# Gadersd/whisper-burn

Measured on NVIDIA H100. Metric: audio-seconds/sec, higher is better.
Workload: dtype f32 (fp16-exact weights, fp32 activations/accumulate)

## Files before the change

### include/whisper_b200.h

```cpp
#ifndef WHISPER_B200_H
#define WHISPER_B200_H

#include <stddef.h>
#include <stdint.h>

#ifdef __cplusplus
extern "C" {
#endif

#define WB_OK 0
#define WB_ERR_INVALID_ARG 1
#define WB_ERR_CUDA 2
#define WB_ERR_OOM 3
#define WB_ERR_STATE 4
#define WB_ERR_UNSUPPORTED 5

#define WB_KV_F32 0
#define WB_KV_F16 1

#define WB_WINDOWS_REFERENCE 0
#define WB_WINDOWS_NATIVE 1

#define WB_SEARCH_BEAM 0
#define WB_SEARCH_GREEDY_LOOP 1

typedef struct wb_model wb_model;
typedef struct wb_session wb_session;

typedef struct wb_dims {
    int32_t n_mels, n_audio_ctx, n_audio_state, n_audio_head, n_audio_layer;
    int32_t n_vocab, n_text_ctx, n_text_state, n_text_head, n_text_layer;
} wb_dims;

typedef struct wb_special_ids {
    int64_t sot, lang, transcribe, notimestamps, eot;
} wb_special_ids;

const char* wb_version(void);
const char* wb_last_error(void);
int wb_device_count(int* n_out);

int64_t wb_max_waveform_samples(int64_t n_frame_max);
int64_t wb_window_samples(int64_t n_audio_ctx, int window_mode);
int wb_prep_audio(int device, const float* wave, int64_t n_batch, int64_t n_samples,
                  float* mel_out, int64_t* n_frames_out);
int wb_prep_audio_dev(int device, const float* wave_dev, int64_t n_batch, int64_t n_samples,
                      float* mel_out_dev, int64_t* n_frames_out);

int wb_model_create(const wb_dims* dims, int device, wb_model** out);
int wb_model_set_tensor(wb_model* m, const char* path, const float* data, const int64_t* shape, int ndim);
int wb_npy_tree_probe(const char* dir, wb_dims* dims_out);
int wb_model_load_npy_tree(const char* dir, int device, int ln_eps_outside, wb_model** out);
int wb_model_set_layernorm_eps_mode(wb_model* m, int outside);
int wb_model_finalize(wb_model* m);
void wb_model_destroy(wb_model* m);
int wb_model_get_dims(const wb_model* m, wb_dims* out);
int wb_model_weights_fp16_exact(const wb_model* m);

int wb_forward_encoder(wb_model* m, const float* mel, int64_t n_batch, int64_t n_mels, int64_t n_ctx,
                       float* out);
int wb_forward_decoder(wb_model* m, const int64_t* tokens, int64_t n_batch, int64_t seq_len,
                       const float* encoder_output, int64_t n_enc_ctx, float* logits_out);

int wb_session_create(wb_model* m, int64_t max_windows, int64_t max_beams, int64_t max_text_len,
                      int kv_dtype, wb_session** out);
int wb_session_create_windows(wb_model* m, int64_t max_windows, int64_t max_beams, int64_t max_text_len,
                              int kv_dtype, int window_mode, wb_session** out);
void wb_session_destroy(wb_session* s);
int wb_session_set_search(wb_session* s, int rule);
int wb_session_set_prev_prompt(wb_session* s, int64_t startofprev);
int wb_session_encode_waveforms(wb_session* s, const float* const* waves, const int64_t* lens,
                                int64_t n_windows);
int wb_session_encode_waveforms_dev(wb_session* s, const float* wave_dev, const int64_t* offsets,
                                    const int64_t* lens, int64_t n_windows);
int wb_session_encode_mels(wb_session* s, const float* mel, int64_t n_windows, int64_t n_mels, int64_t n_ctx);
int wb_session_get_mel(wb_session* s, int64_t window, float* mel_out, int64_t capacity, int64_t* n_ctx_out);
int wb_session_get_encoder_output(wb_session* s, int64_t window, float* out, int64_t capacity, int64_t* n_ctx_out);
int wb_session_begin(wb_session* s, const int64_t* prompt, int64_t prompt_len);
int wb_session_step(wb_session* s, int64_t n_rows, const int32_t* window_of_row, const int32_t* parent_row,
                    const int64_t* token, int apply_special_mask, const uint8_t* is_special,
                    int k, int64_t* topk_ids_out, float* topk_logprob_out);

int wb_transcribe_windows(wb_session* s, const float* const* waves, const int64_t* lens, int64_t n_windows,
                          int beam_size, int max_depth, const wb_special_ids* ids, const uint8_t* is_special,
                          int64_t* tokens_out, int64_t capacity, int64_t* lens_out);
int wb_transcribe_windows_dev(wb_session* s, const float* wave_dev, const int64_t* offsets, const int64_t* lens,
                              int64_t n_windows, int beam_size, int max_depth, const wb_special_ids* ids,
                              const uint8_t* is_special, int64_t* tokens_out, int64_t capacity, int64_t* lens_out);
int wb_transcribe_windows_prev(wb_session* s, const float* const* waves, const int64_t* lens, int64_t n_windows,
                               const int64_t* prev_tokens, const int64_t* prev_lens, int64_t startofprev, int beam_size,
                               int max_depth, const wb_special_ids* ids, const uint8_t* is_special, int64_t* tokens_out,
                               int64_t capacity, int64_t* lens_out);
int wb_waveform_to_tokens(wb_session* s, const float* waveform, int64_t n_samples, int64_t sample_rate,
                          int beam_size, int max_depth, const wb_special_ids* ids, const uint8_t* is_special,
                          int64_t* tokens_out, int64_t capacity, int64_t* n_tokens_out);
int wb_waveforms_to_tokens(wb_session* s, const float* const* waveforms, const int64_t* n_samples, int64_t n_waveforms,
                           int64_t sample_rate, int beam_size, int max_depth, const wb_special_ids* ids,
                           const uint8_t* is_special, int64_t* tokens_out, int64_t capacity, int64_t* n_tokens_out);
int wb_session_last_logprobs(wb_session* s, int64_t index, float* out, int64_t capacity, int64_t* n_out);
int wb_session_score_tokens(wb_session* s, int64_t n_seqs, const int32_t* window_of_seq, const int64_t* tokens,
                            const int64_t* lens, int apply_special_mask, const uint8_t* is_special,
                            float* lp_out, int64_t* argmax_out);
int64_t wb_window_count(int64_t n_samples, int64_t sample_rate, int64_t window_len);
int wb_window_bounds(int64_t n_samples, int64_t sample_rate, int64_t window_len, int64_t* starts, int64_t* ends);
int wb_find_chunk_overlap(const int64_t* prev, int64_t n_prev, const int64_t* curr, int64_t n_curr,
                          int64_t max_n_offsets, int64_t min_n_overlaps, int64_t* prev_index, int64_t* curr_index);
int64_t wb_first_repetition_end(const int64_t* tokens, int64_t n, int64_t period);
int64_t wb_repetition_period(const int64_t* tokens, int64_t n, int64_t min_repetitions);
int wb_find_repeated_tokens_index(const int64_t* tokens, int64_t n, int64_t window_size, int64_t min_repeat_count,
                                  int64_t* first_repeat_index, int64_t* end);

int64_t wb_beam_get_top_elements(const double* scores, int64_t n, int64_t num, int64_t* idx_out);

int64_t wb_beam_search_table(const double* table, int64_t n_ctx, int64_t n_vocab, int64_t first_token, int64_t eot,
                             int64_t beam_size, int64_t max_depth, int64_t* seq_out, int64_t capacity);
int64_t wb_beam_search_table_fixed(const double* table, int64_t n_ctx, int64_t n_vocab, int64_t first_token, int64_t eot,
                                   int64_t beam_size, int64_t max_depth, int64_t* seq_out, int64_t capacity);

int wb_load_wav(const char* path, int strict_16k_mono, float* out, int64_t capacity, int64_t* n_samples_out,
                int64_t* sample_rate_out, int* channels_out);

int wb_session_last_decoder(const wb_session* s);
int wb_session_last_topk(wb_session* s, int64_t n_rows, int64_t k, int64_t* ids_out, float* lp_out);
int64_t wb_kernel_launch_count(void);
void wb_kernel_launch_count_reset(void);
int wb_session_last_timings(wb_session* s, float* ms_out4);
int wb_session_last_steps(wb_session* s, int64_t* n_steps_out);
int wb_session_profile_decode(wb_session* s, const wb_special_ids* ids, int n_steps, float* logits_kernel_ms,
                              float* step_ms);

#ifdef __cplusplus
}
#endif
#endif
```

### whisper-burn_b200/csrc/api.cu

```cuda
#include <algorithm>
#include <cstring>
#include <map>
#include <memory>
#include <mutex>
#include <new>

#include "../host/beam.hpp"
#include "../host/beam_fixed.hpp"
#include "../host/repeat.hpp"
#include "session.h"

struct wb_model {
    wb::Model impl;
    std::mutex fwd_mu;
    std::unique_ptr<wb::Session> fwd;
    wb::Session& forward_session(int64_t n_windows, int64_t text_len) {
        if (!fwd || fwd->max_windows < n_windows || fwd->t_max < text_len) {
            fwd.reset();
            fwd.reset(new wb::Session(&impl, std::max<int64_t>(n_windows, 1), 1, std::max<int64_t>(text_len, 2), WB_KV_F32));
        }
        return *fwd;
    }
    ~wb_model() { fwd.reset(); }
};
struct wb_session {
    std::unique_ptr<wb::Session> impl;
    wb_model* model;
    std::vector<std::vector<float>> logprobs;
    bool have_logprobs = false;
};

namespace {

template <typename F>
int guarded(F&& f) {
    try {
        f();
        return WB_OK;
    } catch (const wb::Error& e) {
        wb::set_last_error(e.what());
        return e.code;
    } catch (const std::bad_alloc&) {
        wb::set_last_error("host out of memory");
        return WB_ERR_OOM;
    } catch (const std::exception& e) {
        wb::set_last_error(e.what());
        return WB_ERR_CUDA;
    }
}

void require_device(int device) {
    int n = 0;
    cudaError_t e = cudaGetDeviceCount(&n);
    if (e != cudaSuccess || n == 0) {
        cudaGetLastError();
        wb::fail(WB_ERR_CUDA, std::string("no CUDA device available (there is no CPU fallback): ") + cudaGetErrorString(e));
    }
    if (device < 0 || device >= n) wb::fail(WB_ERR_INVALID_ARG, "device index out of range");
    WB_CUDA(cudaSetDevice(device));
}

void copy_tokens_out(const std::vector<std::vector<int64_t>>& toks, int64_t* tokens_out, int64_t capacity,
                     int64_t* lens_out) {
    for (size_t w = 0; w < toks.size(); ++w) {
        WB_REQUIRE((int64_t)toks[w].size() <= capacity, "tokens_out capacity too small");
        for (size_t i = 0; i < toks[w].size(); ++i) tokens_out[(int64_t)w * capacity + (int64_t)i] = toks[w][i];
        lens_out[w] = (int64_t)toks[w].size();
    }
}

bool special_given(const wb_session* s, const uint8_t* is_special) {
    return is_special != nullptr || (s && s->impl->search == WB_SEARCH_GREEDY_LOOP);
}

void collect_timings(wb::Session& s) {
    WB_CUDA(cudaStreamSynchronize(s.st));
    cudaEventElapsedTime(&s.last_ms[0], s.ev[0], s.ev[1]);
    cudaEventElapsedTime(&s.last_ms[1], s.ev[1], s.ev[2]);
    cudaEventElapsedTime(&s.last_ms[2], s.ev[2], s.ev[3]);
    cudaEventElapsedTime(&s.last_ms[3], s.ev[0], s.ev[3]);
}

void prep_audio_device(wb::Model& model, const float* wave_dev, int64_t n_batch, int64_t n_samples, float* mel_out_dev,
                       int64_t* n_frames_out, cudaStream_t st) {
    using namespace wb;
    WB_REQUIRE(n_batch >= 1, "prep_audio: n_batch must be >= 1");
    WB_REQUIRE(n_samples >= N_FFT, "prep_audio: waveform shorter than n_fft (audio.rs:292)");
    WB_REQUIRE(n_samples < ((int64_t)1 << 30), "prep_audio: waveform too long");
    const int F = (int)(n_samples / HOP);
    std::vector<LogMelWindow> lw((size_t)n_batch);
    for (int64_t b = 0; b < n_batch; ++b)
        lw[(size_t)b] = LogMelWindow{b * n_samples, (int)n_samples, F, F, 0, b * (int64_t)F * N_MELS};
    DevBuf<LogMelWindow> dwin;
    DevBuf<int> slot;
    DevBuf<float> rows;
    dwin.alloc((size_t)n_batch);
    slot.alloc(1);
    rows.alloc((size_t)n_batch * F * N_MELS + 4);
    WB_CUDA(cudaMemcpyAsync(dwin.p, lw.data(), lw.size() * sizeof(LogMelWindow), cudaMemcpyHostToDevice, st));
    if (F > 0) {
        launch_logmel(model, wave_dev, dwin.p, (int)n_batch, F, rows.p, slot.p, 1, st);
        for (int64_t b = 0; b < n_batch; ++b)
            launch_rows_to_chan(rows.p + b * (int64_t)F * N_MELS, mel_out_dev + b * (int64_t)N_MELS * F, F, st);
    }
    WB_CUDA(cudaStreamSynchronize(st));
    if (n_frames_out) *n_frames_out = F;
}

struct FrontendOnly {
    wb::Model m;
    explicit FrontendOnly(int device) {
        using namespace wb;
        m.device = device;
        const FrontendTables& ft = frontend_tables();
        auto up = [&](const void* src, size_t bytes) {
            void* p = nullptr;
            WB_CUDA(cudaMalloc(&p, bytes));
            m.allocs.push_back(p);
            WB_CUDA(cudaMemcpy(p, src, bytes, cudaMemcpyHostToDevice));
            return p;
        };
        m.basis_t = (float*)up(ft.basis_t.data(), ft.basis_t.size() * sizeof(float));
        m.mel_filt = (float*)up(ft.mel_filt.data(), ft.mel_filt.size() * sizeof(float));
        std::vector<int> rng(2 * N_MELS);
        for (int i = 0; i < N_MELS; ++i) { rng[2 * i] = ft.mel_lo[i]; rng[2 * i + 1] = ft.mel_hi[i]; }
        m.mel_range = (int*)up(rng.data(), rng.size() * sizeof(int));
    }
};

FrontendOnly& frontend_for(int device) {
    static std::mutex mu;
    static std::map<int, std::unique_ptr<FrontendOnly>> cache;
    std::lock_guard<std::mutex> lock(mu);
    auto& slot = cache[device];
    if (!slot) slot.reset(new FrontendOnly(device));
    return *slot;
}

}

extern "C" {

const char* wb_version(void) { return "whisper_b200 0.1.0 (sm_90a)"; }
const char* wb_last_error(void) { return wb::last_error_string().c_str(); }

int wb_device_count(int* n_out) {
    return guarded([&] {
        WB_REQUIRE(n_out != nullptr, "null output");
        int n = 0;
        if (cudaGetDeviceCount(&n) != cudaSuccess) { cudaGetLastError(); n = 0; }
        *n_out = n;
    });
}

int64_t wb_max_waveform_samples(int64_t n_frame_max) {
    return (int64_t)wb::HOP * (n_frame_max + 1) + (wb::N_FFT % 2) - 1;
}

int wb_prep_audio(int device, const float* wave, int64_t n_batch, int64_t n_samples, float* mel_out,
                  int64_t* n_frames_out) {
    return guarded([&] {
        WB_REQUIRE(wave && mel_out, "prep_audio: null pointer");
        WB_REQUIRE(n_batch >= 1, "prep_audio: n_batch must be >= 1");
        WB_REQUIRE(n_samples >= wb::N_FFT, "prep_audio: waveform shorter than n_fft (audio.rs:292)");
        require_device(device);
        FrontendOnly& fe = frontend_for(device);
        const int64_t F = n_samples / wb::HOP;
        wb::DevBuf<float> dw, dm;
        dw.alloc((size_t)(n_batch * n_samples));
        dm.alloc((size_t)(n_batch * wb::N_MELS * F) + 4);
        WB_CUDA(cudaMemcpy(dw.p, wave, (size_t)(n_batch * n_samples) * sizeof(float), cudaMemcpyHostToDevice));
        prep_audio_device(fe.m, dw.p, n_batch, n_samples, dm.p, n_frames_out, nullptr);
        WB_CUDA(cudaMemcpy(mel_out, dm.p, (size_t)(n_batch * wb::N_MELS * F) * sizeof(float), cudaMemcpyDeviceToHost));
    });
}

int wb_prep_audio_dev(int device, const float* wave_dev, int64_t n_batch, int64_t n_samples, float* mel_out_dev,
                      int64_t* n_frames_out) {
    return guarded([&] {
        WB_REQUIRE(wave_dev && mel_out_dev, "prep_audio: null pointer");
        require_device(device);
        FrontendOnly& fe = frontend_for(device);
        prep_audio_device(fe.m, wave_dev, n_batch, n_samples, mel_out_dev, n_frames_out, nullptr);
    });
}

int wb_model_create(const wb_dims* dims, int device, wb_model** out) {
    return guarded([&] {
        WB_REQUIRE(dims && out, "model_create: null pointer");
        WB_REQUIRE(dims->n_mels > 0 && dims->n_audio_ctx > 0 && dims->n_audio_state > 0 && dims->n_audio_head > 0 &&
                       dims->n_audio_layer > 0 && dims->n_vocab > 0 && dims->n_text_ctx > 0 && dims->n_text_state > 0 &&
                       dims->n_text_head > 0 && dims->n_text_layer > 0,
                   "model_create: non-positive dimension");
        require_device(device);
        wb_model* m = new wb_model();
        m->impl.dims = *dims;
        m->impl.device = device;
        *out = m;
    });
}

int wb_model_set_tensor(wb_model* m, const char* path, const float* data, const int64_t* shape, int ndim) {
    return guarded([&] {
        WB_REQUIRE(m != nullptr, "null model");
        wb::model_set_tensor(m->impl, path, data, shape, ndim);
    });
}

int wb_npy_tree_probe(const char* dir, wb_dims* dims_out) {
    return guarded([&] {
        WB_REQUIRE(dir && dims_out, "npy_tree_probe: null pointer");
        wb::npy_tree_probe(dir, *dims_out);
    });
}

int wb_model_load_npy_tree(const char* dir, int device, int ln_eps_outside, wb_model** out) {
    return guarded([&] {
        WB_REQUIRE(dir && out, "model_load_npy_tree: null pointer");
        wb_dims dims{};
        wb::npy_tree_probe(dir, dims);
        require_device(device);
        std::unique_ptr<wb_model> m(new wb_model());
        m->impl.dims = dims;
        m->impl.device = device;
        m->impl.ln_eps_outside = ln_eps_outside ? 1 : 0;
        wb::npy_tree_load(m->impl, dir);
        wb::model_finalize(m->impl);
        *out = m.release();
    });
}

int wb_model_set_layernorm_eps_mode(wb_model* m, int outside) {
    return guarded([&] {
        WB_REQUIRE(m != nullptr, "null model");
        if (m->impl.finalized) wb::fail(WB_ERR_STATE, "model already finalized");
        m->impl.ln_eps_outside = outside ? 1 : 0;
    });
}

int wb_model_finalize(wb_model* m) {
    return guarded([&] {
        WB_REQUIRE(m != nullptr, "null model");
        wb::model_finalize(m->impl);
    });
}

void wb_model_destroy(wb_model* m) { delete m; }

int wb_model_get_dims(const wb_model* m, wb_dims* out) {
    return guarded([&] {
        WB_REQUIRE(m && out, "null pointer");
        *out = m->impl.dims;
    });
}

int wb_model_weights_fp16_exact(const wb_model* m) { return (m && m->impl.fp16_exact) ? 1 : 0; }

int wb_forward_encoder(wb_model* m, const float* mel, int64_t n_batch, int64_t n_mels, int64_t n_ctx, float* out) {
    return guarded([&] {
        WB_REQUIRE(m && mel && out, "forward_encoder: null pointer");
        WB_REQUIRE(n_batch >= 1, "forward_encoder: n_batch must be >= 1");
        std::lock_guard<std::mutex> lock(m->fwd_mu);
        wb::Session& s = m->forward_session(n_batch, 2);
        s.encode_mels_host(mel, n_batch, n_mels, n_ctx);
        const int d = m->impl.dims.n_audio_state;
        WB_CUDA(cudaMemcpy(out, s.xa.p, (size_t)s.M_tot * d * sizeof(float), cudaMemcpyDeviceToHost));
    });
}

int wb_forward_decoder(wb_model* m, const int64_t* tokens, int64_t n_batch, int64_t seq_len, const float* encoder_output,
                       int64_t n_enc_ctx, float* logits_out) {
    return guarded([&] {
        WB_REQUIRE(m && tokens && encoder_output && logits_out, "forward_decoder: null pointer");
        const wb_dims& D = m->impl.dims;
        WB_REQUIRE(n_batch >= 1 && seq_len >= 1, "forward_decoder: empty input");
        WB_REQUIRE(seq_len <= D.n_text_ctx, "Token sequence length must not exceed n_text_ctx (mod.rs:134-139)");
        std::lock_guard<std::mutex> lock(m->fwd_mu);
        wb::Session& s = m->forward_session(n_batch, std::min<int64_t>(D.n_text_ctx, std::max<int64_t>(seq_len, 2)));
        s.load_encoder_output_host(encoder_output, n_batch, n_enc_ctx);
        s.teacher_forced_logits(tokens, n_batch, seq_len, logits_out);
    });
}

int64_t wb_window_samples(int64_t n_audio_ctx, int window_mode) {
    if (n_audio_ctx <= wb::MEL_PADDING || n_audio_ctx > INT32_MAX / 2 || (window_mode != WB_WINDOWS_REFERENCE && window_mode != WB_WINDOWS_NATIVE)) return -1;
    return wb::window_samples((int)n_audio_ctx, window_mode);
}

int wb_session_create_windows(wb_model* m, int64_t max_windows, int64_t max_beams, int64_t max_text_len, int kv_dtype,
                              int window_mode, wb_session** out) {
    return guarded([&] {
        WB_REQUIRE(m && out, "session_create: null pointer");
        std::unique_ptr<wb_session> s(new wb_session());
        s->model = m;
        s->impl.reset(new wb::Session(&m->impl, max_windows, max_beams, max_text_len, kv_dtype, window_mode));
        *out = s.release();
    });
}

int wb_session_create(wb_model* m, int64_t max_windows, int64_t max_beams, int64_t max_text_len, int kv_dtype,
                      wb_session** out) {
    return wb_session_create_windows(m, max_windows, max_beams, max_text_len, kv_dtype, WB_WINDOWS_REFERENCE, out);
}

void wb_session_destroy(wb_session* s) { delete s; }

int wb_session_set_search(wb_session* s, int rule) {
    return guarded([&] {
        WB_REQUIRE(s, "set_search: null pointer");
        s->impl->set_search(rule);
    });
}

int wb_session_set_prev_prompt(wb_session* s, int64_t startofprev) {
    return guarded([&] {
        WB_REQUIRE(s, "set_prev_prompt: null pointer");
        s->impl->set_prev_prompt(startofprev);
    });
}

int wb_session_encode_waveforms(wb_session* s, const float* const* waves, const int64_t* lens, int64_t n_windows) {
    return guarded([&] {
        WB_REQUIRE(s && waves && lens, "encode: null pointer");
        s->impl->encode_waveforms_host(waves, lens, n_windows);
        WB_CUDA(cudaStreamSynchronize(s->impl->st));
    });
}

int wb_session_encode_waveforms_dev(wb_session* s, const float* wave_dev, const int64_t* offsets, const int64_t* lens,
                                    int64_t n_windows) {
    return guarded([&] {
        WB_REQUIRE(s && wave_dev && offsets && lens, "encode: null pointer");
        s->impl->encode_from_device_wave(wave_dev, offsets, lens, n_windows);
        WB_CUDA(cudaStreamSynchronize(s->impl->st));
    });
}

int wb_session_encode_mels(wb_session* s, const float* mel, int64_t n_windows, int64_t n_mels, int64_t n_ctx) {
    return guarded([&] {
        WB_REQUIRE(s && mel, "encode: null pointer");
        s->impl->encode_mels_host(mel, n_windows, n_mels, n_ctx);
    });
}

int wb_session_get_mel(wb_session* s, int64_t window, float* mel_out, int64_t capacity, int64_t* n_ctx_out) {
    return guarded([&] {
        WB_REQUIRE(s && mel_out && n_ctx_out, "get_mel: null pointer");
        wb::Session& S = *s->impl;
        if (!S.encoded) wb::fail(WB_ERR_STATE, "get_mel: nothing encoded");
        WB_REQUIRE(window >= 0 && window < S.n_windows, "get_mel: window out of range");
        const int Tm = S.win_Tm[(size_t)window];
        WB_REQUIRE(capacity >= (int64_t)Tm * wb::N_MELS, "get_mel: capacity too small");
        std::vector<float> rows((size_t)Tm * wb::N_MELS);
        WB_CUDA(cudaMemcpy(rows.data(), S.mel_rows.p + ((int64_t)window * S.TmS + 1) * wb::N_MELS,
                           rows.size() * sizeof(float), cudaMemcpyDeviceToHost));
        for (int t = 0; t < Tm; ++t)
            for (int c = 0; c < wb::N_MELS; ++c) mel_out[(int64_t)c * Tm + t] = rows[(size_t)t * wb::N_MELS + c];
        *n_ctx_out = Tm;
    });
}

int wb_session_get_encoder_output(wb_session* s, int64_t window, float* out, int64_t capacity, int64_t* n_ctx_out) {
    return guarded([&] {
        WB_REQUIRE(s && out && n_ctx_out, "get_encoder_output: null pointer");
        wb::Session& S = *s->impl;
        if (!S.encoded) wb::fail(WB_ERR_STATE, "get_encoder_output: nothing encoded");
        WB_REQUIRE(window >= 0 && window < S.n_windows, "get_encoder_output: window out of range");
        const int d = S.m->dims.n_audio_state;
        const int T = S.win_T[(size_t)window];
        WB_REQUIRE(capacity >= (int64_t)T * d, "get_encoder_output: capacity too small");
        WB_CUDA(cudaMemcpy(out, S.xa.p + S.win_row_off[(size_t)window] * d, (size_t)T * d * sizeof(float),
                           cudaMemcpyDeviceToHost));
        *n_ctx_out = T;
    });
}

int wb_session_begin(wb_session* s, const int64_t* prompt, int64_t prompt_len) {
    return guarded([&] {
        WB_REQUIRE(s && prompt, "begin: null pointer");
        WB_REQUIRE(prompt_len >= 1, "begin: prompt length out of range");
        s->impl->begin(std::vector<std::vector<int64_t>>((size_t)s->impl->n_windows, std::vector<int64_t>(prompt, prompt + prompt_len)));
    });
}

int wb_session_step(wb_session* s, int64_t n_rows, const int32_t* window_of_row, const int32_t* parent_row,
                    const int64_t* token, int apply_special_mask, const uint8_t* is_special, int k,
                    int64_t* topk_ids_out, float* topk_logprob_out) {
    return guarded([&] {
        WB_REQUIRE(s && window_of_row && parent_row && token && topk_ids_out && topk_logprob_out, "step: null pointer");
        if (is_special) s->impl->set_special(is_special);
        WB_REQUIRE(!apply_special_mask || s->impl->have_special, "step: special mask requested but no is_special bitmap given");
        s->impl->step_beams(n_rows, window_of_row, parent_row, token, apply_special_mask, k, topk_ids_out, topk_logprob_out);
    });
}

int wb_transcribe_windows(wb_session* s, const float* const* waves, const int64_t* lens, int64_t n_windows,
                          int beam_size, int max_depth, const wb_special_ids* ids, const uint8_t* is_special,
                          int64_t* tokens_out, int64_t capacity, int64_t* lens_out) {
    return guarded([&] {
        WB_REQUIRE(s && waves && lens && ids && special_given(s, is_special) && tokens_out && lens_out, "transcribe: null pointer");
        s->have_logprobs = false;
        s->impl->encode_waveforms_host(waves, lens, n_windows);
        std::vector<std::vector<int64_t>> toks;
        wb::transcribe_windows(*s->impl, beam_size, max_depth, *ids, is_special, toks, s->logprobs);
        copy_tokens_out(toks, tokens_out, capacity, lens_out);
        collect_timings(*s->impl);
        s->have_logprobs = true;
    });
}

int wb_transcribe_windows_prev(wb_session* s, const float* const* waves, const int64_t* lens, int64_t n_windows,
                               const int64_t* prev_tokens, const int64_t* prev_lens, int64_t startofprev, int beam_size,
                               int max_depth, const wb_special_ids* ids, const uint8_t* is_special, int64_t* tokens_out,
                               int64_t capacity, int64_t* lens_out) {
    return guarded([&] {
        WB_REQUIRE(s && waves && lens && prev_lens && ids && special_given(s, is_special) && tokens_out && lens_out,
                   "transcribe_windows_prev: null pointer");
        wb::Session& S = *s->impl;
        WB_REQUIRE(n_windows >= 1 && n_windows <= S.max_windows, "transcribe_windows_prev: n_windows out of range");
        WB_REQUIRE(startofprev >= 0 && startofprev < S.m->dims.n_vocab, "transcribe_windows_prev: startofprev id out of range");
        WB_REQUIRE(max_depth >= 0, "transcribe_windows_prev: negative max_depth");
        std::vector<std::vector<int64_t>> prev((size_t)n_windows);
        int64_t off = 0, max_lp = 4;
        for (int64_t w = 0; w < n_windows; ++w) {
            WB_REQUIRE(prev_lens[w] >= 0, "transcribe_windows_prev: negative prev_lens entry");
            WB_REQUIRE(prev_lens[w] == 0 || prev_tokens, "transcribe_windows_prev: null prev_tokens");
            WB_REQUIRE(prev_lens[w] == 0 || S.search != WB_SEARCH_GREEDY_LOOP,
                       "transcribe_windows_prev: the greedy loop builds its own prompt; no previous ids with it");
            prev[(size_t)w].assign(prev_tokens + off, prev_tokens + off + prev_lens[w]);
            for (int64_t t : prev[(size_t)w])
                WB_REQUIRE(t >= 0 && t < S.m->dims.n_vocab, "transcribe_windows_prev: previous id out of range");
            off += prev_lens[w];
            max_lp = std::max(max_lp, prev_lens[w] > 0 ? prev_lens[w] + 5 : 4);
        }
        WB_REQUIRE(max_lp + max_depth <= S.t_max, "transcribe_windows_prev: prompt + max_depth exceeds the session's max_text_len");
        WB_REQUIRE(capacity >= max_lp + max_depth + 1, "transcribe_windows_prev: capacity below prompt + max_depth + 1");
        s->have_logprobs = false;
        S.encode_waveforms_host(waves, lens, n_windows);
        std::vector<std::vector<int64_t>> toks;
        wb::transcribe_windows(S, beam_size, max_depth, *ids, is_special, toks, s->logprobs, prev, startofprev);
        copy_tokens_out(toks, tokens_out, capacity, lens_out);
        collect_timings(S);
        s->have_logprobs = true;
    });
}

int wb_transcribe_windows_dev(wb_session* s, const float* wave_dev, const int64_t* offsets, const int64_t* lens,
                              int64_t n_windows, int beam_size, int max_depth, const wb_special_ids* ids,
                              const uint8_t* is_special, int64_t* tokens_out, int64_t capacity, int64_t* lens_out) {
    return guarded([&] {
        WB_REQUIRE(s && wave_dev && offsets && lens && ids && special_given(s, is_special) && tokens_out && lens_out, "transcribe: null pointer");
        s->have_logprobs = false;
        s->impl->encode_from_device_wave(wave_dev, offsets, lens, n_windows);
        std::vector<std::vector<int64_t>> toks;
        wb::transcribe_windows(*s->impl, beam_size, max_depth, *ids, is_special, toks, s->logprobs);
        copy_tokens_out(toks, tokens_out, capacity, lens_out);
        collect_timings(*s->impl);
        s->have_logprobs = true;
    });
}

int64_t wb_window_count(int64_t n_samples, int64_t sample_rate, int64_t window_len) {
    return (int64_t)wb::window_bounds(n_samples, sample_rate, window_len).size();
}

int wb_window_bounds(int64_t n_samples, int64_t sample_rate, int64_t window_len, int64_t* starts, int64_t* ends) {
    return guarded([&] {
        WB_REQUIRE(starts && ends, "window_bounds: null pointer");
        const auto b = wb::window_bounds(n_samples, sample_rate, window_len);
        for (size_t i = 0; i < b.size(); ++i) { starts[i] = b[i].first; ends[i] = b[i].second; }
    });
}

static void merge_window(std::vector<int64_t>& tokens, std::vector<float>& tlp, const std::vector<int64_t>& nt,
                         const std::vector<float>& nl) {
    int64_t pi = 0, ci = 0;
    if (wb::find_chunk_overlap(tokens.data(), (int64_t)tokens.size(), nt.data(), (int64_t)nt.size(), 40, 3, &pi, &ci)) {
        tokens.resize((size_t)pi);
        tokens.insert(tokens.end(), nt.begin() + ci, nt.end());
        tlp.resize((size_t)pi);
        tlp.insert(tlp.end(), nl.begin() + ci, nl.end());
    } else {
        tokens.insert(tokens.end(), nt.begin(), nt.end());
        tlp.insert(tlp.end(), nl.begin(), nl.end());
    }
}

static std::vector<int64_t> prev_nonspecial(const std::vector<int64_t>& tokens, const uint8_t* is_special) {
    std::vector<int64_t> prev;
    for (size_t i = tokens.size(); i-- > 0 && prev.size() < 5;)
        if (!is_special[tokens[i]]) prev.push_back(tokens[i]);
    std::reverse(prev.begin(), prev.end());
    return prev;
}

static void waveforms_to_tokens(wb::Session& S, const float* const* waveforms, const int64_t* n_samples, int64_t n_waveforms,
                                int64_t sample_rate, int beam_size, int max_depth, const wb_special_ids& ids,
                                const uint8_t* is_special, std::vector<std::vector<int64_t>>& out,
                                std::vector<std::vector<float>>& out_lp) {
    WB_REQUIRE(sample_rate == 16000, "waveform_to_tokens: only 16 kHz input is supported (frontend tables are built for 16 kHz)");
    const int64_t window_len = wb::window_samples(S.m->dims.n_audio_ctx, S.window_mode);
    std::vector<const float*> ptrs;
    std::vector<int64_t> lens;
    std::vector<int> owner;
    for (int64_t w = 0; w < n_waveforms; ++w)
        for (const auto& b : wb::window_bounds(n_samples[w], sample_rate, window_len)) {
            ptrs.push_back(waveforms[w] + b.first);
            lens.push_back(b.second - b.first);
            owner.push_back((int)w);
        }
    out.assign((size_t)n_waveforms, {});
    out_lp.assign((size_t)n_waveforms, {});
    const bool prev_prompt = S.startofprev >= 0;
    if (prev_prompt) {
        WB_REQUIRE(S.search != WB_SEARCH_GREEDY_LOOP, "waveform_to_tokens: the greedy loop builds its own prompt; no previous-text prompt with it");
        WB_REQUIRE(is_special != nullptr, "waveform_to_tokens: the previous-text prompt needs is_special");
    }
    std::vector<std::vector<size_t>> rounds(1);
    if (prev_prompt) {
        std::vector<int> idx((size_t)n_waveforms, 0);
        for (size_t j = 0; j < ptrs.size(); ++j) {
            const size_t i = (size_t)idx[(size_t)owner[j]]++;
            if (rounds.size() <= i) rounds.resize(i + 1);
            rounds[i].push_back(j);
        }
    } else {
        for (size_t j = 0; j < ptrs.size(); ++j) rounds[0].push_back(j);
    }
    for (const std::vector<size_t>& round : rounds) {
        for (size_t b0 = 0; b0 < round.size(); b0 += (size_t)S.max_windows) {
            const size_t nb = std::min(round.size() - b0, (size_t)S.max_windows);
            std::vector<const float*> bp(nb);
            std::vector<int64_t> bl(nb);
            std::vector<std::vector<int64_t>> prev(prev_prompt ? nb : 0);
            for (size_t i = 0; i < nb; ++i) {
                const size_t j = round[b0 + i];
                bp[i] = ptrs[j];
                bl[i] = lens[j];
                if (prev_prompt) prev[i] = prev_nonspecial(out[(size_t)owner[j]], is_special);
            }
            S.encode_waveforms_host(bp.data(), bl.data(), (int64_t)nb);
            std::vector<std::vector<int64_t>> toks;
            std::vector<std::vector<float>> lps;
            wb::transcribe_windows(S, beam_size, max_depth, ids, is_special, toks, lps, prev, S.startofprev);
            for (size_t i = 0; i < nb; ++i)
                merge_window(out[(size_t)owner[round[b0 + i]]], out_lp[(size_t)owner[round[b0 + i]]], toks[i], lps[i]);
        }
    }
    collect_timings(S);
}

int wb_waveform_to_tokens(wb_session* s, const float* waveform, int64_t n_samples, int64_t sample_rate, int beam_size,
                          int max_depth, const wb_special_ids* ids, const uint8_t* is_special, int64_t* tokens_out,
                          int64_t capacity, int64_t* n_tokens_out) {
    return guarded([&] {
        WB_REQUIRE(s && waveform && ids && special_given(s, is_special) && tokens_out && n_tokens_out, "waveform_to_tokens: null pointer");
        s->have_logprobs = false;
        std::vector<std::vector<int64_t>> out;
        waveforms_to_tokens(*s->impl, &waveform, &n_samples, 1, sample_rate, beam_size, max_depth, *ids, is_special, out, s->logprobs);
        WB_REQUIRE((int64_t)out[0].size() <= capacity, "tokens_out capacity too small");
        std::memcpy(tokens_out, out[0].data(), out[0].size() * sizeof(int64_t));
        *n_tokens_out = (int64_t)out[0].size();
        s->have_logprobs = true;
    });
}

int wb_waveforms_to_tokens(wb_session* s, const float* const* waveforms, const int64_t* n_samples, int64_t n_waveforms,
                           int64_t sample_rate, int beam_size, int max_depth, const wb_special_ids* ids,
                           const uint8_t* is_special, int64_t* tokens_out, int64_t capacity, int64_t* n_tokens_out) {
    return guarded([&] {
        WB_REQUIRE(s && waveforms && n_samples && ids && special_given(s, is_special) && tokens_out && n_tokens_out, "waveforms_to_tokens: null pointer");
        WB_REQUIRE(n_waveforms >= 1, "waveforms_to_tokens: n_waveforms must be >= 1");
        s->have_logprobs = false;
        std::vector<std::vector<int64_t>> out;
        waveforms_to_tokens(*s->impl, waveforms, n_samples, n_waveforms, sample_rate, beam_size, max_depth, *ids, is_special, out,
                            s->logprobs);
        for (int64_t w = 0; w < n_waveforms; ++w) {
            WB_REQUIRE((int64_t)out[(size_t)w].size() <= capacity, "tokens_out capacity (per waveform) too small");
            std::memcpy(tokens_out + w * capacity, out[(size_t)w].data(), out[(size_t)w].size() * sizeof(int64_t));
            n_tokens_out[w] = (int64_t)out[(size_t)w].size();
        }
        s->have_logprobs = true;
    });
}

int wb_session_last_logprobs(wb_session* s, int64_t index, float* out, int64_t capacity, int64_t* n_out) {
    return guarded([&] {
        WB_REQUIRE(s && n_out, "last_logprobs: null pointer");
        if (!s->have_logprobs) wb::fail(WB_ERR_STATE, "last_logprobs: no transcribe or waveform(s)_to_tokens call yet");
        WB_REQUIRE(index >= 0 && index < (int64_t)s->logprobs.size(), "last_logprobs: index out of range");
        const std::vector<float>& v = s->logprobs[(size_t)index];
        *n_out = (int64_t)v.size();
        if (!out) return;
        WB_REQUIRE(capacity >= (int64_t)v.size(), "last_logprobs: capacity too small");
        std::memcpy(out, v.data(), v.size() * sizeof(float));
    });
}

int wb_session_score_tokens(wb_session* s, int64_t n_seqs, const int32_t* window_of_seq, const int64_t* tokens, const int64_t* lens,
                            int apply_special_mask, const uint8_t* is_special, float* lp_out, int64_t* argmax_out) {
    return guarded([&] {
        WB_REQUIRE(s && window_of_seq && tokens && lens && lp_out, "score_tokens: null pointer");
        s->impl->score_tokens(n_seqs, window_of_seq, tokens, lens, apply_special_mask != 0, is_special, lp_out, argmax_out);
    });
}

int wb_find_chunk_overlap(const int64_t* prev, int64_t n_prev, const int64_t* curr, int64_t n_curr, int64_t max_n_offsets,
                          int64_t min_n_overlaps, int64_t* prev_index, int64_t* curr_index) {
    int64_t pi = 0, ci = 0;
    const bool found = wb::find_chunk_overlap(prev, n_prev, curr, n_curr, max_n_offsets, min_n_overlaps, &pi, &ci);
    if (found) {
        if (prev_index) *prev_index = pi;
        if (curr_index) *curr_index = ci;
    }
    return found ? 1 : 0;
}

int64_t wb_first_repetition_end(const int64_t* tokens, int64_t n, int64_t period) {
    if ((!tokens && n > 0) || n < 0) return -1;
    return wb::repeat::first_repetition_end(tokens, n, period);
}

int64_t wb_repetition_period(const int64_t* tokens, int64_t n, int64_t min_repetitions) {
    if ((!tokens && n > 0) || n < 0) return -1;
    return wb::repeat::repetition_period(tokens, n, min_repetitions);
}

int wb_find_repeated_tokens_index(const int64_t* tokens, int64_t n, int64_t window_size, int64_t min_repeat_count, int64_t* first_repeat_index,
                                  int64_t* end) {
    if ((!tokens && n > 0) || n < 0 || !first_repeat_index || !end) return -1;
    return wb::repeat::find_repeated_tokens_index(tokens, n, window_size, min_repeat_count, first_repeat_index, end);
}

int64_t wb_beam_get_top_elements(const double* scores, int64_t n, int64_t num, int64_t* idx_out) {
    if (!scores || !idx_out || n < 0 || num < 0) return -1;
    std::vector<double> v(scores, scores + n);
    const auto top = wb::beam::get_top_elements(v, [](double s) { return s; }, (size_t)num);
    for (size_t i = 0; i < top.size(); ++i) idx_out[i] = (int64_t)top[i];
    return (int64_t)top.size();
}

int wb_load_wav(const char* path, int strict_16k_mono, float* out, int64_t capacity, int64_t* n_samples_out, int64_t* sample_rate_out,
                int* channels_out) {
    return guarded([&] {
        WB_REQUIRE(path && n_samples_out, "load_wav: null pointer");
        std::vector<float> v;
        int64_t sr = 0;
        int ch = 0;
        wb::load_wav(path, strict_16k_mono != 0, v, sr, ch);
        *n_samples_out = (int64_t)v.size();
        if (sample_rate_out) *sample_rate_out = sr;
        if (channels_out) *channels_out = ch;
        if (out) {
            WB_REQUIRE(capacity >= (int64_t)v.size(), "load_wav: capacity too small");
            std::memcpy(out, v.data(), v.size() * sizeof(float));
        }
    });
}

int wb_session_last_decoder(const wb_session* s) { return s ? s->impl->last_decoder : -1; }

int wb_session_last_topk(wb_session* s, int64_t n_rows, int64_t k, int64_t* ids_out, float* lp_out) {
    return guarded([&] {
        WB_REQUIRE(s && ids_out && lp_out, "last_topk: null pointer");
        s->impl->last_topk(n_rows, k, ids_out, lp_out);
    });
}

int64_t wb_beam_search_table(const double* table, int64_t n_ctx, int64_t n_vocab, int64_t first_token, int64_t eot, int64_t beam_size,
                             int64_t max_depth, int64_t* seq_out, int64_t capacity) {
    if (!table || !seq_out || n_ctx < 1 || n_vocab < 1 || beam_size < 1 || max_depth < 0) return -1;
    using Node = wb::beam::BeamNode<int64_t>;
    auto next = [&](const std::vector<Node>& beams) {
        std::vector<std::vector<std::pair<int64_t, double>>> out(beams.size());
        for (size_t b = 0; b < beams.size(); ++b) {
            const int64_t t = beams[b].seq.back(), n = (int64_t)beams[b].seq.size();
            const double* row = table + ((t * 131 + n) % n_ctx) * n_vocab;
            out[b].reserve((size_t)n_vocab);
            for (int64_t v = 0; v < n_vocab; ++v) out[b].emplace_back(v, beams[b].log_prob + row[v]);
        }
        return out;
    };
    auto fin = [&](const std::vector<int64_t>& seq) { return !seq.empty() && seq.back() == eot; };
    std::vector<Node> init(1);
    init[0].seq = {first_token};
    init[0].log_prob = 0.0;
    const std::vector<int64_t> best = wb::beam::beam_search(init, next, fin, (size_t)beam_size, (size_t)max_depth);
    if ((int64_t)best.size() > capacity) return -1;
    for (size_t i = 0; i < best.size(); ++i) seq_out[i] = best[i];
    return (int64_t)best.size();
}

int64_t wb_beam_search_table_fixed(const double* table, int64_t n_ctx, int64_t n_vocab, int64_t first_token, int64_t eot,
                                   int64_t beam_size, int64_t max_depth, int64_t* seq_out, int64_t capacity) {
    namespace fx = wb::beamfx;
    if (!table || !seq_out || n_ctx < 1 || n_vocab < 1 || beam_size < 1 || beam_size > fx::MAX_BEAM || max_depth < 0) return -1;
    const int B = (int)beam_size;
    std::vector<fx::Head> heads(1);
    std::vector<std::vector<int64_t>> seqs(1, std::vector<int64_t>{first_token});
    heads[0] = fx::Head{0.0, first_token == eot ? 1 : 0, 0, 1, 0};
    std::vector<double> scores((size_t)n_vocab);
    for (int64_t depth = 0; depth < max_depth; ++depth) {
        const int n = (int)heads.size();
        if (fx::search_done(heads.data(), n)) break;
        int step_row[fx::MAX_NODES], cand_id[fx::MAX_NODES * fx::MAX_BEAM];
        double cand_lp[fx::MAX_NODES * fx::MAX_BEAM];
        for (int b = 0; b < n; ++b) {
            step_row[b] = b;
            for (int i = 0; i < B; ++i) cand_id[b * B + i] = -1;
            if (heads[(size_t)b].finished) continue;
            const int64_t t = seqs[(size_t)b].back(), len = (int64_t)seqs[(size_t)b].size();
            const double* row = table + ((t * 131 + len) % n_ctx) * n_vocab;
            for (int64_t v = 0; v < n_vocab; ++v) scores[(size_t)v] = heads[(size_t)b].log_prob + row[v];
            int top[fx::MAX_BEAM + 1];
            const int nt = fx::top_elements(scores.data(), (int)n_vocab, B, top);
            for (int i = 0; i < nt; ++i) {
                cand_id[b * B + i] = top[i];
                cand_lp[b * B + i] = row[top[i]];
            }
        }
        fx::Pick out[fx::MAX_NODES];
        const int n_out = fx::beam_step(heads.data(), n, step_row, cand_id, cand_lp, B, (int)eot, out);
        std::vector<fx::Head> nh((size_t)n_out);
        std::vector<std::vector<int64_t>> ns((size_t)n_out);
        for (int i = 0; i < n_out; ++i) {
            nh[(size_t)i] = out[i].head;
            ns[(size_t)i] = seqs[(size_t)out[i].src];
            if (out[i].token >= 0) ns[(size_t)i].push_back(out[i].token);
        }
        heads.swap(nh);
        seqs.swap(ns);
    }
    const int best = fx::max_by_last(heads.data(), (int)heads.size());
    if (best < 0) return 0;
    const std::vector<int64_t>& s = seqs[(size_t)best];
    if ((int64_t)s.size() > capacity) return -1;
    for (size_t i = 0; i < s.size(); ++i) seq_out[i] = s[i];
    return (int64_t)s.size();
}

int64_t wb_kernel_launch_count(void) { return wb::g_launch_count; }
void wb_kernel_launch_count_reset(void) { wb::g_launch_count = 0; }

int wb_session_last_timings(wb_session* s, float* ms_out4) {
    return guarded([&] {
        WB_REQUIRE(s && ms_out4, "null pointer");
        for (int i = 0; i < 4; ++i) ms_out4[i] = s->impl->last_ms[i];
    });
}

int wb_session_profile_decode(wb_session* s, const wb_special_ids* ids, int n_steps, float* logits_kernel_ms,
                              float* step_ms) {
    return guarded([&] {
        WB_REQUIRE(s && ids && logits_kernel_ms && step_ms, "null pointer");
        const int64_t prompt[4] = {ids->sot, ids->lang, ids->transcribe, ids->notimestamps};
        s->impl->profile_decode(prompt, 4, n_steps, logits_kernel_ms, step_ms);
    });
}

int wb_session_last_steps(wb_session* s, int64_t* n_steps_out) {
    return guarded([&] {
        WB_REQUIRE(s && n_steps_out, "null pointer");
        *n_steps_out = s->impl->last_steps;
    });
}

}
```

### whisper-burn_b200/csrc/gemm_f16.cu

```cuda
#include <cuda.h>
#include <cuda_fp16.h>

#include <climits>
#include <cstring>
#include <mutex>
#include <type_traits>

#include "prims.cuh"
#include "wb_internal.h"
#include "wgmma.cuh"

namespace wb {

namespace {

constexpr int F_BM = 128, F_BK = 64, F_STAGES = 4;
constexpr int F_CONSUMERS = 256;
constexpr int F_THREADS = F_CONSUMERS + 32;

__device__ __forceinline__ void tma_load_3d(void* dst, const CUtensorMap* map, uint64_t* bar, int c0, int c1, int c2) {
    asm volatile("cp.async.bulk.tensor.3d.shared::cluster.global.tile.mbarrier::complete_tx::bytes [%0], [%1, {%3, %4, %5}], [%2];" ::"r"(smem_u32(dst)), "l"(map),
                 "r"(smem_u32(bar)), "r"(c0), "r"(c1), "r"(c2)
                 : "memory");
}
__device__ __forceinline__ void tma_load_2d(void* dst, const CUtensorMap* map, uint64_t* bar, int c0, int c1) {
    asm volatile("cp.async.bulk.tensor.2d.shared::cluster.global.tile.mbarrier::complete_tx::bytes [%0], [%1, {%3, %4}], [%2];" ::"r"(smem_u32(dst)), "l"(map),
                 "r"(smem_u32(bar)), "r"(c0), "r"(c1)
                 : "memory");
}
template <int BN>
__device__ __forceinline__ void wgmma_tile(float (&d)[BN / 2], uint64_t desc_a, uint64_t desc_b) {
    if constexpr (BN == 128) wgmma_m64n128k16(d, desc_a, desc_b);
    else wgmma_m64n64k16(d, desc_a, desc_b);
}

struct F16Args {
    float* C;
    __half *P_hi, *P_lo;
    const float* bias;
    const float* residual;
    const float* pos;
    const GemmGroup* groups;
    GemmGroup single;
    int64_t ldc;
    int N, K;
    int act;
    float scale;
    int scale_cols;
};
struct LogitArgs : F16Args {
    const int* target;
    const uint8_t* row_mask;
    const uint8_t* is_special;
    int V, n_tiles;
    float *tile_m, *tile_s, *tgt_logit;
    int* tile_i;
};

template <int BN>
__device__ __forceinline__ void logit_stats_epilogue(const float (&acc_h)[BN / 2], const float (&acc_l)[BN / 2], const LogitArgs& g, int rows,
                                                     int m_base, int n0, int lane) {
#pragma unroll
    for (int hrow = 0; hrow < 2; ++hrow) {
        const int m = m_base + 8 * hrow;
        const bool live = m < rows;
        const int mr = live ? m : 0;
        const bool masked = g.row_mask != nullptr && g.row_mask[mr] != 0;
        const int tgt = g.target[mr];
        float mx = -INFINITY;
        int ai = INT_MAX;
#pragma unroll
        for (int j = 0; j < BN / 8; ++j)
#pragma unroll
            for (int e = 0; e < 2; ++e) {
                const int n = n0 + 8 * j + 2 * (lane & 3) + e;
                const float x = hl_join(acc_h[4 * j + 2 * hrow + e], acc_l[4 * j + 2 * hrow + e]);
                if (live && n == tgt) g.tgt_logit[m] = x;
                const bool ok = n < g.V && !(masked && __ldg(g.is_special + n));
                if (ok && x > mx) { mx = x; ai = n; }
            }
#pragma unroll
        for (int o = 1; o <= 2; o <<= 1) {
            const float om = __shfl_xor_sync(0xffffffffu, mx, o);
            const int oi = __shfl_xor_sync(0xffffffffu, ai, o);
            if (om > mx || (om == mx && oi < ai)) { mx = om; ai = oi; }
        }
        float s = 0.0f;
#pragma unroll
        for (int j = 0; j < BN / 8; ++j)
#pragma unroll
            for (int e = 0; e < 2; ++e) {
                const int n = n0 + 8 * j + 2 * (lane & 3) + e;
                const float x = hl_join(acc_h[4 * j + 2 * hrow + e], acc_l[4 * j + 2 * hrow + e]);
                if (n < g.V && !(masked && __ldg(g.is_special + n))) s += expf(x - mx);
            }
        s += __shfl_xor_sync(0xffffffffu, s, 1);
        s += __shfl_xor_sync(0xffffffffu, s, 2);
        if (live && (lane & 3) == 0) {
            const int64_t o = (int64_t)m * g.n_tiles + blockIdx.x;
            g.tile_m[o] = mx;
            g.tile_s[o] = s;
            g.tile_i[o] = ai;
        }
    }
}

template <int BN, typename Args>
__global__ void __launch_bounds__(F_THREADS, 1)
gemm_f16_tc_kernel(const __grid_constant__ CUtensorMap map_a_hi, const __grid_constant__ CUtensorMap map_a_lo,
                   const __grid_constant__ CUtensorMap map_b, const Args g) {
    extern __shared__ __align__(1024) uint8_t smem_raw[];
    constexpr int A_BYTES = F_BM * F_BK * 2;
    constexpr int B_BYTES = BN * F_BK * 2;
    constexpr int STAGE = 2 * A_BYTES + B_BYTES;
    uint8_t* base = reinterpret_cast<uint8_t*>((reinterpret_cast<uintptr_t>(smem_raw) + 1023) & ~(uintptr_t)1023);
    uint64_t* full = reinterpret_cast<uint64_t*>(base + F_STAGES * STAGE);
    uint64_t* empty = full + F_STAGES;

    const int warp = threadIdx.x >> 5, lane = threadIdx.x & 31;
    const GemmGroup grp = g.groups ? g.groups[blockIdx.z] : g.single;
    const int m0 = blockIdx.y * F_BM;
    if (m0 >= grp.rows) return;
    const int n0 = blockIdx.x * BN;
    const int nkb = (g.K + F_BK - 1) / F_BK;

    if (threadIdx.x == F_CONSUMERS) {
        asm volatile("prefetch.tensormap [%0];" ::"l"(&map_a_hi) : "memory");
        asm volatile("prefetch.tensormap [%0];" ::"l"(&map_a_lo) : "memory");
        asm volatile("prefetch.tensormap [%0];" ::"l"(&map_b) : "memory");
        for (int s = 0; s < F_STAGES; ++s) {
            mbar_init(full + s, 1);
            mbar_init(empty + s, 2);
        }
        mbar_fence_init();
    }
    __syncthreads();

    if (threadIdx.x >= F_CONSUMERS) {
        if (lane == 0) {
            for (int i = 0; i < nkb; ++i) {
                const int s = i % F_STAGES;
                const uint32_t ph = (i / F_STAGES) & 1;
                mbar_wait(empty + s, ph ^ 1);
                mbar_expect_tx(full + s, STAGE);
                uint8_t* st = base + s * STAGE;
                tma_load_3d(st, &map_a_hi, full + s, i * F_BK, m0, blockIdx.z);
                tma_load_3d(st + A_BYTES, &map_a_lo, full + s, i * F_BK, m0, blockIdx.z);
                tma_load_2d(st + 2 * A_BYTES, &map_b, full + s, i * F_BK, n0);
            }
        }
        return;
    }
    const int wg = warp >> 2;
    float acc_h[BN / 2], acc_l[BN / 2];
#pragma unroll
    for (int j = 0; j < BN / 2; ++j) { acc_h[j] = 0.0f; acc_l[j] = 0.0f; }
    wgmma_fence_regs(acc_h);
    wgmma_fence_regs(acc_l);
#pragma unroll 1
    for (int i = 0; i < nkb; ++i) {
        const int s = i % F_STAGES;
        mbar_wait(full + s, (i / F_STAGES) & 1);
        const uint32_t st = smem_u32(base + s * STAGE);
        const uint64_t dah = wgmma_desc(st + wg * 8192), dal = wgmma_desc(st + A_BYTES + wg * 8192), db = wgmma_desc(st + 2 * A_BYTES);
        wgmma_fence();
#pragma unroll
        for (int k = 0; k < F_BK / 16; ++k) {
            wgmma_tile<BN>(acc_h, dah + 2 * k, db + 2 * k);
            wgmma_tile<BN>(acc_l, dal + 2 * k, db + 2 * k);
        }
        wgmma_commit();
        wgmma_wait<1>();
        if (i > 0 && (threadIdx.x & 127) == 0) mbar_arrive(empty + (i - 1) % F_STAGES);
    }
    wgmma_wait<0>();
    wgmma_fence_regs(acc_h);
    wgmma_fence_regs(acc_l);

    if constexpr (std::is_same<Args, LogitArgs>::value) {
        logit_stats_epilogue<BN>(acc_h, acc_l, g, grp.rows, m0 + wg * 64 + (warp & 3) * 16 + (lane >> 2), n0, lane);
    } else {
#pragma unroll
        for (int hrow = 0; hrow < 2; ++hrow) {
            const int m = m0 + wg * 64 + (warp & 3) * 16 + (lane >> 2) + 8 * hrow;
            if (m >= grp.rows) continue;
            const int64_t crow = grp.c_off + (int64_t)m * g.ldc;
#pragma unroll
            for (int j = 0; j < BN / 8; ++j) {
                const int n = n0 + 8 * j + 2 * (lane & 3);
                float v[2];
#pragma unroll
                for (int e = 0; e < 2; ++e) {
                    float t = hl_join(acc_h[4 * j + 2 * hrow + e], acc_l[4 * j + 2 * hrow + e]);
                    if (g.bias) t = __fadd_rn(t, __ldg(g.bias + n + e));
                    if (g.act == ACT_GELU) t = gelu_erf(t);
                    if (n + e < g.scale_cols) t = __fmul_rn(t, g.scale);
                    v[e] = t;
                }
                if (g.pos) {
                    const float2 p2 = __ldg(reinterpret_cast<const float2*>(g.pos + (int64_t)m * g.N + n));
                    v[0] = __fadd_rn(v[0], p2.x); v[1] = __fadd_rn(v[1], p2.y);
                }
                if (g.residual) {
                    const float2 r2 = *reinterpret_cast<const float2*>(g.residual + crow + n);
                    v[0] = __fadd_rn(r2.x, v[0]); v[1] = __fadd_rn(r2.y, v[1]);
                }
                if (g.C) *reinterpret_cast<float2*>(g.C + crow + n) = make_float2(v[0], v[1]);
                if (g.P_hi) {
                    __half2 h, l;
                    hl_split_pair(v[0], v[1], h, l);
                    *reinterpret_cast<__half2*>(g.P_hi + crow + n) = h;
                    *reinterpret_cast<__half2*>(g.P_lo + crow + n) = l;
                }
            }
        }
    }
}

__global__ void split_f16_kernel(const float4* __restrict__ src, uint2* __restrict__ hi, uint2* __restrict__ lo, int64_t n4) {
    for (int64_t i = (int64_t)blockIdx.x * blockDim.x + threadIdx.x; i < n4; i += (int64_t)gridDim.x * blockDim.x)
        hl_split4(src[i], hi[i], lo[i]);
}

typedef CUresult (*EncodeTiledFn)(CUtensorMap*, CUtensorMapDataType, cuuint32_t, void*, const cuuint64_t*, const cuuint64_t*,
                                  const cuuint32_t*, const cuuint32_t*, CUtensorMapInterleave, CUtensorMapSwizzle,
                                  CUtensorMapL2promotion, CUtensorMapFloatOOBfill);

EncodeTiledFn encode_fn() {
    static std::once_flag once;
    static EncodeTiledFn fn = nullptr;
    std::call_once(once, [] {
        void* p = nullptr;
        cudaDriverEntryPointQueryResult q;
        if (cudaGetDriverEntryPoint("cuTensorMapEncodeTiled", &p, cudaEnableDefault, &q) == cudaSuccess && q == cudaDriverEntryPointSuccess) fn = (EncodeTiledFn)p;
    });
    if (!fn) fail(WB_ERR_CUDA, "cuTensorMapEncodeTiled not available");
    return fn;
}

CUtensorMap make_map(const __half* base, uint64_t dim0, uint64_t dim1, uint64_t dim2, uint64_t s1, uint64_t s2, uint32_t b0, uint32_t b1, int rank) {
    CUtensorMap m;
    std::memset(&m, 0, sizeof(m));
    cuuint64_t dims[3] = {dim0, dim1, dim2};
    cuuint64_t strides[2] = {s1 * sizeof(__half), s2 * sizeof(__half)};
    cuuint32_t box[3] = {b0, b1, 1};
    cuuint32_t estr[3] = {1, 1, 1};
    const CUresult r = encode_fn()(&m, CU_TENSOR_MAP_DATA_TYPE_FLOAT16, (cuuint32_t)rank, (void*)base, dims, strides, box, estr, CU_TENSOR_MAP_INTERLEAVE_NONE,
                                   CU_TENSOR_MAP_SWIZZLE_128B, CU_TENSOR_MAP_L2_PROMOTION_L2_128B, CU_TENSOR_MAP_FLOAT_OOB_FILL_NONE);
    if (r != CUDA_SUCCESS) fail(WB_ERR_UNSUPPORTED, "cuTensorMapEncodeTiled failed: " + std::to_string((int)r));
    return m;
}

template <int BN, typename Args>
void launch_f16_t(const CUtensorMap& ah, const CUtensorMap& al, const CUtensorMap& b, const Args& a, dim3 grid, cudaStream_t st) {
    constexpr size_t smem = 1024 + (size_t)F_STAGES * (2 * F_BM * F_BK * 2 + BN * F_BK * 2) + 2 * F_STAGES * sizeof(uint64_t);
    static std::mutex mu;
    static bool configured[16] = {};
    int dev = 0;
    WB_CUDA(cudaGetDevice(&dev));
    {
        std::lock_guard<std::mutex> lock(mu);
        if (dev >= 0 && dev < 16 && !configured[dev]) {
            WB_CUDA(cudaFuncSetAttribute(gemm_f16_tc_kernel<BN, Args>, cudaFuncAttributeMaxDynamicSharedMemorySize, (int)smem));
            configured[dev] = true;
        }
    }
    gemm_f16_tc_kernel<BN, Args><<<grid, F_THREADS, smem, st>>>(ah, al, b, a);
    WB_LAUNCH_CHECK();
}

}

void launch_split_f16(const float* src, __half* hi, __half* lo, int64_t n, cudaStream_t st) {
    WB_REQUIRE(n % 4 == 0, "split: length must be a multiple of 4");
    const int64_t n4 = n / 4;
    if (n4 == 0) return;
    const int blocks = (int)std::min<int64_t>((n4 + 255) / 256, 132 * 8);
    split_f16_kernel<<<blocks, 256, 0, st>>>(reinterpret_cast<const float4*>(src), reinterpret_cast<uint2*>(hi), reinterpret_cast<uint2*>(lo), n4);
    WB_LAUNCH_CHECK();
}

bool gemm_f16_supported(const GemmF16Params& p) { return p.N % 64 == 0 && p.K % 8 == 0 && p.lda % 8 == 0 && p.ldc % 4 == 0; }

struct GemmF16Plan::Impl {
    CUtensorMap ah, al, b;
    F16Args args;
    dim3 grid;
    int BN;
};
GemmF16Plan::GemmF16Plan() = default;
GemmF16Plan::~GemmF16Plan() { delete impl; }

void GemmF16Plan::build(const GemmF16Params& p, int64_t a_group_stride, int a_rows_total_per_group) {
    WB_REQUIRE(gemm_f16_supported(p), "gemm_f16: unsupported shape");
    delete impl;
    impl = new Impl();
    const int ng = p.groups ? p.n_groups : 1;
    const uint64_t rows = (uint64_t)a_rows_total_per_group;
    const uint64_t gstride = ng > 1 ? (uint64_t)a_group_stride : (uint64_t)p.lda * rows;
    impl->ah = make_map(p.A_hi, (uint64_t)p.K, rows, (uint64_t)ng, (uint64_t)p.lda, gstride, F_BK, F_BM, 3);
    impl->al = make_map(p.A_lo, (uint64_t)p.K, rows, (uint64_t)ng, (uint64_t)p.lda, gstride, F_BK, F_BM, 3);
    impl->BN = (p.N % 128 == 0 && (int64_t)(p.N / 128) * ((p.max_rows + F_BM - 1) / F_BM) * ng >= 96) ? 128 : 64;
    impl->b = make_map(p.B, (uint64_t)p.K, (uint64_t)p.N, 1, (uint64_t)p.K, (uint64_t)p.K * p.N, F_BK, (uint32_t)impl->BN, 2);
    F16Args& a = impl->args;
    a.C = p.C; a.P_hi = p.P_hi; a.P_lo = p.P_lo; a.bias = p.bias; a.residual = p.residual; a.pos = p.pos; a.groups = p.groups;
    a.single = GemmGroup{0, 0, p.max_rows};
    a.ldc = p.ldc; a.N = p.N; a.K = p.K; a.act = p.act; a.scale = p.scale; a.scale_cols = p.scale_cols;
    impl->grid = dim3(p.N / impl->BN, (p.max_rows + F_BM - 1) / F_BM, ng);
    key_rows = p.max_rows;
    key_groups = ng;
}

void GemmF16Plan::launch(cudaStream_t st) const {
    if (!impl || impl->args.single.rows <= 0 || impl->grid.y == 0) return;
    if (impl->BN == 128) launch_f16_t<128>(impl->ah, impl->al, impl->b, impl->args, impl->grid, st);
    else launch_f16_t<64>(impl->ah, impl->al, impl->b, impl->args, impl->grid, st);
}

int logit_stats_tiles(int V) { return (V + 127) / 128; }

void launch_logit_stats(const LogitStatsParams& p, cudaStream_t st) {
    WB_REQUIRE(p.rows >= 1 && p.K % 8 == 0 && p.V >= 1, "logit_stats: unsupported shape");
    constexpr int BN = 128;
    const CUtensorMap ah = make_map(p.A_hi, (uint64_t)p.K, (uint64_t)p.rows, 1, (uint64_t)p.K, (uint64_t)p.K * p.rows, F_BK, F_BM, 3);
    const CUtensorMap al = make_map(p.A_lo, (uint64_t)p.K, (uint64_t)p.rows, 1, (uint64_t)p.K, (uint64_t)p.K * p.rows, F_BK, F_BM, 3);
    const CUtensorMap b = make_map(p.E, (uint64_t)p.K, (uint64_t)p.V, 1, (uint64_t)p.K, (uint64_t)p.K * p.V, F_BK, BN, 2);
    LogitArgs a{};
    a.single = GemmGroup{0, 0, p.rows};
    a.K = p.K;
    a.target = p.target; a.row_mask = p.row_mask; a.is_special = p.is_special;
    a.V = p.V; a.n_tiles = logit_stats_tiles(p.V);
    a.tile_m = p.tile_m; a.tile_s = p.tile_s; a.tile_i = p.tile_i; a.tgt_logit = p.tgt_logit;
    launch_f16_t<BN>(ah, al, b, a, dim3(a.n_tiles, (p.rows + F_BM - 1) / F_BM, 1), st);
}

}
```

### whisper-burn_b200/csrc/model.cu

```cuda
#include <cmath>
#include <cstring>

#include "wb_internal.h"

namespace wb {

thread_local int64_t g_launch_count = 0;
static thread_local std::string g_last_error;

void set_last_error(const std::string& m) { g_last_error = m; }
const std::string& last_error_string() { return g_last_error; }
void fail(int code, const std::string& m) { throw Error(code, m); }

Model::~Model() {
    for (void* p : allocs) cudaFree(p);
}

namespace {

using Tensor = std::pair<std::vector<int64_t>, std::vector<float>>;

const Tensor& need(const Model& m, const std::string& path, std::initializer_list<int64_t> shape) {
    auto it = m.host.find(path);
    if (it == m.host.end()) fail(WB_ERR_STATE, "missing tensor: " + path);
    const auto& sh = it->second.first;
    std::vector<int64_t> want(shape);
    if (sh != want) {
        std::string s = "bad shape for " + path + ": got [";
        for (auto v : sh) s += std::to_string(v) + ",";
        s += "] want [";
        for (auto v : want) s += std::to_string(v) + ",";
        fail(WB_ERR_INVALID_ARG, s + "]");
    }
    return it->second;
}

bool fp16_exact(const std::vector<float>& v) {
    for (float f : v) {
        if (__half2float(__float2half_rn(f)) != f) return false;
    }
    return true;
}

float* up32(Model& m, const std::vector<float>& v) {
    float* p = nullptr;
    WB_CUDA(cudaMalloc((void**)&p, std::max<size_t>(v.size(), 1) * sizeof(float)));
    m.allocs.push_back(p);
    if (!v.empty()) WB_CUDA(cudaMemcpy(p, v.data(), v.size() * sizeof(float), cudaMemcpyHostToDevice));
    return p;
}
__half* up16(Model& m, const std::vector<float>& v) {
    std::vector<__half> h(v.size());
    for (size_t i = 0; i < v.size(); ++i) h[i] = __float2half_rn(v[i]);
    __half* p = nullptr;
    WB_CUDA(cudaMalloc((void**)&p, std::max<size_t>(v.size(), 1) * sizeof(__half)));
    m.allocs.push_back(p);
    if (!v.empty()) WB_CUDA(cudaMemcpy(p, h.data(), h.size() * sizeof(__half), cudaMemcpyHostToDevice));
    return p;
}

void append_transposed(std::vector<float>& dst, const std::vector<float>& w, int d_in, int d_out) {
    const size_t base = dst.size();
    dst.resize(base + (size_t)d_in * d_out);
    for (int i = 0; i < d_in; ++i)
        for (int o = 0; o < d_out; ++o) dst[base + (size_t)o * d_in + i] = w[(size_t)i * d_out + o];
}

struct LinSpec {
    std::vector<float> w;
    std::vector<float> b;
    int n = 0, k = 0;
};

void add_linear(const Model& m, LinSpec& s, const std::string& path, int d_in, int d_out, bool has_bias) {
    const Tensor& w = need(m, path + "/weight", {d_in, d_out});
    append_transposed(s.w, w.second, d_in, d_out);
    if (has_bias) {
        const Tensor& b = need(m, path + "/bias", {d_out});
        s.b.insert(s.b.end(), b.second.begin(), b.second.end());
    } else {
        s.b.insert(s.b.end(), (size_t)d_out, 0.0f);
    }
    s.k = d_in;
    s.n += d_out;
}

LinearW upload_linear(Model& m, const LinSpec& s, bool want32, bool want16) {
    LinearW L;
    L.n = s.n;
    L.k = s.k;
    if (want32) L.w32 = up32(m, s.w);
    if (want16) L.w16 = up16(m, s.w);
    L.b = up32(m, s.b);
    return L;
}

LayerNormW upload_ln(Model& m, const std::string& path, int n) {
    LayerNormW L;
    L.g = up32(m, need(m, path + "/weight", {n}).second);
    L.b = up32(m, need(m, path + "/bias", {n}).second);
    auto it = m.host.find(path + "/eps");
    if (it == m.host.end() || it->second.second.empty()) fail(WB_ERR_STATE, "missing tensor: " + path + "/eps");
    L.eps = it->second.second.back();
    return L;
}

}

void model_set_tensor(Model& m, const char* path, const float* data, const int64_t* shape, int ndim) {
    if (m.finalized) fail(WB_ERR_STATE, "model already finalized");
    WB_REQUIRE(path && data && ndim >= 0 && ndim <= 4, "set_tensor: bad arguments");
    size_t n = 1;
    std::vector<int64_t> sh;
    for (int i = 0; i < ndim; ++i) {
        WB_REQUIRE(shape[i] >= 0, "set_tensor: negative dimension");
        n *= (size_t)shape[i];
        sh.push_back(shape[i]);
    }
    std::string key(path);
    if (key.size() >= 4 && key.compare(key.size() - 4, 4, "/eps") == 0) sh.clear();
    m.host[key] = Tensor(sh, std::vector<float>(data, data + n));
}

void model_finalize(Model& m) {
    if (m.finalized) fail(WB_ERR_STATE, "model already finalized");
    const wb_dims& D = m.dims;
    WB_REQUIRE(D.n_audio_state == D.n_text_state, "Audio encoder state size must be equal to text decoder state size.");
    WB_REQUIRE(D.n_audio_state % D.n_audio_head == 0 && D.n_text_state % D.n_text_head == 0,
               "State size must be a multiple of head size");
    WB_REQUIRE(D.n_audio_state / D.n_audio_head == 64 && D.n_text_state / D.n_text_head == 64,
               "only head dimension 64 (all Whisper sizes) is supported");
    WB_REQUIRE(D.n_mels == N_MELS, "n_mels must be 80");
    WB_REQUIRE(D.n_audio_state % 16 == 0, "n_state must be a multiple of 16");
    WB_CUDA(cudaSetDevice(m.device));
    const int d = D.n_audio_state;

    bool exact = true;
    for (const auto& kv : m.host) {
        if (kv.first.size() >= 4 && kv.first.compare(kv.first.size() - 4, 4, "/eps") == 0) continue;
        if (!fp16_exact(kv.second.second)) { exact = false; break; }
    }
    m.fp16_exact = exact;

    const FrontendTables& ft = frontend_tables();
    m.basis_t = up32(m, ft.basis_t);
    m.mel_filt = up32(m, ft.mel_filt);
    {
        std::vector<int> rng(2 * N_MELS);
        for (int i = 0; i < N_MELS; ++i) { rng[2 * i] = ft.mel_lo[i]; rng[2 * i + 1] = ft.mel_hi[i]; }
        WB_CUDA(cudaMalloc((void**)&m.mel_range, rng.size() * sizeof(int)));
        m.allocs.push_back(m.mel_range);
        WB_CUDA(cudaMemcpy(m.mel_range, rng.data(), rng.size() * sizeof(int), cudaMemcpyHostToDevice));
    }

    auto conv = [&](const std::string& path, int c_in) {
        const Tensor& w = need(m, path + "/weight", {d, c_in, 3});
        const Tensor& b = need(m, path + "/bias", {d});
        LinSpec s;
        s.n = d;
        s.k = 3 * c_in;
        s.w.resize((size_t)d * 3 * c_in);
        for (int o = 0; o < d; ++o)
            for (int c = 0; c < c_in; ++c)
                for (int kk = 0; kk < 3; ++kk)
                    s.w[(size_t)o * 3 * c_in + (size_t)kk * c_in + c] = w.second[((size_t)o * c_in + c) * 3 + kk];
        s.b = b.second;
        return upload_linear(m, s, !exact, exact);
    };
    m.conv1 = conv("encoder/conv1", D.n_mels);
    m.conv2 = conv("encoder/conv2", d);
    m.enc_pos = up32(m, need(m, "encoder/positional_embedding", {D.n_audio_ctx, d}).second);
    m.enc.resize(D.n_audio_layer);
    for (int i = 0; i < D.n_audio_layer; ++i) {
        const std::string p = "encoder/block_" + std::to_string(i);
        EncBlockW& B = m.enc[i];
        B.attn_ln = upload_ln(m, p + "/attn_ln", d);
        B.mlp_ln = upload_ln(m, p + "/mlp_ln", d);
        LinSpec qkv;
        add_linear(m, qkv, p + "/attn/query", d, d, true);
        add_linear(m, qkv, p + "/attn/key", d, d, false);
        add_linear(m, qkv, p + "/attn/value", d, d, true);
        B.qkv = upload_linear(m, qkv, !exact, exact);
        LinSpec o, m1, m2;
        add_linear(m, o, p + "/attn/out", d, d, true);
        add_linear(m, m1, p + "/mlp/mlp1", d, 4 * d, true);
        add_linear(m, m2, p + "/mlp/mlp2", 4 * d, d, true);
        B.out = upload_linear(m, o, !exact, exact);
        B.mlp1 = upload_linear(m, m1, !exact, exact);
        B.mlp2 = upload_linear(m, m2, !exact, exact);
    }
    m.ln_post = upload_ln(m, "encoder/ln_post", d);

    const bool h16 = exact, h32 = !exact;
    const Tensor& emb = need(m, "decoder/token_embedding/weight", {D.n_vocab, d});
    m.tok_emb32 = up32(m, emb.second);
    if (h16) m.tok_emb16 = up16(m, emb.second);
    if (h16 && (d == 128 || d == 384)) {
        const int V = D.n_vocab, tiles = (V + 15) / 16, kh = d / 2;
        std::vector<float> tl((size_t)tiles * 2 * 16 * kh, 0.0f);
        for (int t = 0; t < tiles; ++t)
            for (int hh = 0; hh < 2; ++hh)
                for (int rr = 0; rr < 16 && t * 16 + rr < V; ++rr)
                    std::memcpy(&tl[(((size_t)t * 2 + hh) * 16 + rr) * kh], &emb.second[(size_t)(t * 16 + rr) * d + (size_t)hh * kh], sizeof(float) * kh);
        m.tok_emb16_tiled = up16(m, tl);
    }
    m.dec_pos = up32(m, need(m, "decoder/positional_embedding", {D.n_text_ctx, d}).second);
    m.dec.resize(D.n_text_layer);
    for (int i = 0; i < D.n_text_layer; ++i) {
        const std::string p = "decoder/block_" + std::to_string(i);
        DecBlockW& B = m.dec[i];
        B.attn_ln = upload_ln(m, p + "/attn_ln", d);
        B.cross_ln = upload_ln(m, p + "/cross_attn_ln", d);
        B.mlp_ln = upload_ln(m, p + "/mlp_ln", d);
        LinSpec qkv, o, cq, ckv, co, m1, m2;
        add_linear(m, qkv, p + "/attn/query", d, d, true);
        add_linear(m, qkv, p + "/attn/key", d, d, false);
        add_linear(m, qkv, p + "/attn/value", d, d, true);
        add_linear(m, o, p + "/attn/out", d, d, true);
        add_linear(m, cq, p + "/cross_attn/query", d, d, true);
        add_linear(m, ckv, p + "/cross_attn/key", d, d, false);
        add_linear(m, ckv, p + "/cross_attn/value", d, d, true);
        add_linear(m, co, p + "/cross_attn/out", d, d, true);
        add_linear(m, m1, p + "/mlp/mlp1", d, 4 * d, true);
        add_linear(m, m2, p + "/mlp/mlp2", 4 * d, d, true);
        B.qkv = upload_linear(m, qkv, h32, h16);
        B.out = upload_linear(m, o, h32, h16);
        B.cq = upload_linear(m, cq, h32, h16);
        B.ckv = upload_linear(m, ckv, h32, h16);
        B.cout = upload_linear(m, co, h32, h16);
        B.mlp1 = upload_linear(m, m1, h32, h16);
        B.mlp2 = upload_linear(m, m2, h32, h16);
    }
    m.dec_ln = upload_ln(m, "decoder/ln", d);
    {
        std::vector<float> z((size_t)std::max(4 * d, D.n_vocab), 0.0f);
        m.zero_bias = up32(m, z);
    }
    m.host.clear();
    m.finalized = true;
}

}
```

### whisper-burn_b200/csrc/session.cu

```cuda
#include <algorithm>
#include <cmath>
#include <cstdio>
#include <cstdlib>
#include <cstring>

#include "session.h"

namespace wb {

int window_mel_frames(int n_audio_ctx, int window_mode) {
    WB_REQUIRE(window_mode == WB_WINDOWS_REFERENCE || window_mode == WB_WINDOWS_NATIVE,
               "window_mode must be WB_WINDOWS_REFERENCE or WB_WINDOWS_NATIVE");
    return window_mode == WB_WINDOWS_NATIVE ? 2 * n_audio_ctx : n_audio_ctx;
}

int64_t window_samples(int n_audio_ctx, int window_mode) {
    return wb_max_waveform_samples(window_mel_frames(n_audio_ctx, window_mode) - MEL_PADDING);
}

Session::Session(Model* model, int64_t max_w, int64_t max_b, int64_t max_text_len, int kv, int mode) : m(model) {
    if (!m || !m->finalized) fail(WB_ERR_STATE, "session: model not finalized");
    const wb_dims& D = m->dims;
    WB_REQUIRE(max_w >= 1 && max_b >= 1 && max_w * max_b <= 4096, "session: bad max_windows / max_beams");
    WB_REQUIRE(max_text_len >= 2 && max_text_len <= D.n_text_ctx, "session: max_text_len must be in [2, n_text_ctx]");
    WB_REQUIRE(kv == WB_KV_F32 || kv == WB_KV_F16, "session: kv_dtype must be WB_KV_F32 or WB_KV_F16");
    WB_CUDA(cudaSetDevice(m->device));
    max_windows = (int)max_w;
    max_beams = (int)max_b;
    t_max = (int)max_text_len;
    kv_dtype = kv;
    window_mode = mode;
    mel_limit = window_mel_frames(D.n_audio_ctx, mode);
    Rmax = max_windows * max_beams;
    TmS = mel_limit + 2;
    Tcap = (mel_limit - 1) / 2 + 1;
    Mcap = (int64_t)max_windows * Tcap;
    const int d = D.n_audio_state, H = D.n_text_head, L = D.n_text_layer, V = D.n_vocab;
    WB_REQUIRE(max_beams <= DEC_KC - 1, "session: max_beams must be <= 7 (candidates kept per record by the persistent decoders)");
    if (const char* e = getenv("WB200_DECODER"); e && e[0]) {
        only_decoder = atoi(e);
        WB_REQUIRE(only_decoder >= 3 && only_decoder <= 6, "session: WB200_DECODER must be 3, 4, 5 or 6");
    }

    WB_CUDA(cudaStreamCreateWithFlags(&st, cudaStreamNonBlocking));
    for (auto& e : ev) WB_CUDA(cudaEventCreate(&e));
    d_lmwin.alloc(max_windows); d_g1.alloc(max_windows); d_g2.alloc(max_windows); d_awin.alloc(max_windows);
    d_win_row_off.alloc(max_windows); d_win_T.alloc(max_windows);
    max_slots.alloc(max_windows);
    mel_rows.alloc((size_t)max_windows * TmS * N_MELS);
    x.alloc(Mcap * d);
    xa.alloc(Mcap * d);
    if (kv == WB_KV_F16) ckv16.alloc((size_t)L * Mcap * 2 * d); else ckv.alloc((size_t)L * Mcap * 2 * d);
    use_tc = m->fp16_exact;
    if (use_tc) {
        const size_t nm = (size_t)max_windows * TmS * N_MELS, nh = (size_t)max_windows * TmS * d;
        mel_h.alloc(nm); mel_l.alloc(nm); h1_h.alloc(nh); h1_l.alloc(nh);
        xn_h.alloc(Mcap * d); xn_l.alloc(Mcap * d); qkv_h.alloc(Mcap * 3 * d); qkv_l.alloc(Mcap * 3 * d);
        att_h.alloc(Mcap * d); att_l.alloc(Mcap * d); hid_h.alloc(Mcap * 4 * d); hid_l.alloc(Mcap * 4 * d);
        xa_h.alloc(Mcap * d); xa_l.alloc(Mcap * d);
        enc_plans.resize((size_t)2 + 4 * D.n_audio_layer + L);
        for (auto& pl : enc_plans) pl.reset(new GemmF16Plan());
    } else {
        h1.alloc((size_t)max_windows * TmS * d);
        xn.alloc(Mcap * d); att.alloc(Mcap * d); qkv.alloc(Mcap * 3 * d); hid.alloc(Mcap * 4 * d);
    }
    if (kv == WB_KV_F16) { kc16.alloc((size_t)L * Rmax * t_max * d); vc16.alloc((size_t)L * Rmax * t_max * d); }
    else { kc.alloc((size_t)L * Rmax * t_max * d); vc.alloc((size_t)L * Rmax * t_max * d); }
    dx.alloc((size_t)Rmax * d);
    att_pl.alloc(4 * dec5_plane_uint4(d)); hid_pl.alloc(8 * dec5_plane_uint4(d));
    WB_CUDA(cudaMemsetAsync(att_pl.p, 0, 4 * dec5_plane_uint4(d) * sizeof(uint4), st));
    WB_CUDA(cudaMemsetAsync(hid_pl.p, 0, 8 * dec5_plane_uint4(d) * sizeof(uint4), st));
    dq.alloc((size_t)Rmax * d); dhid.alloc((size_t)Rmax * 4 * d);
    logits.alloc((size_t)Rmax * V);
    tokens.alloc((size_t)Rmax * t_max); token_lp.alloc((size_t)Rmax * t_max); lengths.alloc((size_t)2 * Rmax); cur_tok.alloc(Rmax); finished.alloc(Rmax);
    row_window.alloc(Rmax); anc0.alloc((size_t)Rmax * t_max); anc1.alloc((size_t)Rmax * t_max); parent.alloc(Rmax);
    pos.alloc(1); n_unfinished.alloc(128);
    topk_id.alloc((size_t)Rmax * DEC_KC); topk_lp.alloc((size_t)Rmax * DEC_KC);
    eot_logit.alloc(Rmax);
    is_special.alloc(V);
    {
        ckv_tmp.alloc(Mcap * 2 * d);
        cudaDeviceProp prop;
        WB_CUDA(cudaGetDeviceProperties(&prop, m->device));
        n_sm = prop.multiProcessorCount;
        const int n_logit_ctas = 2 * prop.multiProcessorCount;
        part_o.alloc((size_t)Rmax * H * 16 * 64); part_m.alloc((size_t)Rmax * H * 16); part_l.alloc((size_t)Rmax * H * 16);
        datt.alloc((size_t)Rmax * d); steps_done.alloc(128); dec_bar.alloc(4);
        WB_CUDA(cudaMemsetAsync(dec_bar.p, 0, 4 * sizeof(unsigned int), st));
        {
            const bool h16 = m->fp16_exact;
            auto wp = [&](const LinearW& w) -> const void* { return h16 ? (const void*)w.w16 : (const void*)w.w32; };
            std::vector<DecLayer> lay((size_t)L);
            for (int l = 0; l < L; ++l) {
                const DecBlockW& B = m->dec[(size_t)l];
                DecLayer& y = lay[(size_t)l];
                y.ln1_g = B.attn_ln.g; y.ln1_b = B.attn_ln.b; y.ln1_eps = B.attn_ln.eps;
                y.ln2_g = B.cross_ln.g; y.ln2_b = B.cross_ln.b; y.ln2_eps = B.cross_ln.eps;
                y.ln3_g = B.mlp_ln.g; y.ln3_b = B.mlp_ln.b; y.ln3_eps = B.mlp_ln.eps;
                y.Wqkv = wp(B.qkv); y.Wo = wp(B.out); y.Wcq = wp(B.cq); y.Wco = wp(B.cout); y.W1 = wp(B.mlp1); y.W2 = wp(B.mlp2);
                y.bqkv = B.qkv.b; y.bo = B.out.b; y.bcq = B.cq.b; y.bco = B.cout.b; y.b1 = B.mlp1.b; y.b2 = B.mlp2.b;
            }
            dec_layers.alloc((size_t)L);
            WB_CUDA(cudaMemcpy(dec_layers.p, lay.data(), lay.size() * sizeof(DecLayer), cudaMemcpyHostToDevice));
        }
        dec5_build_tables(*m, n_sm, d5);
        ypart.alloc((size_t)4 * Rmax * d);
        lg_m.alloc((size_t)n_logit_ctas * Rmax); lg_s.alloc((size_t)n_logit_ctas * Rmax);
        lg_v.alloc((size_t)n_logit_ctas * Rmax * DEC_KC); lg_i.alloc((size_t)n_logit_ctas * Rmax * DEC_KC);
    }
    h_parent = pinned<int>(Rmax); h_window = pinned<int>(Rmax); h_token = pinned<int>(Rmax);
    h_topk_id = pinned<int>((size_t)Rmax * DEC_KC);
    WB_CUDA(cudaMemsetAsync(is_special.p, 0, V, st));

    DecArgs& a = dec_base;
    a.Rmax = Rmax; a.d = D.n_text_state; a.H = H; a.L = L; a.V = V; a.t_max = t_max; a.Mcap = Mcap;
    a.eps_outside = m->ln_eps_outside; a.qk_scale = (float)std::pow((double)D.n_text_state / (double)H, -0.25);
    a.layers = dec_layers.p; a.tok_emb = m->tok_emb32; a.pos_emb = m->dec_pos;
    a.E = m->fp16_exact ? (const void*)m->tok_emb16 : (const void*)m->tok_emb32;
    a.E_tiled = m->tok_emb16_tiled;
    a.lnf_g = m->dec_ln.g; a.lnf_b = m->dec_ln.b; a.lnf_eps = m->dec_ln.eps;
    a.x = dx.p; a.q = dq.p; a.att = datt.p; a.hid = dhid.p;
    a.ypart = ypart.p; a.lgbuf = logits.p; a.att_pl = att_pl.p; a.hid_pl = hid_pl.p;
    a.kv_half = kv == WB_KV_F16 ? 1 : 0;
    if (a.kv_half) { a.kc = kc16.p; a.vc = vc16.p; a.ckv = ckv16.p; } else { a.kc = kc.p; a.vc = vc.p; a.ckv = ckv.p; }
    a.row_window = row_window.p; a.win_row_off = d_win_row_off.p; a.win_T = d_win_T.p;
    a.part_o = part_o.p; a.part_m = part_m.p; a.part_l = part_l.p;
    a.tokens = tokens.p; a.token_lp = token_lp.p; a.cur_tok = cur_tok.p; a.lengths = lengths.p; a.finished = finished.p;
    a.eot_logit = eot_logit.p; a.topk_id = topk_id.p; a.topk_lp = topk_lp.p;
    a.lg_m = lg_m.p; a.lg_s = lg_s.p; a.lg_v = lg_v.p; a.lg_i = lg_i.p;
    a.pos = pos.p; a.n_unfinished = n_unfinished.p; a.steps_done = steps_done.p; a.bar = dec_bar.p;
    WB_CUDA(cudaStreamSynchronize(st));
}

Session::~Session() {
    if (st) cudaStreamSynchronize(st);
    for (auto& e : ev)
        if (e) cudaEventDestroy(e);
    if (st) cudaStreamDestroy(st);
}

static void set_geometry(Session& s, const std::vector<int>& Tm) {
    s.n_windows = (int)Tm.size();
    s.win_Tm = Tm;
    s.win_T.resize(Tm.size());
    s.win_row_off.resize(Tm.size());
    s.M_tot = 0;
    s.max_T = 0;
    s.max_Tm = 0;
    for (size_t w = 0; w < Tm.size(); ++w) {
        s.win_T[w] = (Tm[w] - 1) / 2 + 1;
        s.win_row_off[w] = s.M_tot;
        s.M_tot += s.win_T[w];
        s.max_T = std::max(s.max_T, s.win_T[w]);
        s.max_Tm = std::max(s.max_Tm, Tm[w]);
    }
    const int d = s.m->dims.n_audio_state;
    std::vector<GemmGroup> g1(Tm.size()), g2(Tm.size());
    std::vector<AttnWindow> aw(Tm.size());
    for (size_t w = 0; w < Tm.size(); ++w) {
        g1[w] = GemmGroup{(int64_t)w * s.TmS * N_MELS, ((int64_t)w * s.TmS + 1) * d, Tm[w]};
        g2[w] = GemmGroup{(int64_t)w * s.TmS * d, s.win_row_off[w] * d, s.win_T[w]};
        aw[w] = AttnWindow{s.win_row_off[w], s.win_T[w]};
    }
    WB_CUDA(cudaMemcpyAsync(s.d_g1.p, g1.data(), g1.size() * sizeof(GemmGroup), cudaMemcpyHostToDevice, s.st));
    WB_CUDA(cudaMemcpyAsync(s.d_g2.p, g2.data(), g2.size() * sizeof(GemmGroup), cudaMemcpyHostToDevice, s.st));
    WB_CUDA(cudaMemcpyAsync(s.d_awin.p, aw.data(), aw.size() * sizeof(AttnWindow), cudaMemcpyHostToDevice, s.st));
    WB_CUDA(cudaMemcpyAsync(s.d_win_row_off.p, s.win_row_off.data(), Tm.size() * sizeof(int64_t),
                            cudaMemcpyHostToDevice, s.st));
    WB_CUDA(cudaMemcpyAsync(s.d_win_T.p, s.win_T.data(), Tm.size() * sizeof(int), cudaMemcpyHostToDevice, s.st));
    WB_CUDA(cudaStreamSynchronize(s.st));
}

void Session::encode_from_device_wave(const float* wave_dev, const int64_t* offsets, const int64_t* lens, int64_t n) {
    WB_REQUIRE(n >= 1 && n <= max_windows, "encode: n_windows out of range for this session");
    std::vector<LogMelWindow> lw((size_t)n);
    std::vector<int> Tm((size_t)n);
    int max_frames = 0;
    for (int64_t w = 0; w < n; ++w) {
        WB_REQUIRE(lens[w] >= N_FFT, "prep_audio: waveform shorter than n_fft (audio.rs:292)");
        WB_REQUIRE(lens[w] < (int64_t)1 << 30, "prep_audio: waveform too long");
        const int F = (int)(lens[w] / HOP);
        const int keep = std::min(F, mel_limit - MEL_PADDING);
        Tm[(size_t)w] = keep + MEL_PADDING;
        lw[(size_t)w] = LogMelWindow{offsets[w], (int)lens[w], F, keep, (int)w, ((int64_t)w * TmS + 1) * N_MELS};
        max_frames = std::max(max_frames, F);
    }
    WB_CUDA(cudaMemcpyAsync(d_lmwin.p, lw.data(), lw.size() * sizeof(LogMelWindow), cudaMemcpyHostToDevice, st));
    set_geometry(*this, Tm);
    WB_CUDA(cudaEventRecord(ev[0], st));
    WB_CUDA(cudaMemsetAsync(mel_rows.p, 0, (size_t)n * TmS * N_MELS * sizeof(float), st));
    launch_logmel(*m, wave_dev, d_lmwin.p, (int)n, max_frames, mel_rows.p, max_slots.p, (int)n, st);
    WB_CUDA(cudaEventRecord(ev[1], st));
    run_encoder();
    WB_CUDA(cudaEventRecord(ev[2], st));
}

void Session::encode_waveforms_host(const float* const* waves, const int64_t* lens, int64_t n) {
    WB_REQUIRE(n >= 1 && n <= max_windows, "encode: n_windows out of range for this session");
    std::vector<int64_t> offs((size_t)n);
    int64_t total = 0;
    for (int64_t w = 0; w < n; ++w) {
        WB_REQUIRE(waves[w] != nullptr && lens[w] >= 0, "encode: null waveform");
        offs[(size_t)w] = total;
        total += (lens[w] + 3) / 4 * 4;
    }
    wave.ensure((size_t)total);
    for (int64_t w = 0; w < n; ++w)
        WB_CUDA(cudaMemcpyAsync(wave.p + offs[(size_t)w], waves[w], (size_t)lens[w] * sizeof(float),
                                cudaMemcpyHostToDevice, st));
    encode_from_device_wave(wave.p, offs.data(), lens, n);
}

void Session::encode_mels_host(const float* mel, int64_t n, int64_t n_mels, int64_t n_ctx) {
    const wb_dims& D = m->dims;
    WB_REQUIRE(n_mels == D.n_mels, "Audio mel spectrum size must be n_mels (mod.rs:231-235)");
    WB_REQUIRE(n_ctx >= 1 && n_ctx <= mel_limit, "Audio length cannot exceed the session's mel frame limit: n_audio_ctx, "
                                                 "2 * n_audio_ctx in native windowing (mod.rs:236-241)");
    WB_REQUIRE(n >= 1 && n <= max_windows, "encode: n_windows out of range for this session");
    std::vector<int> Tm((size_t)n, (int)n_ctx);
    set_geometry(*this, Tm);
    DevBuf<float> tmp;
    tmp.alloc((size_t)n * n_mels * n_ctx);
    WB_CUDA(cudaMemcpyAsync(tmp.p, mel, tmp.n * sizeof(float), cudaMemcpyHostToDevice, st));
    WB_CUDA(cudaMemsetAsync(mel_rows.p, 0, (size_t)n * TmS * N_MELS * sizeof(float), st));
    for (int64_t w = 0; w < n; ++w)
        launch_chan_to_rows(tmp.p + w * n_mels * n_ctx, mel_rows.p + ((int64_t)w * TmS + 1) * N_MELS, (int)n_ctx, n_ctx, st);
    run_encoder();
    WB_CUDA(cudaStreamSynchronize(st));
}

void Session::load_encoder_output_host(const float* xa_host, int64_t n, int64_t T) {
    WB_REQUIRE(n >= 1 && n <= max_windows && T >= 1 && T <= Tcap, "forward_decoder: encoder output shape out of range");
    std::vector<int> Tm((size_t)n, (int)(2 * T - 1));
    set_geometry(*this, Tm);
    const int d = m->dims.n_audio_state;
    WB_CUDA(cudaMemcpyAsync(xa.p, xa_host, (size_t)n * T * d * sizeof(float), cudaMemcpyHostToDevice, st));
    if (use_tc) launch_split_f16(xa.p, xa_h.p, xa_l.p, (int64_t)n * T * d, st);
    run_cross_kv();
    encoded = true;
}

void Session::run_encoder() {
    if (use_tc) run_encoder_f16();
    else run_encoder_f32();
    run_cross_kv();
    encoded = true;
}

void Session::run_encoder_f16() {
    const wb_dims& D = m->dims;
    const int d = D.n_audio_state;
    const int M = (int)M_tot;
    const float qk_scale = (float)std::pow((double)d / (double)D.n_audio_head, -0.25);
    auto run = [&](size_t site, const GemmF16Params& p, int64_t gstride, int rows_per_group) {
        GemmF16Plan& pl = *enc_plans[site];
        if (!pl.matches(p.max_rows, p.groups ? p.n_groups : 1)) pl.build(p, gstride, rows_per_group);
        pl.launch(st);
    };
    WB_CUDA(cudaMemsetAsync(h1_h.p, 0, (size_t)n_windows * TmS * d * sizeof(__half), st));
    WB_CUDA(cudaMemsetAsync(h1_l.p, 0, (size_t)n_windows * TmS * d * sizeof(__half), st));
    launch_split_f16(mel_rows.p, mel_h.p, mel_l.p, (int64_t)n_windows * TmS * N_MELS, st);
    GemmF16Params p;
    p.A_hi = mel_h.p; p.A_lo = mel_l.p; p.lda = N_MELS; p.B = m->conv1.w16; p.P_hi = h1_h.p; p.P_lo = h1_l.p; p.ldc = d; p.N = d; p.K = 3 * N_MELS;
    p.bias = m->conv1.b; p.act = ACT_GELU; p.groups = d_g1.p; p.n_groups = n_windows; p.max_rows = max_Tm;
    run(0, p, (int64_t)TmS * N_MELS, TmS - 2);
    p = GemmF16Params{};
    p.A_hi = h1_h.p; p.A_lo = h1_l.p; p.lda = 2 * d; p.B = m->conv2.w16; p.C = x.p; p.ldc = d; p.N = d; p.K = 3 * d;
    p.bias = m->conv2.b; p.act = ACT_GELU; p.pos = m->enc_pos; p.groups = d_g2.p; p.n_groups = n_windows; p.max_rows = max_T;
    run(1, p, (int64_t)TmS * d, Tcap);
    for (int l = 0; l < D.n_audio_layer; ++l) {
        const EncBlockW& B = m->enc[(size_t)l];
        const size_t site = (size_t)2 + 4 * l;
        launch_layernorm_f16(x.p, nullptr, xn_h.p, xn_l.p, B.attn_ln, M, d, m->ln_eps_outside, st);
        p = GemmF16Params{};
        p.A_hi = xn_h.p; p.A_lo = xn_l.p; p.lda = d; p.B = B.qkv.w16; p.P_hi = qkv_h.p; p.P_lo = qkv_l.p; p.ldc = 3 * d; p.N = 3 * d; p.K = d;
        p.bias = B.qkv.b; p.scale = qk_scale; p.scale_cols = 2 * d; p.max_rows = M;
        run(site, p, 0, M);
        launch_encoder_attention_tc(qkv_h.p, qkv_l.p, att_h.p, att_l.p, d_awin.p, n_windows, max_T, d, D.n_audio_head, st);
        p = GemmF16Params{};
        p.A_hi = att_h.p; p.A_lo = att_l.p; p.lda = d; p.B = B.out.w16; p.C = x.p; p.ldc = d; p.N = d; p.K = d;
        p.bias = B.out.b; p.residual = x.p; p.max_rows = M;
        run(site + 1, p, 0, M);
        launch_layernorm_f16(x.p, nullptr, xn_h.p, xn_l.p, B.mlp_ln, M, d, m->ln_eps_outside, st);
        p = GemmF16Params{};
        p.A_hi = xn_h.p; p.A_lo = xn_l.p; p.lda = d; p.B = B.mlp1.w16; p.P_hi = hid_h.p; p.P_lo = hid_l.p; p.ldc = 4 * d; p.N = 4 * d; p.K = d;
        p.bias = B.mlp1.b; p.act = ACT_GELU; p.max_rows = M;
        run(site + 2, p, 0, M);
        p = GemmF16Params{};
        p.A_hi = hid_h.p; p.A_lo = hid_l.p; p.lda = 4 * d; p.B = B.mlp2.w16; p.C = x.p; p.ldc = d; p.N = d; p.K = 4 * d;
        p.bias = B.mlp2.b; p.residual = x.p; p.max_rows = M;
        run(site + 3, p, 0, M);
    }
    launch_layernorm_f16(x.p, xa.p, xa_h.p, xa_l.p, m->ln_post, M, d, m->ln_eps_outside, st);
}

void Session::run_encoder_f32() {
    const wb_dims& D = m->dims;
    const int d = D.n_audio_state;
    const int M = (int)M_tot;
    const float qk_scale = (float)std::pow((double)d / (double)D.n_audio_head, -0.25);
    WB_CUDA(cudaMemsetAsync(h1.p, 0, (size_t)n_windows * TmS * d * sizeof(float), st));
    GemmParams p;
    p.A = mel_rows.p; p.lda = N_MELS; p.B = m->conv1.w32; p.C = h1.p; p.ldc = d; p.N = d; p.K = 3 * N_MELS;
    p.bias = m->conv1.b; p.act = ACT_GELU; p.groups = d_g1.p; p.n_groups = n_windows; p.max_rows = max_Tm;
    launch_gemm(p, st);
    p = GemmParams{};
    p.A = h1.p; p.lda = 2 * d; p.B = m->conv2.w32; p.C = x.p; p.ldc = d; p.N = d; p.K = 3 * d;
    p.bias = m->conv2.b; p.act = ACT_GELU; p.pos = m->enc_pos; p.groups = d_g2.p; p.n_groups = n_windows;
    p.max_rows = max_T;
    launch_gemm(p, st);
    for (int l = 0; l < D.n_audio_layer; ++l) {
        const EncBlockW& B = m->enc[(size_t)l];
        launch_layernorm(x.p, xn.p, B.attn_ln, M, d, m->ln_eps_outside, st);
        p = GemmParams{};
        p.A = xn.p; p.lda = d; p.B = B.qkv.w32; p.C = qkv.p; p.ldc = 3 * d; p.N = 3 * d; p.K = d;
        p.bias = B.qkv.b; p.scale = qk_scale; p.scale_cols = 2 * d; p.max_rows = M;
        launch_gemm(p, st);
        launch_encoder_attention(qkv.p, att.p, d_awin.p, n_windows, max_T, d, D.n_audio_head, st);
        p = GemmParams{};
        p.A = att.p; p.lda = d; p.B = B.out.w32; p.C = x.p; p.ldc = d; p.N = d; p.K = d;
        p.bias = B.out.b; p.residual = x.p; p.max_rows = M;
        launch_gemm(p, st);
        launch_layernorm(x.p, xn.p, B.mlp_ln, M, d, m->ln_eps_outside, st);
        p = GemmParams{};
        p.A = xn.p; p.lda = d; p.B = B.mlp1.w32; p.C = hid.p; p.ldc = 4 * d; p.N = 4 * d; p.K = d;
        p.bias = B.mlp1.b; p.act = ACT_GELU; p.max_rows = M;
        launch_gemm(p, st);
        p = GemmParams{};
        p.A = hid.p; p.lda = 4 * d; p.B = B.mlp2.w32; p.C = x.p; p.ldc = d; p.N = d; p.K = 4 * d;
        p.bias = B.mlp2.b; p.residual = x.p; p.max_rows = M;
        launch_gemm(p, st);
    }
    launch_layernorm(x.p, xa.p, m->ln_post, M, d, m->ln_eps_outside, st);
}

void Session::run_cross_kv() {
    const wb_dims& D = m->dims;
    const int d = D.n_text_state;
    const float qk_scale = (float)std::pow((double)d / (double)D.n_text_head, -0.25);
    for (int l = 0; l < D.n_text_layer; ++l) {
        const DecBlockW& B = m->dec[(size_t)l];
        if (use_tc) {
            GemmF16Params p;
            p.A_hi = xa_h.p; p.A_lo = xa_l.p; p.lda = d; p.B = B.ckv.w16; p.C = ckv_tmp.p; p.ldc = 2 * d;
            p.N = 2 * d; p.K = d; p.bias = B.ckv.b; p.scale = qk_scale; p.scale_cols = d; p.max_rows = (int)M_tot;
            GemmF16Plan& pl = *enc_plans[(size_t)2 + 4 * D.n_audio_layer + l];
            if (!pl.matches(p.max_rows, 1)) pl.build(p, 0, (int)M_tot);
            pl.launch(st);
        } else {
            GemmParams p;
            p.A = xa.p; p.lda = d; p.B = B.ckv.w32; p.C = ckv_tmp.p; p.ldc = 2 * d;
            p.N = 2 * d; p.K = d; p.bias = B.ckv.b; p.scale = qk_scale; p.scale_cols = d; p.max_rows = (int)M_tot;
            launch_gemm(p, st);
        }
        void* dst = kv_dtype == WB_KV_F16 ? (void*)(ckv16.p + (size_t)l * Mcap * 2 * d) : (void*)(ckv.p + (size_t)l * Mcap * 2 * d);
        launch_ckv_relayout(ckv_tmp.p, dst, kv_dtype == WB_KV_F16, d_win_row_off.p, d_win_T.p, n_windows, M_tot, d, st);
    }
}

void Session::set_special(const uint8_t* sp) {
    if (sp) {
        WB_CUDA(cudaMemcpyAsync(is_special.p, sp, (size_t)m->dims.n_vocab, cudaMemcpyHostToDevice, st));
        WB_CUDA(cudaStreamSynchronize(st));
        have_special = true;
    }
}

void Session::seat_rows(int rows, int per_window, const std::vector<std::vector<int64_t>>& prompts, int max_depth) {
    if (!encoded) fail(WB_ERR_STATE, "session: decode before encode");
    WB_REQUIRE(rows <= Rmax && (int64_t)prompts.size() * per_window >= rows, "decode: rows out of range");
    const int V = m->dims.n_vocab;
    std::vector<int> tk((size_t)rows * t_max, 0), rw((size_t)rows), len((size_t)rows), lim((size_t)rows);
    for (int r = 0; r < rows; ++r) {
        const std::vector<int64_t>& pr = prompts[(size_t)(r / per_window)];
        WB_REQUIRE(!pr.empty() && (int64_t)pr.size() <= t_max, "decode: prompt length out of range");
        rw[(size_t)r] = r / per_window;
        len[(size_t)r] = (int)pr.size();
        lim[(size_t)r] = (int)pr.size() + max_depth;
        for (size_t i = 0; i < pr.size(); ++i) {
            WB_REQUIRE(pr[i] >= 0 && pr[i] < V, "decode: prompt token out of range");
            tk[(size_t)r * t_max + i] = (int)pr[i];
        }
    }
    WB_CUDA(cudaMemcpyAsync(tokens.p, tk.data(), tk.size() * sizeof(int), cudaMemcpyHostToDevice, st));
    WB_CUDA(cudaMemcpyAsync(row_window.p, rw.data(), rw.size() * sizeof(int), cudaMemcpyHostToDevice, st));
    WB_CUDA(cudaMemsetAsync(finished.p, 0, sizeof(int) * Rmax, st));
    WB_CUDA(cudaMemsetAsync(pos.p, 0, sizeof(int), st));
    WB_CUDA(cudaMemcpyAsync(lengths.p, len.data(), len.size() * sizeof(int), cudaMemcpyHostToDevice, st));
    WB_CUDA(cudaMemcpyAsync(lengths.p + Rmax, lim.data(), lim.size() * sizeof(int), cudaMemcpyHostToDevice, st));
    R = rows;
    anc_identity = true;
    anc_cur = 0;
    host_pos = 0;
}

void Session::feed_positions(int n, float* logits_out) {
    const size_t V = (size_t)m->dims.n_vocab;
    const StepLogits out = logits_out ? StepLogits::topk_and_raw : StepLogits::none;
    for (int p = 0; p < n; ++p, ++host_pos) {
        WB_CUDA(cudaMemcpy2DAsync(cur_tok.p, sizeof(int), tokens.p + p, t_max * sizeof(int), sizeof(int), R, cudaMemcpyDeviceToDevice, st));
        launch_decoder(DecodeLaunch::cached_step(R, host_pos, out, MASK_NONE, 1));
        if (logits_out)
            WB_CUDA(cudaMemcpy2DAsync(logits_out + p * V, n * V * sizeof(float), logits.p, V * sizeof(float), V * sizeof(float), R,
                                      cudaMemcpyDeviceToHost, st));
    }
}

static std::pair<int, int> prompt_range(const std::vector<std::vector<int64_t>>& prompts) {
    int lo = INT_MAX, hi = 0;
    for (const auto& pr : prompts) { lo = std::min(lo, (int)pr.size()); hi = std::max(hi, (int)pr.size()); }
    return {lo, hi};
}

void Session::begin(const std::vector<std::vector<int64_t>>& prompts, bool prefill, int max_depth) {
    WB_REQUIRE((int64_t)prompts.size() == n_windows, "begin: one prompt per encoded window");
    for (const auto& pr : prompts) WB_REQUIRE(!pr.empty() && (int64_t)pr.size() < t_max, "begin: prompt length out of range");
    seat_rows(n_windows, 1, prompts, max_depth);
    if (prefill) feed_positions(prompt_range(prompts).first - 1, nullptr);
    WB_CUDA(cudaStreamSynchronize(st));
}

void Session::teacher_forced_logits(const int64_t* toks, int64_t n_rows, int64_t seq_len, float* logits_out) {
    WB_REQUIRE(n_rows >= 1 && seq_len >= 1, "forward_decoder: empty input");
    std::vector<std::vector<int64_t>> rows((size_t)n_rows);
    for (int64_t r = 0; r < n_rows; ++r) rows[(size_t)r].assign(toks + r * seq_len, toks + (r + 1) * seq_len);
    seat_rows((int)n_rows, 1, rows);
    feed_positions((int)seq_len, logits_out);
    WB_CUDA(cudaStreamSynchronize(st));
}

bool Session::launch_decoder(const DecodeLaunch& l) {
    DecArgs a = dec_base;
    a.R = l.rows;
    a.lg_slices = std::max(1, std::min(16, n_sm / std::max(1, l.rows)));
    a.n_splits = std::max(1, std::min(16, n_sm / std::max(1, l.rows * a.H)));
    a.anc = anc_identity ? nullptr : (anc_cur == 0 ? anc0.p : anc1.p);
    a.use_cur_tok = l.use_cur_tok; a.pos0 = l.pos0; a.n_steps = l.n_steps; a.logits_from = l.logits_from;
    a.is_special = have_special ? is_special.p : nullptr; a.mask_mode = l.mask_mode;
    a.k = l.k; a.greedy = l.greedy; a.eot = l.eot; a.loop_rules = l.loop_rules; a.max_depth = l.max_depth;
    a.logits_out = l.raw_logits ? logits.p : nullptr;
    if (getenv("WB200_TRACE")) {
        dec_trace.ensure(1 << 16);
        WB_CUDA(cudaMemsetAsync(dec_trace.p, 0, sizeof(unsigned long long) * (1 << 16), st));
        a.trace = dec_trace.p;
        a.trace_cap = 1 << 16;
    }
    WB_CUDA(cudaMemsetAsync(dec_bar.p, 0, 4 * sizeof(unsigned int), st));
    const bool h16 = m->fp16_exact;
    auto allowed = [&](int n) { return only_decoder == 0 || only_decoder == n; };
    int groups = 0;
    last_groups = 1;
    if (l.beam > 1) {
        a.beam = l.beam; a.n_win = l.rows / l.beam;
        a.anc = anc0.p; a.anc_alt = anc1.p; a.slot_live = slot_live.p;
        a.bm_head = bm_head.p; a.bm_seq = bm_seq.p; a.bm_cnt = bm_cnt.p; a.bm_win = bm_win.p; a.bm_out = bm_out.p; a.bm_out_len = bm_out_len.p;
        a.bm_seq_lp = bm_seq_lp.p; a.bm_out_lp = bm_out_lp.p;
        if (!allowed(6) || !launch_dec6(a, *m, d6, st)) return false;
        last_decoder = 6;
    } else if (allowed(4) && launch_dec4(a, h16, st)) last_decoder = 4;
    else if (allowed(6) && launch_dec6(a, *m, d6, st)) last_decoder = 6;
    else if (allowed(5) && (groups = launch_dec5(a, d5, n_sm, h16, st)) > 0) { last_decoder = 5; last_groups = groups; }
    else if (allowed(3)) { launch_dec3(a, n_sm, h16, st); last_decoder = 3; }
    else fail(WB_ERR_UNSUPPORTED, "WB200_DECODER=" + std::to_string(only_decoder) + ": decoder" + std::to_string(only_decoder) + " does not cover this launch");
    last_rows = l.rows;
    last_k = l.k;
    if (a.trace) {
        std::vector<unsigned long long> h(1 << 16);
        WB_CUDA(cudaStreamSynchronize(st));
        WB_CUDA(cudaMemcpy(h.data(), dec_trace.p, h.size() * sizeof(unsigned long long), cudaMemcpyDeviceToHost));
        FILE* f = fopen(getenv("WB200_TRACE"), "w");
        if (f) {
            for (size_t i = 0; i < h.size(); ++i)
                if (h[i]) fprintf(f, "%llu\n", h[i]);
            fclose(f);
        }
    }
    return true;
}

void Session::profile_decode(const int64_t* prompt, int64_t prompt_len, int n_steps, float* logits_ms, float* step_ms) {
    WB_REQUIRE(n_steps >= 1 && prompt_len + n_steps <= t_max, "profile: n_steps out of range");
    begin(std::vector<std::vector<int64_t>>((size_t)n_windows, std::vector<int64_t>(prompt, prompt + prompt_len)), false, n_steps);
    const int total = (int)prompt_len - 1 + n_steps;
    WB_CUDA(cudaEventRecord(ev[4], st));
    launch_decoder(DecodeLaunch::greedy_search(R, (int)prompt_len, (int)prompt_len, n_steps, -1, false));
    WB_CUDA(cudaEventRecord(ev[5], st));
    WB_CUDA(cudaStreamSynchronize(st));
    float t = 0.f;
    WB_CUDA(cudaEventElapsedTime(&t, ev[4], ev[5]));
    *logits_ms = t / (float)total;
    *step_ms = t / (float)total;
}

void Session::step_beams(int64_t n_rows, const int32_t* window_of_row, const int32_t* parent_row, const int64_t* token,
                         int apply_mask, int k, int64_t* topk_ids_out, float* topk_lp_out) {
    if (!encoded) fail(WB_ERR_STATE, "session: step before encode/begin");
    WB_REQUIRE(n_rows >= 1 && n_rows <= Rmax, "step: n_rows out of range");
    WB_REQUIRE(k >= 1 && k <= DEC_KC - 1, "step: k must be in [1, 7]");
    WB_REQUIRE(host_pos + 1 < t_max, "step: session max_text_len exceeded");
    const int V = m->dims.n_vocab;
    for (int64_t r = 0; r < n_rows; ++r) {
        WB_REQUIRE(parent_row[r] >= 0 && parent_row[r] < R, "step: parent_row out of range");
        WB_REQUIRE(window_of_row[r] >= 0 && window_of_row[r] < n_windows, "step: window_of_row out of range");
        WB_REQUIRE(token[r] >= 0 && token[r] < V, "step: token out of range");
        h_parent[r] = parent_row[r];
        h_window[r] = window_of_row[r];
        h_token[r] = (int)token[r];
    }
    WB_CUDA(cudaMemcpyAsync(parent.p, h_parent.get(), sizeof(int) * n_rows, cudaMemcpyHostToDevice, st));
    WB_CUDA(cudaMemcpyAsync(row_window.p, h_window.get(), sizeof(int) * n_rows, cudaMemcpyHostToDevice, st));
    WB_CUDA(cudaMemcpyAsync(cur_tok.p, h_token.get(), sizeof(int) * n_rows, cudaMemcpyHostToDevice, st));
    if (anc_identity) {
        launch_dec_anc_identity(anc0.p, Rmax, t_max, st);
        anc_cur = 0;
        anc_identity = false;
    }
    {
        int* cur = anc_cur == 0 ? anc0.p : anc1.p;
        int* nxt = anc_cur == 0 ? anc1.p : anc0.p;
        R = (int)n_rows;
        launch_dec_reorder(cur, nxt, parent.p, pos.p, R, t_max, st);
        anc_cur ^= 1;
    }
    launch_decoder(DecodeLaunch::cached_step(R, host_pos, StepLogits::topk, apply_mask ? MASK_ALWAYS : MASK_NONE, k));
    ++host_pos;
    WB_CUDA(cudaMemcpyAsync(h_topk_id.get(), topk_id.p, sizeof(int) * n_rows * k, cudaMemcpyDeviceToHost, st));
    WB_CUDA(cudaMemcpyAsync(topk_lp_out, topk_lp.p, sizeof(float) * n_rows * k, cudaMemcpyDeviceToHost, st));
    WB_CUDA(cudaStreamSynchronize(st));
    for (int64_t i = 0; i < n_rows * k; ++i) topk_ids_out[i] = h_topk_id[i];
}

void Session::last_topk(int64_t n_rows, int64_t k, int64_t* ids_out, float* lp_out) {
    if (last_decoder == 0) fail(WB_ERR_STATE, "last_topk: no decoder launch yet");
    WB_REQUIRE(k == last_k, "last_topk: k differs from the last launch's k");
    WB_REQUIRE(n_rows >= 1 && n_rows <= last_rows, "last_topk: n_rows exceeds the last launch's rows");
    std::vector<int> ids((size_t)(n_rows * k));
    WB_CUDA(cudaStreamSynchronize(st));
    WB_CUDA(cudaMemcpy(ids.data(), topk_id.p, ids.size() * sizeof(int), cudaMemcpyDeviceToHost));
    WB_CUDA(cudaMemcpy(lp_out, topk_lp.p, ids.size() * sizeof(float), cudaMemcpyDeviceToHost));
    for (size_t i = 0; i < ids.size(); ++i) ids_out[i] = ids[i];
}

void Session::greedy_decode(const std::vector<std::vector<int64_t>>& prompts, int max_depth, int64_t eot,
                            std::vector<std::vector<int64_t>>& out, std::vector<std::vector<float>>& out_lp, bool loop_rules) {
    const auto [min_lp, max_lp] = prompt_range(prompts);
    WB_REQUIRE(max_lp + max_depth <= t_max, "greedy: prompt + max_depth exceeds the session's max_text_len");
    begin(prompts, false, max_depth);
    if (max_depth > 0) launch_decoder(DecodeLaunch::greedy_search(R, min_lp, max_lp, max_depth, (int)eot, loop_rules));
    std::vector<int> tk((size_t)R * t_max), len((size_t)R);
    std::vector<float> lp((size_t)R * t_max);
    int sdv[128] = {0};
    WB_CUDA(cudaMemcpyAsync(tk.data(), tokens.p, tk.size() * sizeof(int), cudaMemcpyDeviceToHost, st));
    WB_CUDA(cudaMemcpyAsync(lp.data(), token_lp.p, lp.size() * sizeof(float), cudaMemcpyDeviceToHost, st));
    WB_CUDA(cudaMemcpyAsync(len.data(), lengths.p, len.size() * sizeof(int), cudaMemcpyDeviceToHost, st));
    if (max_depth > 0) WB_CUDA(cudaMemcpyAsync(sdv, steps_done.p, sizeof(int) * std::min(last_groups, 128), cudaMemcpyDeviceToHost, st));
    WB_CUDA(cudaStreamSynchronize(st));
    int sd = 0;
    for (int g = 0; g < std::min(last_groups, 128); ++g) sd = std::max(sd, sdv[g]);
    last_steps = max_depth > 0 ? sd - (min_lp - 1) : 0;
    host_pos = min_lp - 1 + (int)last_steps;
    out.assign((size_t)R, {});
    out_lp.assign((size_t)R, {});
    for (int r = 0; r < R; ++r) {
        const int64_t prompt_len = (int64_t)prompts[(size_t)r].size();
        for (int i = 0; i < len[(size_t)r]; ++i) {
            out[(size_t)r].push_back(tk[(size_t)r * t_max + i]);
            out_lp[(size_t)r].push_back(i < prompt_len ? 0.0f : lp[(size_t)r * t_max + i]);
        }
        if (loop_rules && max_depth > 0 && len[(size_t)r] <= prompt_len) out_lp[(size_t)r].back() = std::nanf("");
        if (loop_rules && out[(size_t)r].back() != eot) {
            out[(size_t)r].push_back(eot);
            out_lp[(size_t)r].push_back(std::nanf(""));
        }
    }
}

bool Session::beam_decode(const std::vector<std::vector<int64_t>>& prompts, int beam_size, int max_depth, int64_t eot,
                          std::vector<std::vector<int64_t>>& out, std::vector<std::vector<float>>& out_lp) {
    namespace fx = beamfx;
    const auto [min_lp, max_lp] = prompt_range(prompts);
    WB_REQUIRE(min_lp >= 1 && max_lp + max_depth <= t_max, "beam: prompt + max_depth exceeds the session's max_text_len");
    const int B = beam_size, W = n_windows, Rb = W * B;
    if (B < 2 || B > fx::MAX_BEAM || max_depth < 1 || Rb > Rmax) return false;
    seat_rows(Rb, B, prompts, max_depth);
    constexpr int MN = fx::MAX_NODES;
    slot_live.ensure((size_t)Rmax);
    bm_head.ensure((size_t)2 * W * MN); bm_seq.ensure((size_t)2 * W * MN * t_max); bm_seq_lp.ensure((size_t)2 * W * MN * t_max);
    bm_cnt.ensure((size_t)2 * W); bm_win.ensure((size_t)2 * W);
    bm_out.ensure((size_t)W * t_max); bm_out_lp.ensure((size_t)W * t_max); bm_out_len.ensure((size_t)W);
    std::vector<int> live((size_t)Rb);
    for (int r = 0; r < Rb; ++r) live[(size_t)r] = r % B == 0 ? 1 : 0;
    std::vector<fx::Head> heads((size_t)W * MN, fx::Head{0.0, 0, 0, 0, 0});
    std::vector<int> seq((size_t)W * MN * t_max, 0), cnt((size_t)2 * W, 0), win((size_t)2 * W, 0);
    for (int w = 0; w < W; ++w) {
        const std::vector<int64_t>& pr = prompts[(size_t)w];
        heads[(size_t)w * MN] = fx::Head{0.0, pr.back() == eot ? 1 : 0, w * B, (int)pr.size(), 0};
        for (size_t i = 0; i < pr.size(); ++i) seq[(size_t)w * MN * t_max + i] = (int)pr[i];
        cnt[(size_t)w] = 1;
    }
    WB_CUDA(cudaMemcpyAsync(slot_live.p, live.data(), live.size() * sizeof(int), cudaMemcpyHostToDevice, st));
    WB_CUDA(cudaMemcpyAsync(bm_head.p, heads.data(), heads.size() * sizeof(fx::Head), cudaMemcpyHostToDevice, st));
    WB_CUDA(cudaMemcpyAsync(bm_seq.p, seq.data(), seq.size() * sizeof(int), cudaMemcpyHostToDevice, st));
    WB_CUDA(cudaMemsetAsync(bm_seq_lp.p, 0, seq.size() * sizeof(float), st));
    WB_CUDA(cudaMemcpyAsync(bm_cnt.p, cnt.data(), cnt.size() * sizeof(int), cudaMemcpyHostToDevice, st));
    WB_CUDA(cudaMemcpyAsync(bm_win.p, win.data(), win.size() * sizeof(int), cudaMemcpyHostToDevice, st));
    launch_dec_anc_identity(anc0.p, Rb, t_max, st);
    const bool ran = launch_decoder(DecodeLaunch::beam_search(Rb, B, min_lp, max_lp, max_depth, (int)eot));
    std::vector<int> res((size_t)W * t_max), res_len((size_t)W);
    std::vector<float> res_lp((size_t)W * t_max);
    int sd = 0;
    if (ran) {
        WB_CUDA(cudaMemcpyAsync(res.data(), bm_out.p, res.size() * sizeof(int), cudaMemcpyDeviceToHost, st));
        WB_CUDA(cudaMemcpyAsync(res_lp.data(), bm_out_lp.p, res_lp.size() * sizeof(float), cudaMemcpyDeviceToHost, st));
        WB_CUDA(cudaMemcpyAsync(res_len.data(), bm_out_len.p, res_len.size() * sizeof(int), cudaMemcpyDeviceToHost, st));
        WB_CUDA(cudaMemcpyAsync(&sd, steps_done.p, sizeof(int), cudaMemcpyDeviceToHost, st));
    }
    WB_CUDA(cudaStreamSynchronize(st));
    if (!ran) return false;
    last_steps = sd;
    host_pos = min_lp - 1 + sd;
    anc_identity = false;
    anc_cur = (sd - 1) & 1;
    out.assign((size_t)W, {});
    out_lp.assign((size_t)W, {});
    for (int w = 0; w < W; ++w)
        for (int i = 0; i < res_len[(size_t)w]; ++i) {
            out[(size_t)w].push_back(res[(size_t)w * t_max + i]);
            out_lp[(size_t)w].push_back(res_lp[(size_t)w * t_max + i]);
        }
    return true;
}

}
```

### whisper-burn_b200/csrc/session.h

```cpp
#pragma once
#include <climits>
#include <memory>
#include <vector>

#include "decoder.h"
#include "wb_internal.h"

namespace wb {

constexpr int MEL_PADDING = 10;

int window_mel_frames(int n_audio_ctx, int window_mode);
int64_t window_samples(int n_audio_ctx, int window_mode);

enum class StepLogits { none, topk, topk_and_raw };

struct DecodeLaunch {
    int rows = 0, pos0 = 0, n_steps = 1, logits_from = INT_MAX;
    bool use_cur_tok = false, raw_logits = false;
    int mask_mode = MASK_NONE, k = 1, eot = -1;
    bool greedy = false, loop_rules = false;
    int beam = 0, max_depth = 0;

    static DecodeLaunch cached_step(int rows, int pos, StepLogits out, int mask_mode, int k) {
        DecodeLaunch l;
        l.rows = rows; l.pos0 = pos; l.use_cur_tok = true; l.mask_mode = mask_mode; l.k = k;
        l.logits_from = out == StepLogits::none ? INT_MAX : 0; l.raw_logits = out == StepLogits::topk_and_raw;
        return l;
    }
    static DecodeLaunch greedy_search(int rows, int min_lp, int max_lp, int max_depth, int eot, bool loop_rules) {
        DecodeLaunch l;
        l.rows = rows; l.n_steps = max_lp - 1 + max_depth; l.logits_from = min_lp - 1; l.eot = eot; l.max_depth = max_depth;
        l.greedy = true; l.loop_rules = loop_rules; l.mask_mode = loop_rules ? MASK_NONE : MASK_SHORT;
        return l;
    }
    static DecodeLaunch beam_search(int rows, int beam, int min_lp, int max_lp, int max_depth, int eot) {
        DecodeLaunch l = greedy_search(rows, min_lp, max_lp, max_depth, eot, false);
        l.greedy = false; l.k = l.beam = beam;
        return l;
    }
};

struct ScoreWs {
    DevBuf<int> tok, pos, target, seq_win, tile_i, am;
    DevBuf<uint8_t> row_mask, special;
    DevBuf<AttnWindow> seqs;
    DevBuf<float> x, tile_m, tile_s, tgt_logit, lp;
    DevBuf<__half> xn_h, xn_l, qkv_h, qkv_l, att_h, att_l, hid_h, hid_l;
    std::vector<std::unique_ptr<GemmF16Plan>> plans;
};

struct PinnedFree { void operator()(void* p) const { cudaFreeHost(p); } };
template <typename T> using Pinned = std::unique_ptr<T[], PinnedFree>;
template <typename T> Pinned<T> pinned(size_t n) { void* p = nullptr; WB_CUDA(cudaMallocHost(&p, n * sizeof(T))); return Pinned<T>((T*)p); }

struct Session {
    Model* m = nullptr;
    cudaStream_t st = nullptr;
    int max_windows = 0, max_beams = 0, t_max = 0, kv_dtype = WB_KV_F32;
    int window_mode = WB_WINDOWS_REFERENCE;
    int search = WB_SEARCH_BEAM;
    int64_t startofprev = -1;
    int mel_limit = 0;
    int Rmax = 0;
    int TmS = 0;
    int Tcap = 0;
    int64_t Mcap = 0;

    int n_windows = 0;
    std::vector<int> win_Tm, win_T;
    std::vector<int64_t> win_row_off;
    int64_t M_tot = 0;
    int max_T = 0, max_Tm = 0;
    bool encoded = false;

    DevBuf<LogMelWindow> d_lmwin;
    DevBuf<GemmGroup> d_g1, d_g2;
    DevBuf<AttnWindow> d_awin;
    DevBuf<int64_t> d_win_row_off;
    DevBuf<int> d_win_T;
    DevBuf<float> wave;
    DevBuf<int> max_slots;
    DevBuf<float> mel_rows, x, xa;
    DevBuf<float> h1, xn, att, qkv, hid;
    DevBuf<__half> mel_h, mel_l, h1_h, h1_l, xn_h, xn_l, qkv_h, qkv_l, att_h, att_l, hid_h, hid_l, xa_h, xa_l;
    std::vector<std::unique_ptr<GemmF16Plan>> enc_plans;
    bool use_tc = true;
    void run_encoder_f16();
    void run_encoder_f32();
    DevBuf<float> ckv;
    DevBuf<float> ckv_tmp;
    DevBuf<float> kc, vc;
    DevBuf<__half> kc16, vc16, ckv16;
    DevBuf<float> dx, dq, dhid, logits;
    Dec5Tables d5;
    DevBuf<uint4> att_pl, hid_pl;
    DevBuf<float> part_o, part_m, part_l;
    DevBuf<int> tokens, lengths, cur_tok, finished, row_window, anc0, anc1, parent, pos, n_unfinished, topk_id;
    DevBuf<float> topk_lp;
    DevBuf<float> token_lp;
    DevBuf<float> eot_logit;
    DevBuf<uint8_t> is_special;
    bool have_special = false;
    int anc_cur = 0;
    bool anc_identity = true;
    int R = 0;
    int host_pos = 0;
    Pinned<int> h_parent, h_window, h_token, h_topk_id;
    cudaEvent_t ev[6] = {};
    float last_ms[4] = {0, 0, 0, 0};
    int64_t last_steps = 0;
    int last_groups = 1;
    int last_decoder = 0;
    int last_rows = 0, last_k = 0;
    int only_decoder = 0;
    int n_sm = 0;
    DevBuf<DecLayer> dec_layers;
    Dec6Pack d6;
    DevBuf<unsigned int> dec_bar;
    DevBuf<int> steps_done;
    DevBuf<float> datt;
    DevBuf<unsigned long long> dec_trace;
    DecArgs dec_base;
    bool launch_decoder(const DecodeLaunch& l);
    DevBuf<int> slot_live, bm_seq, bm_cnt, bm_win, bm_out, bm_out_len;
    DevBuf<float> bm_seq_lp, bm_out_lp;
    DevBuf<beamfx::Head> bm_head;
    DevBuf<float> ypart, lg_m, lg_s, lg_v;
    DevBuf<int> lg_i;
    void profile_decode(const int64_t* prompt, int64_t prompt_len, int n_steps, float* logits_ms, float* step_ms);

    Session(Model* model, int64_t max_windows, int64_t max_beams, int64_t max_text_len, int kv_dtype,
            int window_mode = WB_WINDOWS_REFERENCE);
    ~Session();
    Session(const Session&) = delete;
    Session& operator=(const Session&) = delete;

    void encode_from_device_wave(const float* wave_dev, const int64_t* offsets, const int64_t* lens, int64_t n);
    void encode_waveforms_host(const float* const* waves, const int64_t* lens, int64_t n);
    void encode_mels_host(const float* mel, int64_t n, int64_t n_mels, int64_t n_ctx);
    void load_encoder_output_host(const float* xa_host, int64_t n, int64_t T);
    void run_encoder();
    void run_cross_kv();

    void set_search(int rule) {
        WB_REQUIRE(rule == WB_SEARCH_BEAM || rule == WB_SEARCH_GREEDY_LOOP, "set_search: unknown search rule");
        search = rule;
    }
    void set_prev_prompt(int64_t id) {
        WB_REQUIRE(id == -1 || (id >= 0 && id < m->dims.n_vocab), "set_prev_prompt: startofprev must be -1 or an id in [0, n_vocab)");
        startofprev = id;
    }
    void set_special(const uint8_t* is_special_host);
    void seat_rows(int rows, int per_window, const std::vector<std::vector<int64_t>>& prompts, int max_depth = 0);
    void feed_positions(int n, float* logits_out);
    void begin(const std::vector<std::vector<int64_t>>& prompts, bool prefill = true, int max_depth = 0);
    void teacher_forced_logits(const int64_t* tokens, int64_t n_rows, int64_t seq_len, float* logits_out);
    void step_beams(int64_t n_rows, const int32_t* window_of_row, const int32_t* parent_row, const int64_t* token,
                    int apply_mask, int k, int64_t* topk_ids_out, float* topk_lp_out);
    void last_topk(int64_t n_rows, int64_t k, int64_t* ids_out, float* lp_out);
    void greedy_decode(const std::vector<std::vector<int64_t>>& prompts, int max_depth, int64_t eot,
                       std::vector<std::vector<int64_t>>& out, std::vector<std::vector<float>>& out_lp, bool loop_rules = false);
    bool beam_decode(const std::vector<std::vector<int64_t>>& prompts, int beam_size, int max_depth, int64_t eot,
                     std::vector<std::vector<int64_t>>& out, std::vector<std::vector<float>>& out_lp);
    void score_tokens(int64_t n_seqs, const int32_t* window_of_seq, const int64_t* tokens, const int64_t* lens, bool apply_mask,
                      const uint8_t* is_special_host, float* lp_out, int64_t* argmax_out);
    ScoreWs score_ws;
};

void transcribe_windows(Session& s, int beam_size, int max_depth, const wb_special_ids& ids,
                        const uint8_t* is_special, std::vector<std::vector<int64_t>>& out,
                        std::vector<std::vector<float>>& out_lp,
                        const std::vector<std::vector<int64_t>>& prev = {}, int64_t startofprev = -1);
std::vector<std::pair<int64_t, int64_t>> window_bounds(int64_t n_samples, int64_t sample_rate, int64_t window_len);
bool find_chunk_overlap(const int64_t* prev, int64_t n_prev, const int64_t* curr, int64_t n_curr, int64_t max_n_offsets,
                        int64_t min_n_overlaps, int64_t* prev_index, int64_t* curr_index);

void load_wav(const std::string& path, bool strict, std::vector<float>& out, int64_t& sample_rate, int& channels);

void npy_tree_probe(const std::string& dir, wb_dims& dims);
void npy_tree_load(Model& m, const std::string& dir);

void model_set_tensor(Model& m, const char* path, const float* data, const int64_t* shape, int ndim);
void model_finalize(Model& m);
const std::string& last_error_string();

}
```

### whisper-burn_b200/csrc/wb_internal.h

```cpp
#pragma once

#include <cuda_fp16.h>
#include <cuda_runtime.h>
#include <stdint.h>

#include <algorithm>
#include <cstdio>
#include <cstdlib>
#include <map>
#include <mutex>
#include <stdexcept>
#include <string>
#include <vector>

#include "../../include/whisper_b200.h"

namespace wb {

struct Error : std::runtime_error {
    int code;
    Error(int c, const std::string& m) : std::runtime_error(m), code(c) {}
};
void set_last_error(const std::string& m);
[[noreturn]] void fail(int code, const std::string& m);

#define WB_CUDA(expr)                                                                           \
    do {                                                                                        \
        cudaError_t _e = (expr);                                                                \
        if (_e != cudaSuccess)                                                                  \
            ::wb::fail(_e == cudaErrorMemoryAllocation ? WB_ERR_OOM : WB_ERR_CUDA,              \
                       std::string(#expr) + ": " + cudaGetErrorString(_e) + " (" + __FILE__ + ":" + \
                           std::to_string(__LINE__) + ")");                                     \
    } while (0)

#define WB_REQUIRE(cond, msg)                                   \
    do {                                                        \
        if (!(cond)) ::wb::fail(WB_ERR_INVALID_ARG, (msg));     \
    } while (0)

extern thread_local int64_t g_launch_count;
#define WB_LAUNCH_CHECK()                     \
    do {                                      \
        ++::wb::g_launch_count;               \
        WB_CUDA(cudaPeekAtLastError());       \
    } while (0)

struct PerDeviceConfig {
    std::mutex mu;
    size_t value[16] = {};
    template <typename F>
    bool ensure(size_t want, F&& configure) {
        int dev = 0;
        if (cudaGetDevice(&dev) != cudaSuccess || dev < 0 || dev >= 16) return configure();
        std::lock_guard<std::mutex> lock(mu);
        if (value[dev] == want) return true;
        if (!configure()) return false;
        value[dev] = want;
        return true;
    }
};

struct ClusterLaunch {
    std::mutex mu;
    int clusters[16] = {};
    bool plain[16] = {};
    static cudaLaunchConfig_t config(int cs, int n_clusters, int threads, size_t smem, cudaStream_t st, cudaLaunchAttribute (&attr)[2]) {
        cudaLaunchConfig_t cfg{};
        cfg.gridDim = dim3(n_clusters * cs);
        cfg.blockDim = dim3(threads);
        cfg.dynamicSmemBytes = smem;
        cfg.stream = st;
        attr[0].id = cudaLaunchAttributeClusterDimension;
        attr[0].val.clusterDim.x = cs;
        attr[0].val.clusterDim.y = 1;
        attr[0].val.clusterDim.z = 1;
        attr[1].id = cudaLaunchAttributeCooperative;
        attr[1].val.cooperative = 1;
        cfg.attrs = attr;
        cfg.numAttrs = 1;
        return cfg;
    }
    int capacity(const void* k, int cs, int threads, size_t smem, const char* name) {
        int dev = 0;
        WB_CUDA(cudaGetDevice(&dev));
        if (dev < 0 || dev >= 16) return 0;
        std::lock_guard<std::mutex> lock(mu);
        if (clusters[dev] == 0) {
            clusters[dev] = -1;
            if (cudaFuncSetAttribute(k, cudaFuncAttributeMaxDynamicSharedMemorySize, (int)smem) != cudaSuccess ||
                (cs > 8 && cudaFuncSetAttribute(k, cudaFuncAttributeNonPortableClusterSizeAllowed, 1) != cudaSuccess)) {
                cudaGetLastError();
                return 0;
            }
            cudaLaunchAttribute attr[2];
            const cudaLaunchConfig_t cfg = config(cs, 1, threads, smem, nullptr, attr);
            int n = 0;
            const cudaError_t e = cudaOccupancyMaxActiveClusters(&n, k, &cfg);
            if (getenv("WB200_VERBOSE")) fprintf(stderr, "[wb] %s: cluster %d, smem %zu B, max active clusters %d (%s)\n", name, cs, smem, n, cudaGetErrorString(e));
            if (e != cudaSuccess || n < 1) {
                cudaGetLastError();
                return 0;
            }
            clusters[dev] = n;
            plain[dev] = getenv("WB200_NO_COOP") != nullptr;
        }
        return std::max(clusters[dev], 0);
    }
    void launch(const void* k, int cs, int n_clusters, int threads, size_t smem, void** args, cudaStream_t st, const char* name) {
        int dev = 0;
        WB_CUDA(cudaGetDevice(&dev));
        std::lock_guard<std::mutex> lock(mu);
        cudaLaunchAttribute attr[2];
        cudaLaunchConfig_t cfg = config(cs, n_clusters, threads, smem, st, attr);
        if (!plain[dev]) {
            cfg.numAttrs = 2;
            const cudaError_t e = cudaLaunchKernelExC(&cfg, k, args);
            if (e == cudaSuccess) {
                WB_LAUNCH_CHECK();
                return;
            }
            cudaGetLastError();
            plain[dev] = true;
            cfg.numAttrs = 1;
            if (getenv("WB200_VERBOSE")) fprintf(stderr, "[wb] %s: cooperative cluster launch rejected (%s), using a plain cluster launch\n", name, cudaGetErrorString(e));
        }
        WB_CUDA(cudaLaunchKernelExC(&cfg, k, args));
        WB_LAUNCH_CHECK();
    }
};

template <typename T>
struct DevBuf {
    T* p = nullptr;
    size_t n = 0;
    DevBuf() = default;
    DevBuf(const DevBuf&) = delete;
    DevBuf& operator=(const DevBuf&) = delete;
    ~DevBuf() { release(); }
    void release() {
        if (p) cudaFree(p);
        p = nullptr;
        n = 0;
    }
    void alloc(size_t count) {
        release();
        if (count == 0) return;
        WB_CUDA(cudaMalloc((void**)&p, count * sizeof(T)));
        n = count;
    }
    void ensure(size_t count) {
        if (count > n) alloc(count);
    }
    void zero(cudaStream_t st) {
        if (p) WB_CUDA(cudaMemsetAsync(p, 0, n * sizeof(T), st));
    }
};

constexpr int N_FFT = 400, HOP = 160, N_MELS = 80, N_FREQ = 201;
constexpr int KPAD = 208;
struct FrontendTables {
    std::vector<float> hann;
    std::vector<float> basis_t;
    std::vector<float> mel_filt;
    int mel_lo[N_MELS], mel_hi[N_MELS];
};
const FrontendTables& frontend_tables();

struct LinearW {
    float* w32 = nullptr;
    __half* w16 = nullptr;
    float* b = nullptr;
    int n = 0, k = 0;
};
struct LayerNormW {
    float* g = nullptr;
    float* b = nullptr;
    float eps = 1e-5f;
};
struct EncBlockW {
    LayerNormW attn_ln, mlp_ln;
    LinearW qkv;
    LinearW out, mlp1, mlp2;
};
struct DecBlockW {
    LayerNormW attn_ln, cross_ln, mlp_ln;
    LinearW qkv;
    LinearW out;
    LinearW cq;
    LinearW ckv;
    LinearW cout, mlp1, mlp2;
};

struct Model {
    wb_dims dims{};
    int device = 0;
    bool finalized = false;
    bool fp16_exact = false;
    int ln_eps_outside = 1;
    std::map<std::string, std::pair<std::vector<int64_t>, std::vector<float>>> host;

    std::vector<void*> allocs;
    float* basis_t = nullptr;
    float* mel_filt = nullptr;
    int* mel_range = nullptr;
    LinearW conv1;
    LinearW conv2;
    float* enc_pos = nullptr;
    std::vector<EncBlockW> enc;
    LayerNormW ln_post;
    float* tok_emb32 = nullptr;
    __half* tok_emb16 = nullptr;
    __half* tok_emb16_tiled = nullptr;
    float* dec_pos = nullptr;
    std::vector<DecBlockW> dec;
    LayerNormW dec_ln;
    float* zero_bias = nullptr;

    ~Model();
};

struct GemmGroup {
    int64_t a_off;
    int64_t c_off;
    int rows;
};
enum { ACT_NONE = 0, ACT_GELU = 1 };
struct GemmParams {
    const float* A = nullptr;
    int64_t lda = 0;
    const float* B = nullptr;
    float* C = nullptr;
    int64_t ldc = 0;
    int N = 0, K = 0;
    const float* bias = nullptr;
    int act = ACT_NONE;
    float scale = 1.0f;
    int scale_cols = 0;
    const float* residual = nullptr;
    const float* pos = nullptr;
    const GemmGroup* groups = nullptr;
    int n_groups = 1;
    int max_rows = 0;
};
void launch_gemm(const GemmParams& p, cudaStream_t st);

struct GemmF16Params {
    const __half *A_hi = nullptr, *A_lo = nullptr;
    int64_t lda = 0;
    const __half* B = nullptr;
    float* C = nullptr;
    __half *P_hi = nullptr, *P_lo = nullptr;
    int64_t ldc = 0;
    int N = 0, K = 0;
    const float* bias = nullptr;
    int act = ACT_NONE;
    float scale = 1.0f;
    int scale_cols = 0;
    const float* residual = nullptr;
    const float* pos = nullptr;
    const GemmGroup* groups = nullptr;
    int n_groups = 1;
    int max_rows = 0;
};
bool gemm_f16_supported(const GemmF16Params& p);
class GemmF16Plan {
public:
    GemmF16Plan();
    ~GemmF16Plan();
    GemmF16Plan(const GemmF16Plan&) = delete;
    GemmF16Plan& operator=(const GemmF16Plan&) = delete;
    void build(const GemmF16Params& p, int64_t a_group_stride, int a_rows_total_per_group);
    void launch(cudaStream_t st) const;
    bool matches(int max_rows, int n_groups) const { return impl != nullptr && key_rows == max_rows && key_groups == n_groups; }
private:
    struct Impl;
    Impl* impl = nullptr;
    int key_rows = -1, key_groups = -1;
};
void launch_split_f16(const float* src, __half* hi, __half* lo, int64_t n, cudaStream_t st);
struct LogitStatsParams {
    const __half *A_hi = nullptr, *A_lo = nullptr;
    const __half* E = nullptr;
    int rows = 0, K = 0, V = 0;
    const int* target = nullptr;
    const uint8_t* row_mask = nullptr;
    const uint8_t* is_special = nullptr;
    float *tile_m = nullptr, *tile_s = nullptr, *tgt_logit = nullptr;
    int* tile_i = nullptr;
};
int logit_stats_tiles(int V);
void launch_logit_stats(const LogitStatsParams& p, cudaStream_t st);

struct LogMelWindow {
    int64_t wave_off;
    int n_samples;
    int n_frames;
    int n_store;
    int max_slot;
    int64_t out_off;
};
void launch_logmel(const Model& m, const float* wave, const LogMelWindow* win_dev, int n_windows,
                   int max_frames, float* mel_rows, int* max_slots, int n_slots, cudaStream_t st);
void launch_rows_to_chan(const float* rows, float* chan, int n_frames, cudaStream_t st);
void launch_chan_to_rows(const float* chan, float* rows, int n_frames, int64_t chan_stride, cudaStream_t st);

void launch_ckv_relayout(const float* src, void* dst, bool dst_half, const int64_t* win_row_off, const int* win_T, int n_windows,
                         int64_t M, int d, cudaStream_t st);
void launch_layernorm(const float* x, float* y, const LayerNormW& ln, int rows, int d, int eps_outside, cudaStream_t st);
struct AttnWindow {
    int64_t row_off;
    int T;
};
void launch_encoder_attention(const float* qkv, float* out, const AttnWindow* win_dev, int n_windows, int max_T, int d, int n_head,
                              cudaStream_t st);
void launch_encoder_attention_tc(const __half* qkv_hi, const __half* qkv_lo, __half* out_hi, __half* out_lo, const AttnWindow* win_dev,
                                 int n_windows, int max_T, int d, int n_head, cudaStream_t st);
void launch_causal_attention_tc(const __half* qkv_hi, const __half* qkv_lo, __half* out_hi, __half* out_lo, const AttnWindow* seq_dev,
                                int n_seqs, int max_T, int d, int n_head, bool kv_f16, cudaStream_t st);
void launch_cross_attention_tc(const __half* q_hi, const __half* q_lo, const void* ckv_layer, bool kv_f16, __half* out_hi, __half* out_lo,
                               const AttnWindow* seq_dev, const int* seq_win_dev, const int64_t* win_row_off_dev, const int* win_T_dev,
                               int n_seqs, int max_T, int d, int n_head, cudaStream_t st);
void launch_layernorm_f16(const float* x, float* y, __half* y_hi, __half* y_lo, const LayerNormW& ln, int rows, int d, int eps_outside,
                          cudaStream_t st);

}
```

### whisper-burn_b200/ffi.py

```python
from __future__ import annotations

import ctypes as C
import os
from pathlib import Path

_HERE = Path(__file__).resolve().parent


class WbError(RuntimeError):
    def __init__(self, code: int, msg: str):
        super().__init__(f"[wb status {code}] {msg}")
        self.code = code
        self.msg = msg


WB_OK, WB_ERR_INVALID_ARG, WB_ERR_CUDA, WB_ERR_OOM, WB_ERR_STATE, WB_ERR_UNSUPPORTED = range(6)
WB_KV_F32, WB_KV_F16 = 0, 1
WB_WINDOWS_REFERENCE, WB_WINDOWS_NATIVE = 0, 1
WB_SEARCH_BEAM, WB_SEARCH_GREEDY_LOOP = 0, 1


class Dims(C.Structure):
    _fields_ = [(n, C.c_int32) for n in (
        "n_mels", "n_audio_ctx", "n_audio_state", "n_audio_head", "n_audio_layer",
        "n_vocab", "n_text_ctx", "n_text_state", "n_text_head", "n_text_layer")]


class SpecialIds(C.Structure):
    _fields_ = [(n, C.c_int64) for n in ("sot", "lang", "transcribe", "notimestamps", "eot")]


def library_path() -> Path:
    return Path(os.environ.get("WB200_LIB", _HERE / "libwhisper_b200.so"))


_P = C.c_void_p
_F = C.POINTER(C.c_float)
_I64 = C.POINTER(C.c_int64)
_I32 = C.POINTER(C.c_int32)
_U8 = C.POINTER(C.c_uint8)
SYMBOLS = {
    "wb_version": (C.c_char_p, []),
    "wb_last_error": (C.c_char_p, []),
    "wb_device_count": (C.c_int, [C.POINTER(C.c_int)]),
    "wb_max_waveform_samples": (C.c_int64, [C.c_int64]),
    "wb_window_samples": (C.c_int64, [C.c_int64, C.c_int]),
    "wb_prep_audio": (C.c_int, [C.c_int, _F, C.c_int64, C.c_int64, _F, _I64]),
    "wb_prep_audio_dev": (C.c_int, [C.c_int, _P, C.c_int64, C.c_int64, _P, _I64]),
    "wb_model_create": (C.c_int, [C.POINTER(Dims), C.c_int, C.POINTER(_P)]),
    "wb_model_set_tensor": (C.c_int, [_P, C.c_char_p, _F, _I64, C.c_int]),
    "wb_npy_tree_probe": (C.c_int, [C.c_char_p, C.POINTER(Dims)]),
    "wb_model_load_npy_tree": (C.c_int, [C.c_char_p, C.c_int, C.c_int, C.POINTER(_P)]),
    "wb_model_set_layernorm_eps_mode": (C.c_int, [_P, C.c_int]),
    "wb_model_finalize": (C.c_int, [_P]),
    "wb_model_destroy": (None, [_P]),
    "wb_model_get_dims": (C.c_int, [_P, C.POINTER(Dims)]),
    "wb_model_weights_fp16_exact": (C.c_int, [_P]),
    "wb_forward_encoder": (C.c_int, [_P, _F, C.c_int64, C.c_int64, C.c_int64, _F]),
    "wb_forward_decoder": (C.c_int, [_P, _I64, C.c_int64, C.c_int64, _F, C.c_int64, _F]),
    "wb_session_create": (C.c_int, [_P, C.c_int64, C.c_int64, C.c_int64, C.c_int, C.POINTER(_P)]),
    "wb_session_create_windows": (C.c_int, [_P, C.c_int64, C.c_int64, C.c_int64, C.c_int, C.c_int, C.POINTER(_P)]),
    "wb_session_destroy": (None, [_P]),
    "wb_session_set_search": (C.c_int, [_P, C.c_int]),
    "wb_session_set_prev_prompt": (C.c_int, [_P, C.c_int64]),
    "wb_session_encode_waveforms": (C.c_int, [_P, C.POINTER(_F), _I64, C.c_int64]),
    "wb_session_encode_waveforms_dev": (C.c_int, [_P, _P, _I64, _I64, C.c_int64]),
    "wb_session_encode_mels": (C.c_int, [_P, _F, C.c_int64, C.c_int64, C.c_int64]),
    "wb_session_get_mel": (C.c_int, [_P, C.c_int64, _F, C.c_int64, _I64]),
    "wb_session_get_encoder_output": (C.c_int, [_P, C.c_int64, _F, C.c_int64, _I64]),
    "wb_session_begin": (C.c_int, [_P, _I64, C.c_int64]),
    "wb_session_step": (C.c_int, [_P, C.c_int64, _I32, _I32, _I64, C.c_int, _U8, C.c_int, _I64, _F]),
    "wb_transcribe_windows": (C.c_int, [_P, C.POINTER(_F), _I64, C.c_int64, C.c_int, C.c_int,
                                        C.POINTER(SpecialIds), _U8, _I64, C.c_int64, _I64]),
    "wb_transcribe_windows_dev": (C.c_int, [_P, _P, _I64, _I64, C.c_int64, C.c_int, C.c_int,
                                            C.POINTER(SpecialIds), _U8, _I64, C.c_int64, _I64]),
    "wb_transcribe_windows_prev": (C.c_int, [_P, C.POINTER(_F), _I64, C.c_int64, _I64, _I64, C.c_int64, C.c_int, C.c_int,
                                             C.POINTER(SpecialIds), _U8, _I64, C.c_int64, _I64]),
    "wb_waveform_to_tokens": (C.c_int, [_P, _F, C.c_int64, C.c_int64, C.c_int, C.c_int,
                                        C.POINTER(SpecialIds), _U8, _I64, C.c_int64, _I64]),
    "wb_waveforms_to_tokens": (C.c_int, [_P, C.POINTER(C.c_void_p), _I64, C.c_int64, C.c_int64, C.c_int, C.c_int,
                                         C.POINTER(SpecialIds), _U8, _I64, C.c_int64, _I64]),
    "wb_session_last_logprobs": (C.c_int, [_P, C.c_int64, _F, C.c_int64, _I64]),
    "wb_session_score_tokens": (C.c_int, [_P, C.c_int64, _I32, _I64, _I64, C.c_int, _U8, _F, _I64]),
    "wb_session_last_decoder": (C.c_int, [_P]),
    "wb_session_last_topk": (C.c_int, [_P, C.c_int64, C.c_int64, _I64, _F]),
    "wb_beam_search_table": (C.c_int64, [C.POINTER(C.c_double), C.c_int64, C.c_int64, C.c_int64, C.c_int64, C.c_int64, C.c_int64, _I64, C.c_int64]),
    "wb_beam_search_table_fixed": (C.c_int64, [C.POINTER(C.c_double), C.c_int64, C.c_int64, C.c_int64, C.c_int64, C.c_int64, C.c_int64, _I64, C.c_int64]),
    "wb_load_wav": (C.c_int, [C.c_char_p, C.c_int, _F, C.c_int64, _I64, _I64, C.POINTER(C.c_int)]),
    "wb_window_count": (C.c_int64, [C.c_int64, C.c_int64, C.c_int64]),
    "wb_window_bounds": (C.c_int, [C.c_int64, C.c_int64, C.c_int64, _I64, _I64]),
    "wb_find_chunk_overlap": (C.c_int, [_I64, C.c_int64, _I64, C.c_int64, C.c_int64, C.c_int64, _I64, _I64]),
    "wb_first_repetition_end": (C.c_int64, [_I64, C.c_int64, C.c_int64]),
    "wb_repetition_period": (C.c_int64, [_I64, C.c_int64, C.c_int64]),
    "wb_find_repeated_tokens_index": (C.c_int, [_I64, C.c_int64, C.c_int64, C.c_int64, _I64, _I64]),
    "wb_beam_get_top_elements": (C.c_int64, [C.POINTER(C.c_double), C.c_int64, C.c_int64, _I64]),
    "wb_kernel_launch_count": (C.c_int64, []),
    "wb_kernel_launch_count_reset": (None, []),
    "wb_session_last_timings": (C.c_int, [_P, _F]),
    "wb_session_last_steps": (C.c_int, [_P, _I64]),
    "wb_session_profile_decode": (C.c_int, [_P, C.POINTER(SpecialIds), C.c_int, _F, _F]),
}

_lib = None


def lib() -> C.CDLL:
    global _lib
    if _lib is None:
        path = library_path()
        if not path.exists():
            raise WbError(WB_ERR_STATE, f"{path} not built: run `python -c 'import __graft_entry__ as g; g.build()'` "
                                        f"or `make -C whisper-burn_b200/csrc` (there is no CPU fallback)")
        handle = C.CDLL(str(path))
        for name, (res, args) in SYMBOLS.items():
            fn = getattr(handle, name)
            fn.restype = res
            fn.argtypes = args
        _lib = handle
    return _lib


def check(status: int) -> None:
    if status != WB_OK:
        raise WbError(status, (lib().wb_last_error() or b"").decode("utf-8", "replace"))


def fptr(a):
    return a.ctypes.data_as(_F)


def i64ptr(a):
    return a.ctypes.data_as(_I64)


def i32ptr(a):
    return a.ctypes.data_as(_I32)


def u8ptr(a):
    return a.ctypes.data_as(_U8)
```

### whisper-burn_b200/transcribe.py

```python
from __future__ import annotations

import ctypes as C
from typing import List, Optional, Sequence

import numpy as np

from . import ffi
from .model import Whisper


WINDOW_MODES = {"reference": ffi.WB_WINDOWS_REFERENCE, "native": ffi.WB_WINDOWS_NATIVE}
SEARCH_RULES = {"beam": ffi.WB_SEARCH_BEAM, "greedy_loop": ffi.WB_SEARCH_GREEDY_LOOP}


def window_samples(n_audio_ctx: int, mode: str = "reference") -> int:
    n = int(ffi.lib().wb_window_samples(n_audio_ctx, WINDOW_MODES[mode]))
    if n < 0:
        raise ValueError(f"window_samples: n_audio_ctx {n_audio_ctx} out of range")
    return n


def _special(is_special: Optional[np.ndarray]):
    return None if is_special is None else ffi.u8ptr(np.ascontiguousarray(is_special, dtype=np.uint8))


class Session:

    def __init__(self, whisper: Whisper, max_windows: int, max_beams: int = 5, max_text_len: int = 104,
                 kv_dtype: int = ffi.WB_KV_F32, windows: str = "reference", search: str = "beam"):
        if windows not in WINDOW_MODES:
            raise ValueError(f"windows must be one of {sorted(WINDOW_MODES)}, not {windows!r}")
        if search not in SEARCH_RULES:
            raise ValueError(f"search must be one of {sorted(SEARCH_RULES)}, not {search!r}")
        self.whisper = whisper
        self.max_windows = max_windows
        self.windows = windows
        n_ctx = whisper.config.n_audio_ctx
        self.max_mel_frames = 2 * n_ctx if windows == "native" else n_ctx
        self._h = C.c_void_p()
        ffi.check(ffi.lib().wb_session_create_windows(whisper.handle, max_windows, max_beams, max_text_len, kv_dtype,
                                                      WINDOW_MODES[windows], C.byref(self._h)))
        self.search = search
        ffi.check(ffi.lib().wb_session_set_search(self._h, SEARCH_RULES[search]))

    def close(self):
        if getattr(self, "_h", None):
            ffi.lib().wb_session_destroy(self._h)
            self._h = None

    def __del__(self):
        try:
            self.close()
        except Exception:
            pass

    def set_prev_prompt(self, startofprev: int) -> None:
        ffi.check(ffi.lib().wb_session_set_prev_prompt(self._h, startofprev))

    def encode_waveforms(self, waves: Sequence[np.ndarray]) -> None:
        ws = [np.ascontiguousarray(w, dtype=np.float32) for w in waves]
        ptrs = (ffi._F * len(ws))(*[ffi.fptr(w) for w in ws])
        lens = np.asarray([w.shape[0] for w in ws], dtype=np.int64)
        ffi.check(ffi.lib().wb_session_encode_waveforms(self._h, ptrs, ffi.i64ptr(lens), len(ws)))

    def encode_mels(self, mels: np.ndarray) -> None:
        mels = np.ascontiguousarray(mels, dtype=np.float32)
        n, n_mels, n_ctx = mels.shape
        ffi.check(ffi.lib().wb_session_encode_mels(self._h, ffi.fptr(mels), n, n_mels, n_ctx))

    def get_mel(self, window: int) -> np.ndarray:
        cap = 80 * self.max_mel_frames
        buf = np.empty(cap, dtype=np.float32)
        n = C.c_int64(0)
        ffi.check(ffi.lib().wb_session_get_mel(self._h, window, ffi.fptr(buf), cap, C.byref(n)))
        return buf[:80 * n.value].reshape(80, n.value).copy()

    def get_encoder_output(self, window: int) -> np.ndarray:
        d = self.whisper.config.n_audio_state
        cap = d * ((self.max_mel_frames - 1) // 2 + 1)
        buf = np.empty(cap, dtype=np.float32)
        n = C.c_int64(0)
        ffi.check(ffi.lib().wb_session_get_encoder_output(self._h, window, ffi.fptr(buf), cap, C.byref(n)))
        return buf[:d * n.value].reshape(n.value, d).copy()

    def begin(self, prompt: Sequence[int]) -> None:
        p = np.asarray(prompt, dtype=np.int64)
        ffi.check(ffi.lib().wb_session_begin(self._h, ffi.i64ptr(p), len(p)))

    def step(self, window_of_row, parent_row, token, apply_special_mask: bool, is_special: Optional[np.ndarray], k: int):
        w = np.asarray(window_of_row, dtype=np.int32)
        pr = np.asarray(parent_row, dtype=np.int32)
        tk = np.asarray(token, dtype=np.int64)
        n = len(w)
        ids = np.empty((n, k), dtype=np.int64)
        lps = np.empty((n, k), dtype=np.float32)
        sp = ffi.u8ptr(np.ascontiguousarray(is_special, dtype=np.uint8)) if is_special is not None else None
        ffi.check(ffi.lib().wb_session_step(self._h, n, ffi.i32ptr(w), ffi.i32ptr(pr), ffi.i64ptr(tk),
                                           1 if apply_special_mask else 0, sp, k, ffi.i64ptr(ids), ffi.fptr(lps)))
        return ids, lps

    def transcribe_windows(self, waves: Sequence[np.ndarray], special, is_special: np.ndarray, beam_size: int = 5,
                           max_depth: int = 100) -> List[List[int]]:
        ws = [np.ascontiguousarray(w, dtype=np.float32) for w in waves]
        ptrs = (ffi._F * len(ws))(*[ffi.fptr(w) for w in ws])
        lens = np.asarray([w.shape[0] for w in ws], dtype=np.int64)
        cap = 4 + max_depth + 1
        out = np.zeros((len(ws), cap), dtype=np.int64)
        out_len = np.zeros(len(ws), dtype=np.int64)
        ids = ffi.SpecialIds(special.sot, special.lang, special.transcribe, special.notimestamps, special.eot)
        sp = _special(is_special)
        ffi.check(ffi.lib().wb_transcribe_windows(self._h, ptrs, ffi.i64ptr(lens), len(ws), beam_size, max_depth,
                                                 C.byref(ids), sp, ffi.i64ptr(out), cap, ffi.i64ptr(out_len)))
        return [[int(t) for t in out[i, :out_len[i]]] for i in range(len(ws))]

    def transcribe_windows_prev(self, waves: Sequence[np.ndarray], prev: Sequence[Sequence[int]], special,
                                is_special: Optional[np.ndarray], beam_size: int = 5, max_depth: int = 100,
                                startofprev: Optional[int] = None) -> List[List[int]]:
        ws = [np.ascontiguousarray(w, dtype=np.float32) for w in waves]
        if len(prev) != len(ws):
            raise ValueError(f"transcribe_windows_prev: {len(ws)} windows but {len(prev)} previous-id lists")
        ptrs = (ffi._F * len(ws))(*[ffi.fptr(w) for w in ws])
        lens = np.asarray([w.shape[0] for w in ws], dtype=np.int64)
        prev_lens = np.asarray([len(p) for p in prev], dtype=np.int64)
        prev_toks = np.ascontiguousarray(np.concatenate([np.asarray(p, dtype=np.int64) for p in prev] + [np.zeros(1, np.int64)]))
        cap = max([4] + [len(p) + 5 for p in prev if len(p)]) + max_depth + 1
        out = np.zeros((len(ws), cap), dtype=np.int64)
        out_len = np.zeros(len(ws), dtype=np.int64)
        ids = ffi.SpecialIds(special.sot, special.lang, special.transcribe, special.notimestamps, special.eot)
        sop = special.startofprev if startofprev is None else startofprev
        ffi.check(ffi.lib().wb_transcribe_windows_prev(self._h, ptrs, ffi.i64ptr(lens), len(ws), ffi.i64ptr(prev_toks),
                                                      ffi.i64ptr(prev_lens), sop, beam_size, max_depth, C.byref(ids),
                                                      _special(is_special), ffi.i64ptr(out), cap, ffi.i64ptr(out_len)))
        return [[int(t) for t in out[i, :out_len[i]]] for i in range(len(ws))]

    def transcribe_windows_dev(self, wave_dev_ptr: int, offsets, lens, special, is_special: np.ndarray,
                               beam_size: int = 5, max_depth: int = 100) -> List[List[int]]:
        offs = np.asarray(offsets, dtype=np.int64)
        ln = np.asarray(lens, dtype=np.int64)
        cap = 4 + max_depth + 1
        out = np.zeros((len(ln), cap), dtype=np.int64)
        out_len = np.zeros(len(ln), dtype=np.int64)
        ids = ffi.SpecialIds(special.sot, special.lang, special.transcribe, special.notimestamps, special.eot)
        sp = _special(is_special)
        ffi.check(ffi.lib().wb_transcribe_windows_dev(self._h, C.c_void_p(wave_dev_ptr), ffi.i64ptr(offs), ffi.i64ptr(ln),
                                                     len(ln), beam_size, max_depth, C.byref(ids), sp,
                                                     ffi.i64ptr(out), cap, ffi.i64ptr(out_len)))
        return [[int(t) for t in out[i, :out_len[i]]] for i in range(len(ln))]

    def waveform_to_tokens(self, waveform: np.ndarray, special, is_special: np.ndarray, sample_rate: int = 16000,
                           beam_size: int = 5, max_depth: int = 100) -> List[int]:
        w = np.ascontiguousarray(waveform, dtype=np.float32)
        cap = (len(w) // 1000 + 2) * (10 + max_depth + 1) + 16
        out = np.zeros(cap, dtype=np.int64)
        n = C.c_int64(0)
        ids = ffi.SpecialIds(special.sot, special.lang, special.transcribe, special.notimestamps, special.eot)
        sp = _special(is_special)
        ffi.check(ffi.lib().wb_waveform_to_tokens(self._h, ffi.fptr(w), len(w), sample_rate, beam_size, max_depth,
                                                 C.byref(ids), sp, ffi.i64ptr(out), cap, C.byref(n)))
        return [int(t) for t in out[:n.value]]

    def waveforms_to_tokens(self, waveforms: Sequence[np.ndarray], special, is_special: np.ndarray, sample_rate: int = 16000,
                            beam_size: int = 5, max_depth: int = 100) -> List[List[int]]:
        ws = [np.ascontiguousarray(w, dtype=np.float32) for w in waveforms]
        cap = (max(len(w) for w in ws) // 1000 + 2) * (10 + max_depth + 1) + 16
        out = np.zeros((len(ws), cap), dtype=np.int64)
        n = np.zeros(len(ws), dtype=np.int64)
        ptrs = (C.c_void_p * len(ws))(*[w.ctypes.data for w in ws])
        lens = np.array([len(w) for w in ws], dtype=np.int64)
        ids = ffi.SpecialIds(special.sot, special.lang, special.transcribe, special.notimestamps, special.eot)
        sp = _special(is_special)
        ffi.check(ffi.lib().wb_waveforms_to_tokens(self._h, ptrs, ffi.i64ptr(lens), len(ws), sample_rate, beam_size, max_depth,
                                                  C.byref(ids), sp, ffi.i64ptr(out), cap, ffi.i64ptr(n)))
        return [[int(t) for t in out[i, :n[i]]] for i in range(len(ws))]

    def last_logprobs(self, index: int) -> np.ndarray:
        n = C.c_int64(0)
        ffi.check(ffi.lib().wb_session_last_logprobs(self._h, index, None, 0, C.byref(n)))
        out = np.empty(n.value, dtype=np.float32)
        ffi.check(ffi.lib().wb_session_last_logprobs(self._h, index, ffi.fptr(out), n.value, C.byref(n)))
        return out

    def score_tokens(self, seqs: Sequence[Sequence[int]], windows: Sequence[int], apply_special_mask: bool = False,
                     is_special: Optional[np.ndarray] = None):
        lens = np.asarray([len(s) for s in seqs], dtype=np.int64)
        toks = np.ascontiguousarray(np.concatenate([np.asarray(s, dtype=np.int64) for s in seqs]) if len(seqs)
                                    else np.zeros(0, dtype=np.int64), dtype=np.int64)
        win = np.ascontiguousarray(windows, dtype=np.int32)
        if len(win) != len(lens):
            raise ValueError(f"score_tokens: {len(lens)} sequences but {len(win)} windows")
        lp = np.empty(max(len(toks), 1), dtype=np.float32)
        am = np.empty(max(len(toks), 1), dtype=np.int64)
        ffi.check(ffi.lib().wb_session_score_tokens(self._h, len(lens), ffi.i32ptr(win), ffi.i64ptr(toks), ffi.i64ptr(lens),
                                                   1 if apply_special_mask else 0, _special(is_special), ffi.fptr(lp),
                                                   ffi.i64ptr(am)))
        offs = np.concatenate([[0], np.cumsum(lens)])
        return [(lp[offs[i]:offs[i + 1]].copy(), am[offs[i]:offs[i + 1]].copy()) for i in range(len(lens))]

    def last_decoder(self) -> int:
        return int(ffi.lib().wb_session_last_decoder(self._h))

    def last_topk(self, n_rows: int, k: int = 1):
        ids = np.empty((n_rows, k), dtype=np.int64)
        lps = np.empty((n_rows, k), dtype=np.float32)
        ffi.check(ffi.lib().wb_session_last_topk(self._h, n_rows, k, ffi.i64ptr(ids), ffi.fptr(lps)))
        return ids, lps

    def last_timings_ms(self):
        buf = np.zeros(4, dtype=np.float32)
        ffi.check(ffi.lib().wb_session_last_timings(self._h, ffi.fptr(buf)))
        return {"logmel": float(buf[0]), "encoder": float(buf[1]), "decode": float(buf[2]), "total": float(buf[3])}

    def profile_decode(self, special, n_steps: int = 50):
        ids = ffi.SpecialIds(special.sot, special.lang, special.transcribe, special.notimestamps, special.eot)
        a, b = C.c_float(0), C.c_float(0)
        ffi.check(ffi.lib().wb_session_profile_decode(self._h, C.byref(ids), n_steps, C.byref(a), C.byref(b)))
        return float(a.value), float(b.value)

    def last_steps(self) -> int:
        n = C.c_int64(0)
        ffi.check(ffi.lib().wb_session_last_steps(self._h, C.byref(n)))
        return int(n.value)


def waveform_to_text(whisper: Whisper, special, is_special: np.ndarray, waveform: np.ndarray, sample_rate: int = 16000,
                     beam_size: int = 5, max_depth: int = 100, max_windows: int = 8) -> List[int]:
    s = Session(whisper, max_windows=max_windows, max_beams=max(beam_size, 1), max_text_len=4 + max_depth + 1)
    try:
        return s.waveform_to_tokens(waveform, special, is_special, sample_rate, beam_size, max_depth)
    finally:
        s.close()


def window_bounds(n_samples: int, sample_rate: int, window_len: int):
    n = int(ffi.lib().wb_window_count(n_samples, sample_rate, window_len))
    st = np.zeros(n, dtype=np.int64)
    en = np.zeros(n, dtype=np.int64)
    ffi.check(ffi.lib().wb_window_bounds(n_samples, sample_rate, window_len, ffi.i64ptr(st), ffi.i64ptr(en)))
    return [(int(a), int(b)) for a, b in zip(st, en)]


def find_chunk_overlap(prev_tokens, curr_tokens, max_n_offsets: int, min_n_overlaps: int):
    p = np.asarray(prev_tokens, dtype=np.int64)
    c = np.asarray(curr_tokens, dtype=np.int64)
    pi, ci = C.c_int64(0), C.c_int64(0)
    found = ffi.lib().wb_find_chunk_overlap(ffi.i64ptr(p), len(p), ffi.i64ptr(c), len(c), max_n_offsets, min_n_overlaps,
                                            C.byref(pi), C.byref(ci))
    return (pi.value, ci.value) if found else None


def first_repetition_end(tokens, period: int) -> int:
    t = np.asarray(tokens, dtype=np.int64)
    r = int(ffi.lib().wb_first_repetition_end(ffi.i64ptr(t), len(t), period))
    if r < 0:
        raise ValueError("first_repetition_end: period exceeds the token count")
    return r


def repetition_period(tokens, min_repetitions: int):
    t = np.asarray(tokens, dtype=np.int64)
    r = int(ffi.lib().wb_repetition_period(ffi.i64ptr(t), len(t), min_repetitions))
    if r < 0:
        raise ValueError("repetition_period: invalid argument")
    return r if r > 0 else None


def find_repeated_tokens_index(tokens, window_size: int, min_repeat_count: int):
    t = np.asarray(tokens, dtype=np.int64)
    a, b = C.c_int64(0), C.c_int64(0)
    r = int(ffi.lib().wb_find_repeated_tokens_index(ffi.i64ptr(t), len(t), window_size, min_repeat_count, C.byref(a), C.byref(b)))
    if r < 0:
        raise ValueError("find_repeated_tokens_index: the reference unwraps a repeat that does not exist")
    return (a.value, b.value) if r else None
```

Baseline: 2647.

## Fuse all decoder cross-K/V projections into one GEMM writing cache layout directly

Concatenates the cross-attention K/V weights of every decoder layer into a single fp16 linear, so one grouped GEMM produces every layer's cross K/V. A custom epilogue scatters results straight into the swizzled per-window cross-KV cache, replacing per-layer GEMMs plus a separate relayout pass. Host staging buffers become pinned and reused, set_geometry is skipped when the geometry is unchanged, and several stream synchronizations are replaced by stage events. It also adds debug entry points to read back the cross KV and to recompute it per layer. The risks are index mistakes in the epilogue's window binary search and layout math, and reuse of pinned buffers while a previous copy is still in flight.

```diff
diff --git a/include/whisper_b200.h b/include/whisper_b200.h
--- a/include/whisper_b200.h
+++ b/include/whisper_b200.h
@@ -76,6 +76,8 @@
 int wb_session_encode_mels(wb_session* s, const float* mel, int64_t n_windows, int64_t n_mels, int64_t n_ctx);
 int wb_session_get_mel(wb_session* s, int64_t window, float* mel_out, int64_t capacity, int64_t* n_ctx_out);
 int wb_session_get_encoder_output(wb_session* s, int64_t window, float* out, int64_t capacity, int64_t* n_ctx_out);
+int wb_session_get_cross_kv(wb_session* s, int64_t layer, void* out, int64_t capacity_bytes, int64_t* bytes_out);
+int wb_session_recompute_cross_kv_per_layer(wb_session* s);
 int wb_session_begin(wb_session* s, const int64_t* prompt, int64_t prompt_len);
 int wb_session_step(wb_session* s, int64_t n_rows, const int32_t* window_of_row, const int32_t* parent_row,
                     const int64_t* token, int apply_special_mask, const uint8_t* is_special,
diff --git a/whisper-burn_b200/csrc/api.cu b/whisper-burn_b200/csrc/api.cu
--- a/whisper-burn_b200/csrc/api.cu
+++ b/whisper-burn_b200/csrc/api.cu
@@ -375,11 +375,38 @@
     });
 }
 
+int wb_session_get_cross_kv(wb_session* s, int64_t layer, void* out, int64_t capacity_bytes, int64_t* bytes_out) {
+    return guarded([&] {
+        WB_REQUIRE(s && out && bytes_out, "get_cross_kv: null pointer");
+        wb::Session& S = *s->impl;
+        if (!S.encoded) wb::fail(WB_ERR_STATE, "get_cross_kv: nothing encoded");
+        const int d = S.m->dims.n_text_state;
+        WB_REQUIRE(layer >= 0 && layer < S.m->dims.n_text_layer, "get_cross_kv: layer out of range");
+        const bool half = S.kv_dtype == WB_KV_F16;
+        const size_t elt = half ? sizeof(__half) : sizeof(float), n = (size_t)S.M_tot * 2 * d;
+        WB_REQUIRE(capacity_bytes >= (int64_t)(n * elt), "get_cross_kv: capacity too small");
+        const size_t off = (size_t)layer * S.Mcap * 2 * d;
+        const void* src = half ? (const void*)(S.ckv16.p + off) : (const void*)(S.ckv.p + off);
+        WB_CUDA(cudaStreamSynchronize(S.st));
+        WB_CUDA(cudaMemcpy(out, src, n * elt, cudaMemcpyDeviceToHost));
+        *bytes_out = (int64_t)(n * elt);
+    });
+}
+
+int wb_session_recompute_cross_kv_per_layer(wb_session* s) {
+    return guarded([&] {
+        WB_REQUIRE(s, "recompute_cross_kv_per_layer: null pointer");
+        s->impl->cross_kv_per_layer();
+        WB_CUDA(cudaStreamSynchronize(s->impl->st));
+    });
+}
+
 int wb_session_begin(wb_session* s, const int64_t* prompt, int64_t prompt_len) {
     return guarded([&] {
         WB_REQUIRE(s && prompt, "begin: null pointer");
         WB_REQUIRE(prompt_len >= 1, "begin: prompt length out of range");
         s->impl->begin(std::vector<std::vector<int64_t>>((size_t)s->impl->n_windows, std::vector<int64_t>(prompt, prompt + prompt_len)));
+        WB_CUDA(cudaStreamSynchronize(s->impl->st));
     });
 }
 
diff --git a/whisper-burn_b200/csrc/gemm_f16.cu b/whisper-burn_b200/csrc/gemm_f16.cu
--- a/whisper-burn_b200/csrc/gemm_f16.cu
+++ b/whisper-burn_b200/csrc/gemm_f16.cu
@@ -48,6 +48,14 @@
     float scale;
     int scale_cols;
 };
+struct CkvArgs : F16Args {
+    void* dst;
+    int half;
+    const int64_t* win_row_off;
+    const int* win_T;
+    int n_windows, d;
+    int64_t layer_stride;
+};
 struct LogitArgs : F16Args {
     const int* target;
     const uint8_t* row_mask;
@@ -101,6 +109,45 @@
             g.tile_m[o] = mx;
             g.tile_s[o] = s;
             g.tile_i[o] = ai;
+        }
+    }
+}
+
+template <int BN>
+__device__ __forceinline__ void ckv_epilogue(const float (&acc_h)[BN / 2], const float (&acc_l)[BN / 2], const CkvArgs& g, int rows,
+                                             int m_base, int n0, int lane) {
+#pragma unroll
+    for (int hrow = 0; hrow < 2; ++hrow) {
+        const int m = m_base + 8 * hrow;
+        if (m >= rows) continue;
+        int lo = 0, hi = g.n_windows - 1;
+        while (lo < hi) {
+            const int mid = (lo + hi + 1) >> 1;
+            if (g.win_row_off[mid] <= m) lo = mid; else hi = mid - 1;
+        }
+        const int64_t off = g.win_row_off[lo];
+        const int T = g.win_T[lo];
+        const int j = (int)(m - off);
+#pragma unroll
+        for (int jj = 0; jj < BN / 8; ++jj) {
+            const int n = n0 + 8 * jj + 2 * (lane & 3);
+            const int layer = n / (2 * g.d), c = n - layer * 2 * g.d, which = c >= g.d ? 1 : 0, cc = c - which * g.d;
+            const int h = cc >> 6, e = cc & 63;
+            float v[2];
+#pragma unroll
+            for (int q = 0; q < 2; ++q) {
+                float t = __fadd_rn(hl_join(acc_h[4 * jj + 2 * hrow + q], acc_l[4 * jj + 2 * hrow + q]), __ldg(g.bias + n + q));
+                if (!which) t = __fmul_rn(t, g.scale);
+                v[q] = t;
+            }
+            const int64_t o = layer * g.layer_stride + off * 2 * g.d + (int64_t)h * T * 128 + (int64_t)j * 128 + which * 64;
+            if (g.half) {
+                const int e_phys = (((e >> 3) ^ (4 * (j & 1))) << 3) + (e & 7);
+                *reinterpret_cast<__half2*>(static_cast<__half*>(g.dst) + o + e_phys) = __floats2half2_rn(v[0], v[1]);
+            } else {
+                const int e_phys = (((e >> 2) ^ (4 * (j & 1))) << 2) + (e & 3);
+                *reinterpret_cast<float2*>(static_cast<float*>(g.dst) + o + e_phys) = make_float2(v[0], v[1]);
+            }
         }
     }
 }
@@ -179,6 +226,8 @@
 
     if constexpr (std::is_same<Args, LogitArgs>::value) {
         logit_stats_epilogue<BN>(acc_h, acc_l, g, grp.rows, m0 + wg * 64 + (warp & 3) * 16 + (lane >> 2), n0, lane);
+    } else if constexpr (std::is_same<Args, CkvArgs>::value) {
+        ckv_epilogue<BN>(acc_h, acc_l, g, grp.rows, m0 + wg * 64 + (warp & 3) * 16 + (lane >> 2), n0, lane);
     } else {
 #pragma unroll
         for (int hrow = 0; hrow < 2; ++hrow) {
@@ -284,15 +333,17 @@
 
 struct GemmF16Plan::Impl {
     CUtensorMap ah, al, b;
-    F16Args args;
+    CkvArgs args;
+    bool ckv;
     dim3 grid;
     int BN;
 };
 GemmF16Plan::GemmF16Plan() = default;
 GemmF16Plan::~GemmF16Plan() { delete impl; }
 
-void GemmF16Plan::build(const GemmF16Params& p, int64_t a_group_stride, int a_rows_total_per_group) {
+void GemmF16Plan::build(const GemmF16Params& p, int64_t a_group_stride, int a_rows_total_per_group, const CkvDest* ckv) {
     WB_REQUIRE(gemm_f16_supported(p), "gemm_f16: unsupported shape");
+    WB_REQUIRE(!ckv || (!p.groups && ckv->d % 64 == 0 && p.N % (2 * ckv->d) == 0 && ckv->n_windows >= 1), "gemm_f16: bad cross K/V destination");
     delete impl;
     impl = new Impl();
     const int ng = p.groups ? p.n_groups : 1;
@@ -302,19 +353,28 @@
     impl->al = make_map(p.A_lo, (uint64_t)p.K, rows, (uint64_t)ng, (uint64_t)p.lda, gstride, F_BK, F_BM, 3);
     impl->BN = (p.N % 128 == 0 && (int64_t)(p.N / 128) * ((p.max_rows + F_BM - 1) / F_BM) * ng >= 96) ? 128 : 64;
     impl->b = make_map(p.B, (uint64_t)p.K, (uint64_t)p.N, 1, (uint64_t)p.K, (uint64_t)p.K * p.N, F_BK, (uint32_t)impl->BN, 2);
-    F16Args& a = impl->args;
+    CkvArgs& a = impl->args;
+    impl->ckv = ckv != nullptr;
+    if (ckv) {
+        a.dst = ckv->dst; a.half = ckv->half ? 1 : 0; a.win_row_off = ckv->win_row_off; a.win_T = ckv->win_T;
+        a.n_windows = ckv->n_windows; a.d = ckv->d; a.layer_stride = ckv->layer_stride;
+    }
     a.C = p.C; a.P_hi = p.P_hi; a.P_lo = p.P_lo; a.bias = p.bias; a.residual = p.residual; a.pos = p.pos; a.groups = p.groups;
     a.single = GemmGroup{0, 0, p.max_rows};
     a.ldc = p.ldc; a.N = p.N; a.K = p.K; a.act = p.act; a.scale = p.scale; a.scale_cols = p.scale_cols;
     impl->grid = dim3(p.N / impl->BN, (p.max_rows + F_BM - 1) / F_BM, ng);
     key_rows = p.max_rows;
-    key_groups = ng;
+    key_groups = ckv ? ckv->n_windows : ng;
 }
 
 void GemmF16Plan::launch(cudaStream_t st) const {
     if (!impl || impl->args.single.rows <= 0 || impl->grid.y == 0) return;
-    if (impl->BN == 128) launch_f16_t<128>(impl->ah, impl->al, impl->b, impl->args, impl->grid, st);
-    else launch_f16_t<64>(impl->ah, impl->al, impl->b, impl->args, impl->grid, st);
+    const F16Args& f = impl->args;
+    if (impl->ckv) {
+        if (impl->BN == 128) launch_f16_t<128>(impl->ah, impl->al, impl->b, impl->args, impl->grid, st);
+        else launch_f16_t<64>(impl->ah, impl->al, impl->b, impl->args, impl->grid, st);
+    } else if (impl->BN == 128) launch_f16_t<128>(impl->ah, impl->al, impl->b, f, impl->grid, st);
+    else launch_f16_t<64>(impl->ah, impl->al, impl->b, f, impl->grid, st);
 }
 
 int logit_stats_tiles(int V) { return (V + 127) / 128; }
diff --git a/whisper-burn_b200/csrc/model.cu b/whisper-burn_b200/csrc/model.cu
--- a/whisper-burn_b200/csrc/model.cu
+++ b/whisper-burn_b200/csrc/model.cu
@@ -206,6 +206,7 @@
     }
     m.dec_pos = up32(m, need(m, "decoder/positional_embedding", {D.n_text_ctx, d}).second);
     m.dec.resize(D.n_text_layer);
+    LinSpec ckv_all;
     for (int i = 0; i < D.n_text_layer; ++i) {
         const std::string p = "decoder/block_" + std::to_string(i);
         DecBlockW& B = m.dec[i];
@@ -226,11 +227,16 @@
         B.qkv = upload_linear(m, qkv, h32, h16);
         B.out = upload_linear(m, o, h32, h16);
         B.cq = upload_linear(m, cq, h32, h16);
-        B.ckv = upload_linear(m, ckv, h32, h16);
+        if (h32) B.ckv = upload_linear(m, ckv, true, false);
+        ckv_all.w.insert(ckv_all.w.end(), ckv.w.begin(), ckv.w.end());
+        ckv_all.b.insert(ckv_all.b.end(), ckv.b.begin(), ckv.b.end());
+        ckv_all.n += ckv.n;
+        ckv_all.k = ckv.k;
         B.cout = upload_linear(m, co, h32, h16);
         B.mlp1 = upload_linear(m, m1, h32, h16);
         B.mlp2 = upload_linear(m, m2, h32, h16);
     }
+    if (h16) m.ckv_all = upload_linear(m, ckv_all, false, true);
     m.dec_ln = upload_ln(m, "decoder/ln", d);
     {
         std::vector<float> z((size_t)std::max(4 * d, D.n_vocab), 0.0f);
diff --git a/whisper-burn_b200/csrc/session.cu b/whisper-burn_b200/csrc/session.cu
--- a/whisper-burn_b200/csrc/session.cu
+++ b/whisper-burn_b200/csrc/session.cu
@@ -58,10 +58,11 @@
         xn_h.alloc(Mcap * d); xn_l.alloc(Mcap * d); qkv_h.alloc(Mcap * 3 * d); qkv_l.alloc(Mcap * 3 * d);
         att_h.alloc(Mcap * d); att_l.alloc(Mcap * d); hid_h.alloc(Mcap * 4 * d); hid_l.alloc(Mcap * 4 * d);
         xa_h.alloc(Mcap * d); xa_l.alloc(Mcap * d);
-        enc_plans.resize((size_t)2 + 4 * D.n_audio_layer + L);
+        enc_plans.resize((size_t)3 + 4 * D.n_audio_layer);
         for (auto& pl : enc_plans) pl.reset(new GemmF16Plan());
     } else {
         h1.alloc((size_t)max_windows * TmS * d);
+        ckv_tmp.alloc(Mcap * 2 * d);
         xn.alloc(Mcap * d); att.alloc(Mcap * d); qkv.alloc(Mcap * 3 * d); hid.alloc(Mcap * 4 * d);
     }
     if (kv == WB_KV_F16) { kc16.alloc((size_t)L * Rmax * t_max * d); vc16.alloc((size_t)L * Rmax * t_max * d); }
@@ -79,7 +80,6 @@
     eot_logit.alloc(Rmax);
     is_special.alloc(V);
     {
-        ckv_tmp.alloc(Mcap * 2 * d);
         cudaDeviceProp prop;
         WB_CUDA(cudaGetDeviceProperties(&prop, m->device));
         n_sm = prop.multiProcessorCount;
@@ -110,6 +110,12 @@
     }
     h_parent = pinned<int>(Rmax); h_window = pinned<int>(Rmax); h_token = pinned<int>(Rmax);
     h_topk_id = pinned<int>((size_t)Rmax * DEC_KC);
+    for (auto& e : stage_ev) WB_CUDA(cudaEventCreateWithFlags(&e, cudaEventDisableTiming));
+    h_lmwin = pinned<LogMelWindow>(max_windows); h_g1 = pinned<GemmGroup>(max_windows); h_g2 = pinned<GemmGroup>(max_windows);
+    h_awin = pinned<AttnWindow>(max_windows); h_win_row_off = pinned<int64_t>(max_windows); h_win_T = pinned<int>(max_windows);
+    h_special = pinned<uint8_t>(V);
+    h_seat = pinned<int>((size_t)Rmax * t_max + 3 * Rmax);
+    h_res = pinned<int>((size_t)Rmax * t_max + Rmax + 128); h_res_lp = pinned<float>((size_t)Rmax * t_max);
     WB_CUDA(cudaMemsetAsync(is_special.p, 0, V, st));
 
     DecArgs& a = dec_base;
@@ -136,10 +142,13 @@
     if (st) cudaStreamSynchronize(st);
     for (auto& e : ev)
         if (e) cudaEventDestroy(e);
+    for (auto& e : stage_ev)
+        if (e) cudaEventDestroy(e);
     if (st) cudaStreamDestroy(st);
 }
 
 static void set_geometry(Session& s, const std::vector<int>& Tm) {
+    if (!s.win_Tm.empty() && Tm == s.win_Tm) return;
     s.n_windows = (int)Tm.size();
     s.win_Tm = Tm;
     s.win_T.resize(Tm.size());
@@ -155,25 +164,24 @@
         s.max_Tm = std::max(s.max_Tm, Tm[w]);
     }
     const int d = s.m->dims.n_audio_state;
-    std::vector<GemmGroup> g1(Tm.size()), g2(Tm.size());
-    std::vector<AttnWindow> aw(Tm.size());
     for (size_t w = 0; w < Tm.size(); ++w) {
-        g1[w] = GemmGroup{(int64_t)w * s.TmS * N_MELS, ((int64_t)w * s.TmS + 1) * d, Tm[w]};
-        g2[w] = GemmGroup{(int64_t)w * s.TmS * d, s.win_row_off[w] * d, s.win_T[w]};
-        aw[w] = AttnWindow{s.win_row_off[w], s.win_T[w]};
-    }
-    WB_CUDA(cudaMemcpyAsync(s.d_g1.p, g1.data(), g1.size() * sizeof(GemmGroup), cudaMemcpyHostToDevice, s.st));
-    WB_CUDA(cudaMemcpyAsync(s.d_g2.p, g2.data(), g2.size() * sizeof(GemmGroup), cudaMemcpyHostToDevice, s.st));
-    WB_CUDA(cudaMemcpyAsync(s.d_awin.p, aw.data(), aw.size() * sizeof(AttnWindow), cudaMemcpyHostToDevice, s.st));
-    WB_CUDA(cudaMemcpyAsync(s.d_win_row_off.p, s.win_row_off.data(), Tm.size() * sizeof(int64_t),
-                            cudaMemcpyHostToDevice, s.st));
-    WB_CUDA(cudaMemcpyAsync(s.d_win_T.p, s.win_T.data(), Tm.size() * sizeof(int), cudaMemcpyHostToDevice, s.st));
-    WB_CUDA(cudaStreamSynchronize(s.st));
+        s.h_g1[w] = GemmGroup{(int64_t)w * s.TmS * N_MELS, ((int64_t)w * s.TmS + 1) * d, Tm[w]};
+        s.h_g2[w] = GemmGroup{(int64_t)w * s.TmS * d, s.win_row_off[w] * d, s.win_T[w]};
+        s.h_awin[w] = AttnWindow{s.win_row_off[w], s.win_T[w]};
+        s.h_win_row_off[w] = s.win_row_off[w];
+        s.h_win_T[w] = s.win_T[w];
+    }
+    const size_t n = Tm.size();
+    WB_CUDA(cudaMemcpyAsync(s.d_g1.p, s.h_g1.get(), n * sizeof(GemmGroup), cudaMemcpyHostToDevice, s.st));
+    WB_CUDA(cudaMemcpyAsync(s.d_g2.p, s.h_g2.get(), n * sizeof(GemmGroup), cudaMemcpyHostToDevice, s.st));
+    WB_CUDA(cudaMemcpyAsync(s.d_awin.p, s.h_awin.get(), n * sizeof(AttnWindow), cudaMemcpyHostToDevice, s.st));
+    WB_CUDA(cudaMemcpyAsync(s.d_win_row_off.p, s.h_win_row_off.get(), n * sizeof(int64_t), cudaMemcpyHostToDevice, s.st));
+    WB_CUDA(cudaMemcpyAsync(s.d_win_T.p, s.h_win_T.get(), n * sizeof(int), cudaMemcpyHostToDevice, s.st));
 }
 
 void Session::encode_from_device_wave(const float* wave_dev, const int64_t* offsets, const int64_t* lens, int64_t n) {
     WB_REQUIRE(n >= 1 && n <= max_windows, "encode: n_windows out of range for this session");
-    std::vector<LogMelWindow> lw((size_t)n);
+    stage_wait(STAGE_GEOMETRY);
     std::vector<int> Tm((size_t)n);
     int max_frames = 0;
     for (int64_t w = 0; w < n; ++w) {
@@ -182,11 +190,12 @@
         const int F = (int)(lens[w] / HOP);
         const int keep = std::min(F, mel_limit - MEL_PADDING);
         Tm[(size_t)w] = keep + MEL_PADDING;
-        lw[(size_t)w] = LogMelWindow{offsets[w], (int)lens[w], F, keep, (int)w, ((int64_t)w * TmS + 1) * N_MELS};
+        h_lmwin[w] = LogMelWindow{offsets[w], (int)lens[w], F, keep, (int)w, ((int64_t)w * TmS + 1) * N_MELS};
         max_frames = std::max(max_frames, F);
     }
-    WB_CUDA(cudaMemcpyAsync(d_lmwin.p, lw.data(), lw.size() * sizeof(LogMelWindow), cudaMemcpyHostToDevice, st));
+    WB_CUDA(cudaMemcpyAsync(d_lmwin.p, h_lmwin.get(), (size_t)n * sizeof(LogMelWindow), cudaMemcpyHostToDevice, st));
     set_geometry(*this, Tm);
+    stage_done(STAGE_GEOMETRY);
     WB_CUDA(cudaEventRecord(ev[0], st));
     WB_CUDA(cudaMemsetAsync(mel_rows.p, 0, (size_t)n * TmS * N_MELS * sizeof(float), st));
     launch_logmel(*m, wave_dev, d_lmwin.p, (int)n, max_frames, mel_rows.p, max_slots.p, (int)n, st);
@@ -218,7 +227,9 @@
                                                  "2 * n_audio_ctx in native windowing (mod.rs:236-241)");
     WB_REQUIRE(n >= 1 && n <= max_windows, "encode: n_windows out of range for this session");
     std::vector<int> Tm((size_t)n, (int)n_ctx);
+    stage_wait(STAGE_GEOMETRY);
     set_geometry(*this, Tm);
+    stage_done(STAGE_GEOMETRY);
     DevBuf<float> tmp;
     tmp.alloc((size_t)n * n_mels * n_ctx);
     WB_CUDA(cudaMemcpyAsync(tmp.p, mel, tmp.n * sizeof(float), cudaMemcpyHostToDevice, st));
@@ -232,7 +243,9 @@
 void Session::load_encoder_output_host(const float* xa_host, int64_t n, int64_t T) {
     WB_REQUIRE(n >= 1 && n <= max_windows && T >= 1 && T <= Tcap, "forward_decoder: encoder output shape out of range");
     std::vector<int> Tm((size_t)n, (int)(2 * T - 1));
+    stage_wait(STAGE_GEOMETRY);
     set_geometry(*this, Tm);
+    stage_done(STAGE_GEOMETRY);
     const int d = m->dims.n_audio_state;
     WB_CUDA(cudaMemcpyAsync(xa.p, xa_host, (size_t)n * T * d * sizeof(float), cudaMemcpyHostToDevice, st));
     if (use_tc) launch_split_f16(xa.p, xa_h.p, xa_l.p, (int64_t)n * T * d, st);
@@ -338,39 +351,74 @@
     const wb_dims& D = m->dims;
     const int d = D.n_text_state;
     const float qk_scale = (float)std::pow((double)d / (double)D.n_text_head, -0.25);
+    const bool half = kv_dtype == WB_KV_F16;
+    if (use_tc) {
+        GemmF16Params p;
+        p.A_hi = xa_h.p; p.A_lo = xa_l.p; p.lda = d; p.B = m->ckv_all.w16; p.N = D.n_text_layer * 2 * d; p.K = d;
+        p.bias = m->ckv_all.b; p.scale = qk_scale; p.max_rows = (int)M_tot;
+        GemmF16Plan& pl = *enc_plans[(size_t)2 + 4 * D.n_audio_layer];
+        if (!pl.matches(p.max_rows, n_windows)) {
+            CkvDest c;
+            c.dst = half ? (void*)ckv16.p : (void*)ckv.p; c.half = half;
+            c.win_row_off = d_win_row_off.p; c.win_T = d_win_T.p; c.n_windows = n_windows; c.d = d; c.layer_stride = Mcap * 2 * d;
+            pl.build(p, 0, (int)M_tot, &c);
+        }
+        pl.launch(st);
+        return;
+    }
     for (int l = 0; l < D.n_text_layer; ++l) {
         const DecBlockW& B = m->dec[(size_t)l];
-        if (use_tc) {
-            GemmF16Params p;
-            p.A_hi = xa_h.p; p.A_lo = xa_l.p; p.lda = d; p.B = B.ckv.w16; p.C = ckv_tmp.p; p.ldc = 2 * d;
-            p.N = 2 * d; p.K = d; p.bias = B.ckv.b; p.scale = qk_scale; p.scale_cols = d; p.max_rows = (int)M_tot;
-            GemmF16Plan& pl = *enc_plans[(size_t)2 + 4 * D.n_audio_layer + l];
-            if (!pl.matches(p.max_rows, 1)) pl.build(p, 0, (int)M_tot);
-            pl.launch(st);
-        } else {
-            GemmParams p;
-            p.A = xa.p; p.lda = d; p.B = B.ckv.w32; p.C = ckv_tmp.p; p.ldc = 2 * d;
-            p.N = 2 * d; p.K = d; p.bias = B.ckv.b; p.scale = qk_scale; p.scale_cols = d; p.max_rows = (int)M_tot;
-            launch_gemm(p, st);
-        }
-        void* dst = kv_dtype == WB_KV_F16 ? (void*)(ckv16.p + (size_t)l * Mcap * 2 * d) : (void*)(ckv.p + (size_t)l * Mcap * 2 * d);
-        launch_ckv_relayout(ckv_tmp.p, dst, kv_dtype == WB_KV_F16, d_win_row_off.p, d_win_T.p, n_windows, M_tot, d, st);
+        GemmParams p;
+        p.A = xa.p; p.lda = d; p.B = B.ckv.w32; p.C = ckv_tmp.p; p.ldc = 2 * d;
+        p.N = 2 * d; p.K = d; p.bias = B.ckv.b; p.scale = qk_scale; p.scale_cols = d; p.max_rows = (int)M_tot;
+        launch_gemm(p, st);
+        void* dst = half ? (void*)(ckv16.p + (size_t)l * Mcap * 2 * d) : (void*)(ckv.p + (size_t)l * Mcap * 2 * d);
+        launch_ckv_relayout(ckv_tmp.p, dst, half, d_win_row_off.p, d_win_T.p, n_windows, M_tot, d, st);
+    }
+}
+
+void Session::cross_kv_per_layer() {
+    if (!encoded) fail(WB_ERR_STATE, "recompute_cross_kv_per_layer: nothing encoded");
+    if (!use_tc) fail(WB_ERR_UNSUPPORTED, "recompute_cross_kv_per_layer: the weights are not fp16-exact");
+    const wb_dims& D = m->dims;
+    const int d = D.n_text_state;
+    const float qk_scale = (float)std::pow((double)d / (double)D.n_text_head, -0.25);
+    const bool half = kv_dtype == WB_KV_F16;
+    ckv_tmp.ensure((size_t)Mcap * 2 * d);
+    for (int l = 0; l < D.n_text_layer; ++l) {
+        GemmF16Params p;
+        p.A_hi = xa_h.p; p.A_lo = xa_l.p; p.lda = d; p.B = m->ckv_all.w16 + (size_t)l * 2 * d * d; p.C = ckv_tmp.p; p.ldc = 2 * d;
+        p.N = 2 * d; p.K = d; p.bias = m->ckv_all.b + (size_t)l * 2 * d; p.scale = qk_scale; p.scale_cols = d; p.max_rows = (int)M_tot;
+        GemmF16Plan pl;
+        pl.build(p, 0, (int)M_tot);
+        pl.launch(st);
+        void* dst = half ? (void*)(ckv16.p + (size_t)l * Mcap * 2 * d) : (void*)(ckv.p + (size_t)l * Mcap * 2 * d);
+        launch_ckv_relayout(ckv_tmp.p, dst, half, d_win_row_off.p, d_win_T.p, n_windows, M_tot, d, st);
     }
 }
 
 void Session::set_special(const uint8_t* sp) {
-    if (sp) {
-        WB_CUDA(cudaMemcpyAsync(is_special.p, sp, (size_t)m->dims.n_vocab, cudaMemcpyHostToDevice, st));
-        WB_CUDA(cudaStreamSynchronize(st));
-        have_special = true;
-    }
+    if (!sp) return;
+    const size_t V = (size_t)m->dims.n_vocab;
+    if (have_special && std::memcmp(special_host.data(), sp, V) == 0) return;
+    special_host.assign(sp, sp + V);
+    stage_wait(STAGE_SPECIAL);
+    std::memcpy(h_special.get(), sp, V);
+    WB_CUDA(cudaMemcpyAsync(is_special.p, h_special.get(), V, cudaMemcpyHostToDevice, st));
+    stage_done(STAGE_SPECIAL);
+    have_special = true;
 }
 
 void Session::seat_rows(int rows, int per_window, const std::vector<std::vector<int64_t>>& prompts, int max_depth) {
     if (!encoded) fail(WB_ERR_STATE, "session: decode before encode");
     WB_REQUIRE(rows <= Rmax && (int64_t)prompts.size() * per_window >= rows, "decode: rows out of range");
     const int V = m->dims.n_vocab;
-    std::vector<int> tk((size_t)rows * t_max, 0), rw((size_t)rows), len((size_t)rows), lim((size_t)rows);
+    stage_wait(STAGE_SEAT);
+    int* tk = h_seat.get();
+    int* rw = tk + (size_t)Rmax * t_max;
+    int* len = rw + Rmax;
+    int* lim = len + Rmax;
+    std::memset(tk, 0, (size_t)rows * t_max * sizeof(int));
     for (int r = 0; r < rows; ++r) {
         const std::vector<int64_t>& pr = prompts[(size_t)(r / per_window)];
         WB_REQUIRE(!pr.empty() && (int64_t)pr.size() <= t_max, "decode: prompt length out of range");
@@ -382,12 +430,13 @@
             tk[(size_t)r * t_max + i] = (int)pr[i];
         }
     }
-    WB_CUDA(cudaMemcpyAsync(tokens.p, tk.data(), tk.size() * sizeof(int), cudaMemcpyHostToDevice, st));
-    WB_CUDA(cudaMemcpyAsync(row_window.p, rw.data(), rw.size() * sizeof(int), cudaMemcpyHostToDevice, st));
+    WB_CUDA(cudaMemcpyAsync(tokens.p, tk, (size_t)rows * t_max * sizeof(int), cudaMemcpyHostToDevice, st));
+    WB_CUDA(cudaMemcpyAsync(row_window.p, rw, (size_t)rows * sizeof(int), cudaMemcpyHostToDevice, st));
     WB_CUDA(cudaMemsetAsync(finished.p, 0, sizeof(int) * Rmax, st));
     WB_CUDA(cudaMemsetAsync(pos.p, 0, sizeof(int), st));
-    WB_CUDA(cudaMemcpyAsync(lengths.p, len.data(), len.size() * sizeof(int), cudaMemcpyHostToDevice, st));
-    WB_CUDA(cudaMemcpyAsync(lengths.p + Rmax, lim.data(), lim.size() * sizeof(int), cudaMemcpyHostToDevice, st));
+    WB_CUDA(cudaMemcpyAsync(lengths.p, len, (size_t)rows * sizeof(int), cudaMemcpyHostToDevice, st));
+    WB_CUDA(cudaMemcpyAsync(lengths.p + Rmax, lim, (size_t)rows * sizeof(int), cudaMemcpyHostToDevice, st));
+    stage_done(STAGE_SEAT);
     R = rows;
     anc_identity = true;
     anc_cur = 0;
@@ -417,7 +466,6 @@
     for (const auto& pr : prompts) WB_REQUIRE(!pr.empty() && (int64_t)pr.size() < t_max, "begin: prompt length out of range");
     seat_rows(n_windows, 1, prompts, max_depth);
     if (prefill) feed_positions(prompt_range(prompts).first - 1, nullptr);
-    WB_CUDA(cudaStreamSynchronize(st));
 }
 
 void Session::teacher_forced_logits(const int64_t* toks, int64_t n_rows, int64_t seq_len, float* logits_out) {
@@ -547,12 +595,14 @@
     WB_REQUIRE(max_lp + max_depth <= t_max, "greedy: prompt + max_depth exceeds the session's max_text_len");
     begin(prompts, false, max_depth);
     if (max_depth > 0) launch_decoder(DecodeLaunch::greedy_search(R, min_lp, max_lp, max_depth, (int)eot, loop_rules));
-    std::vector<int> tk((size_t)R * t_max), len((size_t)R);
-    std::vector<float> lp((size_t)R * t_max);
-    int sdv[128] = {0};
-    WB_CUDA(cudaMemcpyAsync(tk.data(), tokens.p, tk.size() * sizeof(int), cudaMemcpyDeviceToHost, st));
-    WB_CUDA(cudaMemcpyAsync(lp.data(), token_lp.p, lp.size() * sizeof(float), cudaMemcpyDeviceToHost, st));
-    WB_CUDA(cudaMemcpyAsync(len.data(), lengths.p, len.size() * sizeof(int), cudaMemcpyDeviceToHost, st));
+    int* tk = h_res.get();
+    int* len = tk + (size_t)Rmax * t_max;
+    int* sdv = len + Rmax;
+    const float* lp = h_res_lp.get();
+    std::fill(sdv, sdv + 128, 0);
+    WB_CUDA(cudaMemcpyAsync(tk, tokens.p, (size_t)R * t_max * sizeof(int), cudaMemcpyDeviceToHost, st));
+    WB_CUDA(cudaMemcpyAsync(h_res_lp.get(), token_lp.p, (size_t)R * t_max * sizeof(float), cudaMemcpyDeviceToHost, st));
+    WB_CUDA(cudaMemcpyAsync(len, lengths.p, (size_t)R * sizeof(int), cudaMemcpyDeviceToHost, st));
     if (max_depth > 0) WB_CUDA(cudaMemcpyAsync(sdv, steps_done.p, sizeof(int) * std::min(last_groups, 128), cudaMemcpyDeviceToHost, st));
     WB_CUDA(cudaStreamSynchronize(st));
     int sd = 0;
@@ -563,11 +613,11 @@
     out_lp.assign((size_t)R, {});
     for (int r = 0; r < R; ++r) {
         const int64_t prompt_len = (int64_t)prompts[(size_t)r].size();
-        for (int i = 0; i < len[(size_t)r]; ++i) {
+        for (int i = 0; i < len[r]; ++i) {
             out[(size_t)r].push_back(tk[(size_t)r * t_max + i]);
             out_lp[(size_t)r].push_back(i < prompt_len ? 0.0f : lp[(size_t)r * t_max + i]);
         }
-        if (loop_rules && max_depth > 0 && len[(size_t)r] <= prompt_len) out_lp[(size_t)r].back() = std::nanf("");
+        if (loop_rules && max_depth > 0 && len[r] <= prompt_len) out_lp[(size_t)r].back() = std::nanf("");
         if (loop_rules && out[(size_t)r].back() != eot) {
             out[(size_t)r].push_back(eot);
             out_lp[(size_t)r].push_back(std::nanf(""));
diff --git a/whisper-burn_b200/csrc/session.h b/whisper-burn_b200/csrc/session.h
--- a/whisper-burn_b200/csrc/session.h
+++ b/whisper-burn_b200/csrc/session.h
@@ -107,6 +107,20 @@
     int R = 0;
     int host_pos = 0;
     Pinned<int> h_parent, h_window, h_token, h_topk_id;
+    enum { STAGE_GEOMETRY, STAGE_SPECIAL, STAGE_SEAT, N_STAGES };
+    cudaEvent_t stage_ev[N_STAGES] = {};
+    Pinned<LogMelWindow> h_lmwin;
+    Pinned<GemmGroup> h_g1, h_g2;
+    Pinned<AttnWindow> h_awin;
+    Pinned<int64_t> h_win_row_off;
+    Pinned<int> h_win_T;
+    Pinned<uint8_t> h_special;
+    std::vector<uint8_t> special_host;
+    Pinned<int> h_seat;
+    Pinned<int> h_res;
+    Pinned<float> h_res_lp;
+    void stage_wait(int i) { WB_CUDA(cudaEventSynchronize(stage_ev[i])); }
+    void stage_done(int i) { WB_CUDA(cudaEventRecord(stage_ev[i], st)); }
     cudaEvent_t ev[6] = {};
     float last_ms[4] = {0, 0, 0, 0};
     int64_t last_steps = 0;
@@ -142,6 +156,7 @@
     void load_encoder_output_host(const float* xa_host, int64_t n, int64_t T);
     void run_encoder();
     void run_cross_kv();
+    void cross_kv_per_layer();
 
     void set_search(int rule) {
         WB_REQUIRE(rule == WB_SEARCH_BEAM || rule == WB_SEARCH_GREEDY_LOOP, "set_search: unknown search rule");
diff --git a/whisper-burn_b200/csrc/wb_internal.h b/whisper-burn_b200/csrc/wb_internal.h
--- a/whisper-burn_b200/csrc/wb_internal.h
+++ b/whisper-burn_b200/csrc/wb_internal.h
@@ -213,6 +213,7 @@
     __half* tok_emb16_tiled = nullptr;
     float* dec_pos = nullptr;
     std::vector<DecBlockW> dec;
+    LinearW ckv_all;
     LayerNormW dec_ln;
     float* zero_bias = nullptr;
 
@@ -263,13 +264,21 @@
     int max_rows = 0;
 };
 bool gemm_f16_supported(const GemmF16Params& p);
+struct CkvDest {
+    void* dst = nullptr;
+    bool half = false;
+    const int64_t* win_row_off = nullptr;
+    const int* win_T = nullptr;
+    int n_windows = 0, d = 0;
+    int64_t layer_stride = 0;
+};
 class GemmF16Plan {
 public:
     GemmF16Plan();
     ~GemmF16Plan();
     GemmF16Plan(const GemmF16Plan&) = delete;
     GemmF16Plan& operator=(const GemmF16Plan&) = delete;
-    void build(const GemmF16Params& p, int64_t a_group_stride, int a_rows_total_per_group);
+    void build(const GemmF16Params& p, int64_t a_group_stride, int a_rows_total_per_group, const CkvDest* ckv = nullptr);
     void launch(cudaStream_t st) const;
     bool matches(int max_rows, int n_groups) const { return impl != nullptr && key_rows == max_rows && key_groups == n_groups; }
 private:
diff --git a/whisper-burn_b200/ffi.py b/whisper-burn_b200/ffi.py
--- a/whisper-burn_b200/ffi.py
+++ b/whisper-burn_b200/ffi.py
@@ -68,6 +68,8 @@
     "wb_session_encode_mels": (C.c_int, [_P, _F, C.c_int64, C.c_int64, C.c_int64]),
     "wb_session_get_mel": (C.c_int, [_P, C.c_int64, _F, C.c_int64, _I64]),
     "wb_session_get_encoder_output": (C.c_int, [_P, C.c_int64, _F, C.c_int64, _I64]),
+    "wb_session_get_cross_kv": (C.c_int, [_P, C.c_int64, _P, C.c_int64, _I64]),
+    "wb_session_recompute_cross_kv_per_layer": (C.c_int, [_P]),
     "wb_session_begin": (C.c_int, [_P, _I64, C.c_int64]),
     "wb_session_step": (C.c_int, [_P, C.c_int64, _I32, _I32, _I64, C.c_int, _U8, C.c_int, _I64, _F]),
     "wb_transcribe_windows": (C.c_int, [_P, C.POINTER(_F), _I64, C.c_int64, C.c_int, C.c_int,
diff --git a/whisper-burn_b200/transcribe.py b/whisper-burn_b200/transcribe.py
--- a/whisper-burn_b200/transcribe.py
+++ b/whisper-burn_b200/transcribe.py
@@ -83,6 +83,17 @@
         ffi.check(ffi.lib().wb_session_get_encoder_output(self._h, window, ffi.fptr(buf), cap, C.byref(n)))
         return buf[:d * n.value].reshape(n.value, d).copy()
 
+    def get_cross_kv(self, layer: int) -> np.ndarray:
+        cfg = self.whisper.config
+        cap = 4 * self.max_windows * ((self.max_mel_frames - 1) // 2 + 1) * 2 * cfg.n_text_state
+        buf = np.empty(cap, dtype=np.uint8)
+        n = C.c_int64(0)
+        ffi.check(ffi.lib().wb_session_get_cross_kv(self._h, layer, buf.ctypes.data_as(C.c_void_p), cap, C.byref(n)))
+        return buf[:n.value].copy()
+
+    def recompute_cross_kv_per_layer(self) -> None:
+        ffi.check(ffi.lib().wb_session_recompute_cross_kv_per_layer(self._h))
+
     def begin(self, prompt: Sequence[int]) -> None:
         p = np.asarray(prompt, dtype=np.int64)
         ffi.check(ffi.lib().wb_session_begin(self._h, ffi.i64ptr(p), len(p)))
```

After: 2654 (median of 6 runs). Within noise of the previous version (+0.3%).
